# amazon-science/gnn-tail-generalization

Hardware: AMD Instinct MI355X
Metric: teachergnn_fullgraph_train_steps_per_sec (higher is better)
Workload: dtype f32

## Files before the change

gnn-tail-generalization_amd/_lib.py:

```python
import ctypes
import os

import torch

_HERE = os.path.dirname(os.path.abspath(__file__))
LIB_PATH = os.path.join(_HERE, 'lib', 'libcoldbrew_hip.so')

_c_i32p = ctypes.c_void_p
_c_f32p = ctypes.c_void_p
_I64 = ctypes.c_int64
_I32 = ctypes.c_int32
_SZ = ctypes.c_size_t
_P = ctypes.c_void_p


class CsrView(ctypes.Structure):
    _fields_ = [('rowptr', _P), ('col', _P), ('col_flags', _I32), ('n_rows', _I64), ('n_edges', _I64),
                ('hub_threshold', _I32), ('n_hubs', _I32), ('n_chunks', _I32), ('hub_rows', _P), ('hub_chunk_ptr', _P),
                ('ws', _P), ('ws_bytes', _SZ)]


class TrunkStore(ctypes.Structure):
    _fields_ = [('mix_src', _P), ('ld_mix', _I64), ('mix_index', _P), ('c_act', ctypes.c_float), ('c_mix', ctypes.c_float), ('drop_p', ctypes.c_float),
                ('seed', ctypes.c_uint64), ('seed_dev', _P), ('row0', _I64), ('relu_bits', _P), ('bits_relu_only', _I32), ('out_act', _P), ('ld_act', _I64)]


_G = ctypes.POINTER(CsrView)
_S = ctypes.POINTER(TrunkStore)

SIGNATURES = {
    'cb_version': (ctypes.c_int, []),
    'cb_last_error': (ctypes.c_char_p, []),
    'cb_device_status': (ctypes.c_int, []),
    'cb_agg_gemm_handover_selftest': (ctypes.c_int, [_P]),
    'cb_rows_zero_outside_mask_f32': (ctypes.c_int, [_P, _I64, _I64, _I64, _P, _P, _P]),
    'cb_csr_workspace_bytes': (_SZ, [_I64, _I64]),
    'cb_csr_from_coo_i64': (ctypes.c_int, [_P, _P, _I64, _I64, _P, _P, _P, _P, _P, _P, _SZ, _P]),
    'cb_deg_norm_f32': (ctypes.c_int, [_P, _I64, _P, _P]),
    'cb_csr64_from_coo_i64': (ctypes.c_int, [_P, _P, _I64, _I64, _P, _P, _P, _P, _P, _P, _SZ, _P]),
    'cb_csr_rebase_i64': (ctypes.c_int, [_P, _I64, _I64, _P, _P]),
    'cb_deg_norm_i64ptr_f32': (ctypes.c_int, [_P, _I64, _P, _P]),
    'cb_spmm_hub_count': (ctypes.c_int, [_P, _I64, _I32, _P, _P]),
    'cb_spmm_hub_fill_scratch_ints': (_I64, [_I64]),
    'cb_spmm_hub_fill': (ctypes.c_int, [_P, _I64, _I32, _I32, _P, _P, _P, _P]),
    'cb_spmm_workspace_bytes': (_SZ, [_I64, _I64]),
    'cb_spmm_csr_f32': (ctypes.c_int, [_G, _P, _I32, _I64, _I64, _P, _P, _P, ctypes.c_int, _P, _I64, _P, _I64, _P]),
    'cb_dropout_f32': (ctypes.c_int, [_P, _P, _I64, ctypes.c_float, ctypes.c_uint64, _P, _I64, _P]),
    'cb_axpby_f32': (ctypes.c_int, [ctypes.c_float, _P, ctypes.c_float, _P, _P, _I64, _P]),
    'cb_colsum_workspace_bytes': (_SZ, [_I64, _I64]),
    'cb_act_bwd_f32': (ctypes.c_int, [_P, _P, _P, _P, _I64, _I64, _P, _P, _SZ, _P]),
    'cb_reduce_workspace_bytes': (_SZ, []),
    'cb_frobenius_norm_f32': (ctypes.c_int, [_P, _I64, _P, _P, _SZ, _P]),
    'cb_nll_logsoftmax_f32': (ctypes.c_int, [_P, _I64, _P, _P, _I64, _I64, _I64, _P, _P, _P, _SZ, _P]),
    'cb_adam_step_f32': (ctypes.c_int, [_P, _P, _P, _P, _I64, ctypes.c_float, ctypes.c_float, ctypes.c_float,
                                        ctypes.c_float, ctypes.c_float, _I64, _P, _P]),
    'cb_adam_multi_f32': (ctypes.c_int, [_I32, _P, _P, _P, _P, _P, _P, ctypes.c_float, ctypes.c_float, ctypes.c_float, ctypes.c_float,
                                         ctypes.c_float, _I64, _P, _P, _P]),
    'cb_gemm_nn_workspace_bytes': (_SZ, [_I64, _I64]),
    'cb_gemm_nn_splitk_workspace_bytes': (_SZ, [_I64, _I64, _I64]),
    'cb_gemm_nn_f32': (ctypes.c_int, [_P, _I64, _P, _I64, _P, _I64, _I64, _I64, _I64, _P, _P, _I64, _P, ctypes.c_int, _P, _SZ, _P]),
    'cb_gemm_nn_drop2_f32': (ctypes.c_int, [_P, _I64, _P, _I64, _P, _I64, _P, _I64, _I64, _I64, _I64, _P, _P, _I64, _P, ctypes.c_int,
                                            ctypes.c_float, ctypes.c_uint64, _P, _I64, _P, _SZ, _P]),
    'cb_gemm_tn_workspace_bytes': (_SZ, [_I64, _I64, _I64]),
    'cb_gemm_tn_f32': (ctypes.c_int, [_P, _I64, _P, _I64, _P, _P, _I64, _I64, _I64, _P, _SZ, _P]),
    'cb_spmm_csr_fused_f32': (ctypes.c_int, [_G, _P, _P, _I32, _I64, _I64, _P, _P, _P, _I64, _S, _P, _I64, _P]),
    'cb_trunk_layer_bwd_f32': (ctypes.c_int, [_P, _P, _P, _P, ctypes.c_int, _P, ctypes.c_int, _I64, _I64, ctypes.c_float, ctypes.c_uint64,
                                              _P, _I64, ctypes.c_float, ctypes.c_float, _P, ctypes.c_uint64, ctypes.c_float, _P, _P, _P, _SZ, _P]),
    'cb_gemm_nn_bf16out_f32': (ctypes.c_int, [_P, _I64, _P, _I64, _P, _I64, _I64, _I64, _I64, _P, _P, _I64, _P, ctypes.c_int, _P, _SZ, _P]),
    'cb_node_norm_fwd_f32': (ctypes.c_int, [_P, _P, _P, _I64, _I64, ctypes.c_float, ctypes.c_float, ctypes.c_float, _P]),
    'cb_node_norm_bwd_f32': (ctypes.c_int, [_P, _P, _P, _P, _I64, _I64, ctypes.c_float, ctypes.c_float, _P]),
    'cb_colstats_workspace_bytes': (_SZ, [_I64, _I64]),
    'cb_colstats_f32': (ctypes.c_int, [_P, _P, _P, _I64, _I64, _P, _P, _P, _SZ, _P]),
    'cb_col_affine_f32': (ctypes.c_int, [_P, _P, _P, _P, ctypes.c_float, _P, _I64, _I64, _P]),
    'cb_col_bwd_combine_f32': (ctypes.c_int, [_P, _P, _P, _P, _P, _P, ctypes.c_float, ctypes.c_float, _P, _I64, _I64, _P]),
    'cb_topk_replace_workspace_bytes': (_SZ, [_I64, _I64, _I64]),
    'cb_topk_replace_f32': (ctypes.c_int, [_P, _I64, _P, _I64, _I64, _I64, _I64, _I32, _P, _P, _P, _P, _SZ, _P]),
    'cb_gather_rows_f32': (ctypes.c_int, [_P, _I64, _P, _I64, _I64, _P, _P]),
    'cb_gather_rows_bf16_f32': (ctypes.c_int, [_P, _I64, _P, _I64, _I64, _P, _P]),
    'cb_adam_norm_workspace_bytes': (ctypes.c_size_t, [_I32]),
    'cb_adam_multi_norm_f32': (ctypes.c_int, [_I32, _P, _P, _P, _P, _P, _P, _P, ctypes.c_float, ctypes.c_float, ctypes.c_float, ctypes.c_float,
                                              ctypes.c_float, _I64, _P, _P, _P, _SZ, _P]),
    'cb_expand_rows_f32': (ctypes.c_int, [_P, _P, _I64, _I64, ctypes.c_float, _P, _P]),
    'cb_gemm_nn_store_rows_supported': (ctypes.c_int, [_P, _I64, _P, _I64, _P, _I64, _I64, _I64, _I64]),
    'cb_gemm_nn_store_rows_f32': (ctypes.c_int, [_P, _I64, _P, _I64, _P, _I64, _I64, _I64, _I64, _P, _P, _I64, _P, _P, _S, _P, _SZ, _P]),
    'cb_trunk_store_rows_f32': (ctypes.c_int, [_P, _P, _I64, _I64, _S, _P, _P]),
    'cb_agg_gemm_image_bytes': (_SZ, [_I64, _I64]),
    'cb_agg_gemm_image_f32': (ctypes.c_int, [_P, _I64, _I64, _I64, ctypes.c_int, _P, _SZ, _P]),
    'cb_spmm_gemm_f32': (ctypes.c_int, [_G, _P, _I64, _I64, _P, _P, ctypes.c_int, _P, _I64, _P, _I64, _P, _P, _P, _I64, _P, _I64, _P]),
    'cb_spmm_gemm_fused_f32': (ctypes.c_int, [_G, _P, _I64, _P, _I64, _I64, _P, _P, _S, _P, _I64, _I32, _P, _P, _P, _I64, _P, _I64, _P]),
    'cb_agg_gemm_head_image_bytes': (_SZ, [_I64, _I64]),
    'cb_agg_gemm_head_image_f32': (ctypes.c_int, [_P, _I64, _I64, _I64, ctypes.c_int, _P, _SZ, _P]),
    'cb_spmm_gemm_fused_head_f32': (ctypes.c_int, [_G, _P, _I64, _P, _I64, _I64, _P, _P, _S, _P, _I64, _I32, _P, _P, _I64, _P, _I64, _P]),
    'cb_spmm_gemm_store_rows_f32': (ctypes.c_int, [_G, _P, _I64, _I64, _P, _P, _I64, _P, _P, _P, _P, _S, _P, _I64, _P]),
    'cb_spmm_csr_weighted_f32': (ctypes.c_int, [_P, _P, _P, _I64, _I64, _P, _I64, _I64, _P, _P, ctypes.c_int, _P, _I64, _P]),
    'cb_spmm_edge_dot_f32': (ctypes.c_int, [_P, _P, _I64, _I64, _P, _I64, _P, _I64, _I64, _P, _P]),
    'cb_gemm_nn_indrop_supported': (ctypes.c_int, [_P, _I64, _P, _I64, _P, _I64, _P, _I64, _I64, _I64, _I64]),
    'cb_gemm_nn_indrop_drop2_f32': (ctypes.c_int, [_P, _I64, _P, _I64, _P, _I64, _P, _I64, _I64, _I64, _I64, _P, ctypes.c_int, ctypes.c_float,
                                                   ctypes.c_uint64, ctypes.c_float, ctypes.c_uint64, _P, _I64, _P, _P]),
    'cb_gemm_nn_indrop_f32': (ctypes.c_int, [_P, _I64, _P, _I64, _P, _I64, _I64, _I64, _I64, _P, _P, _I64, _P, ctypes.c_int, ctypes.c_float,
                                             ctypes.c_uint64, _P, _I64, _P, _P]),
    'cb_gemm_tn_adrop_supported': (ctypes.c_int, [_P, _I64, _P, _I64, _I64, _I64]),
    'cb_gemm_tn_adrop_f32': (ctypes.c_int, [_P, _I64, _P, _I64, _P, _P, _I64, _I64, _I64, ctypes.c_float, ctypes.c_uint64, _P, _I64, _P, _SZ, _P]),
    'cb_front_image_bytes': (_SZ, [_I64]),
    'cb_front_image_f32': (ctypes.c_int, [_P, _I64, _I64, ctypes.c_int, _P, _SZ, _P]),
    'cb_trunk_front_f32': (ctypes.c_int, [_P, _I64, _I64, _I64, _P, _P, _P, _P, _P, _I64, _P, _I64, _P, _P, _I64, _P, _I64, ctypes.c_float,
                                          ctypes.c_uint64, ctypes.c_uint64, _P, _I64, _P]),
    'cb_gemm_tn_gdrop_supported': (ctypes.c_int, [_P, _I64, _P, _I64, _I64, _I64]),
    'cb_gemm_tn_gdrop_f32': (ctypes.c_int, [_P, _I64, _P, _I64, _P, _I64, _I64, _I64, ctypes.c_float, ctypes.c_uint64, _P, _I64, _P, _SZ, _P]),
    'cb_spmm_csr_lp_f32': (ctypes.c_int, [_G, _P, _I64, _I64, _P, _P, _I64, ctypes.c_float, _P, _P, _I64, _P]),
    'cb_spmm_csr_prop_f32': (ctypes.c_int, [_G, _P, _I64, _I64, _P, _P, _I64, ctypes.c_float, ctypes.c_float, ctypes.c_float, _P, _P, _P, _I64, _P]),
    'cb_cs_workspace_bytes': (_SZ, [_I64, _I64]),
    'cb_cs_residual_init_f32': (ctypes.c_int, [_P, _I64, _P, _P, _I64, _I64, _I64, _P, _P, _P, _P, _P, _SZ, _P]),
    'cb_cs_correct_snap_f32': (ctypes.c_int, [_I32, _P, _I64, _P, _I64, _P, _P, _I64, _I64, _I64, _P, _I64, ctypes.c_float, _P, _P, _I64, _P, _P, _P]),
    'cb_trunk_input_bwd_multi_f32': (ctypes.c_int, [_P, ctypes.c_uint64, _I32, _P, _P, ctypes.c_float, _P, _P, _I64, _I64, ctypes.c_float,
                                                    _P, _I64, _P, _P, _SZ, _P, _P, _P]),
    'cb_trunk_input_bwd_multi_cs_f32': (ctypes.c_int, [_P, ctypes.c_uint64, _I32, _P, _P, ctypes.c_float, _P, _P, _I64, _I64, ctypes.c_float,
                                                       _P, _I64, _P, _P, _SZ, _P, _P, _I32, _P, _P, _P, _P, _P, _SZ, _P]),
    'cb_spmm_csr_store_bwd_f32': (ctypes.c_int, [_G, _P, _I64, _I64, _P, _P, _P, ctypes.c_float, ctypes.c_float, ctypes.c_uint64, _P, _I64, _P, _I64, _P, _I64, _P]),
    'cb_spmm_store_bwd_mix_workspace_bytes': (_SZ, [_I64, _I64, _I64]),
    'cb_spmm_csr_store_bwd_mix_f32': (ctypes.c_int, [_G, _P, _I64, _I64, _P, _P, _P, ctypes.c_float, ctypes.c_float, ctypes.c_uint64, _P, _I64, _P, _I64, _P, _I64,
                                                     _I32, _P, _P, _P, ctypes.c_float, _P, _P, _SZ, _P]),
    'cb_gemm_tn_instage_supported': (ctypes.c_int, [_P, _P, _P, _I64, _I64, _I64]),
    'cb_gemm_tn_instage_workspace_bytes': (_SZ, [_I64, _I64]),
    'cb_gemm_tn_instage_f32': (ctypes.c_int, [_P, _P, _P, _P, _I64, _P, _P, _I64, _I64, ctypes.c_float, ctypes.c_uint64, ctypes.c_float, ctypes.c_uint64, _P, _I64,
                                              _P, _SZ, _P]),
    'cb_trunk_layer_bwd_fold_f32': (ctypes.c_int, [_P, _P, _P, _P, _I64, _I64, ctypes.c_float, ctypes.c_uint64, _P, _I64, ctypes.c_float, ctypes.c_float, _I32, _P, _P, _P,
                                                   _P, _P, _P, _SZ, _I32, _P, ctypes.c_float, _P, _P, _SZ, _P]),
    'cb_trunk_layer_bwd_rows_f32': (ctypes.c_int, [_P, _P, _I64, _P, _P, _P, _I64, ctypes.c_float, ctypes.c_uint64, _P, _I64, ctypes.c_float,
                                                   _P, ctypes.c_uint64, ctypes.c_float, _P, _P, _P, _SZ, _P]),
    'cb_id_count_i64': (ctypes.c_int, [_P, _I64, _I64, _P, _P, _P]),
    'cb_value_hist_i32': (ctypes.c_int, [_P, _I64, _I32, _P, _P, _P]),
    'cb_compact_workspace_bytes': (_SZ, [_I64]),
    'cb_select_range_i32': (ctypes.c_int, [_P, _I64, _I32, _I32, _P, _P, _P, _P, _SZ, _P]),
    'cb_craft_isolation_i64': (ctypes.c_int, [_P, _P, _I64, _P, _I64, _P, _P, _P, _P, _SZ, _P]),
    'cb_symmetrize_workspace_bytes': (_SZ, [_I64, _I64]),
    'cb_symmetrize_i64': (ctypes.c_int, [_P, _P, _I64, _I64, _P, _P, _P, _P, _P, _SZ, _P]),
    'cb_trunk_input_bwd_f32': (ctypes.c_int, [_P, _P, _P, _P, _I64, _I64, ctypes.c_float, ctypes.c_uint64, _P, _I64, _P, _P, _SZ, _P]),
    'cb_ln_gelu_drop_fwd_f32': (ctypes.c_int, [_P, _I64, _I64, _P, _P, ctypes.c_float, ctypes.c_float, ctypes.c_uint64, _P, _P, _P, _P]),
    'cb_ln_gelu_drop_bwd_workspace_bytes': (_SZ, [_I64, _I64]),
    'cb_ln_gelu_drop_bwd_f32': (ctypes.c_int, [_P, _P, _P, _I64, _I64, _P, _P, ctypes.c_float, ctypes.c_uint64, _P, _P, _P, _P, _P, _P, _SZ, _P]),
    'cb_mse_rows_f32': (ctypes.c_int, [_P, _I64, _I64, _P, _I64, _I64, _P, _P, _P, _P, _SZ, _P]),
    'cb_part2_assemble_f32': (ctypes.c_int, [_P, _I64, _P, _P, _I64, _P, _I64, _P, _P]),
    'cb_part2_assemble_bwd_f32': (ctypes.c_int, [_P, _I64, _P, _P, _I64, _I64, _P, _P, _SZ, _P]),
    'cb_ncloss_positions_i64': (ctypes.c_int, [_P, _I64, _I64, _P, _P, _P]),
    'cb_ncloss_row_norms_f32': (ctypes.c_int, [_P, _I64, _I64, _I64, _P, _P, _P]),
    'cb_cosine_scale_f32': (ctypes.c_int, [_P, _I64, _I64, _P, _P]),
    'cb_ncloss_uses_limb_core': (ctypes.c_int, [_P, _I64, _I64]),
    'cb_ncloss_workspace_bytes': (_SZ, [_I64, _I32]),
    'cb_ncloss_fwd_f32': (ctypes.c_int, [_P, _I64, _I64, _I64, ctypes.c_float, _P, _P, _P, _I64, _P, _P, _P, _I32, _P, _P, _P, _P, _P, _P, _P, _P, _SZ, _P]),
    'cb_ncloss_normalize_rows_f32': (ctypes.c_int, [_P, _I64, _I64, _I64, _P, _P, _P]),
    'cb_ncloss_bwd_slab_f32': (ctypes.c_int, [_P, _I64, _I64, _I64, ctypes.c_float, _P, _P, _I64, _I64, _I32, _P, _I64, _P]),
    'cb_ncloss_bwd_finish_f32': (ctypes.c_int, [_P, _I64, _P, _I64, _I64, ctypes.c_float, _P, _P, _P, _P, _P, _P, _P, _P, _I64, _P, _P, _P, _P, _P, _P, _P]),
    'cb_spgemm_offsets_workspace_bytes': (_SZ, [_I64]),
    'cb_spgemm_entry_offsets_i64': (ctypes.c_int, [_P, _I64, _P, _I64, _P, _P, _P, _SZ, _P]),
    'cb_spgemm_chunk_workspace_bytes': (_SZ, [_I64]),
    'cb_spgemm_chunk_count_f32': (ctypes.c_int, [_P, _P, _P, _P, _P, _P, _P, _I64, _I64, _I64, _I64, _I64, _P, _P, _SZ, _P]),
    'cb_spgemm_chunk_emit_f32': (ctypes.c_int, [_P, _SZ, _I64, _I64, _I64, _I64, _I64, _I64, _P, _P, _P, _P]),
    'cb_csr_transpose_workspace_bytes': (_SZ, [_I64]),
    'cb_csr_transpose_f32': (ctypes.c_int, [_P, _P, _P, _I64, _I64, _I64, _P, _P, _P, _P, _SZ, _P]),
    'cb_linkp_max_tries': (ctypes.c_int, []),
    'cb_linkp_valid_counts_i32': (ctypes.c_int, [_P, _P, _I32, _P, _P]),
    'cb_linkp_positives_i32': (ctypes.c_int, [_P, _P, _I32, _P, _I64, _I64, ctypes.c_uint64, _P, _P, _P]),
    'cb_linkp_negatives_i32': (ctypes.c_int, [_P, _P, _I32, _P, _I64, _I64, ctypes.c_uint64, _P, _P, _P, _P]),
    'cb_linkp_loss_fwd_f32': (ctypes.c_int, [_P, _I64, _I64, _I64, _P, _I64, _P, _I64, _P, _P, _P, _P, _P]),
    'cb_linkp_mrr_f32': (ctypes.c_int, [_P, _I64, _P, _I64, _P, _P]),
    'cb_linkp_bwd_workspace_bytes': (_SZ, [_I64, _I64]),
    'cb_linkp_loss_bwd_f32': (ctypes.c_int, [_P, _I64, _I64, _I64, _P, _I64, _P, _I64, _P, _P, _P, _I64, _P, _SZ, _P]),
    'cb_heur_aa_weights_f64': (ctypes.c_int, [_P, _P, _P]),
    'cb_heur_pair_scores_f32': (ctypes.c_int, [_P, _P, _P, _I64, _P, _P, _P]),
    'cb_heur_pair_scores_width_f32': (ctypes.c_int, [_P, _P, _P, _I64, _I32, _P, _P, _P]),
    'cb_rank_counts_workspace_bytes': (_SZ, [_I64, _I64]),
    'cb_rank_counts_f32': (ctypes.c_int, [_P, _I64, _P, _I64, _P, _P, _P, _P, _SZ, _P]),
    'cb_pair_gemm_nn_supported': (ctypes.c_int, [_P, _I64, _P, _I64, _I64, _I64]),
    'cb_pair_gemm_nn_f32': (ctypes.c_int, [_P, _I64, _I64, _P, _I64, _P, _I64, _P, _I64, _P, _I64, _I64, _I64, _P, ctypes.c_int, ctypes.c_float,
                                           ctypes.c_uint64, _P, _I64, _P, _P]),
    'cb_pair_dot_f32': (ctypes.c_int, [_P, _I64, _I64, _I64, _P, _I64, _P, _P, _P]),
    'cb_pair_scatter_workspace_bytes': (_SZ, [_I64]),
    'cb_pair_scatter_f32': (ctypes.c_int, [_P, _I64, _I64, _I64, _P, _I64, _P, _I64, _P, _I64, _P, _SZ, _P]),
    'cb_rank_loss_workspace_bytes': (_SZ, []),
    'cb_rank_loss_fwd_f32': (ctypes.c_int, [_I32, _P, _I64, _P, _I64, _P, _P, _P, _SZ, _P]),
    'cb_rank_loss_bwd_f32': (ctypes.c_int, [_I32, _P, _I64, _P, _I64, _P, _P, _P, _P, _P]),
    'cb_sage_image_bytes': (_SZ, [ctypes.c_int]),
    'cb_sage_image_f32': (ctypes.c_int, [_P, _I64, _P, _I64, ctypes.c_int, _P, _SZ, _P]),
    'cb_sage_layer_supported': (ctypes.c_int, [_I64, _I64, _I32, _P, _I64, _P, _I64, _P, _I64, _P, _I64]),
    'cb_sage_layer_f32': (ctypes.c_int, [_P, _P, _I64, _P, _I64, _P, _P, _P, _P, ctypes.c_int, ctypes.c_float, ctypes.c_uint64, _P, _I64, _P, _I64, _I32,
                                         _P, _I64, _P]),
}

_lib = None


class HipExtensionError(RuntimeError):
    pass


def load():
    global _lib
    if _lib is not None:
        return _lib
    if not os.path.isfile(LIB_PATH):
        raise HipExtensionError(
            f'{LIB_PATH} not found: the HIP extension is required (no CPU fallback). '
            'Build it with `python __graft_entry__.py` or `make -C gnn-tail-generalization_amd/csrc`.')
    lib = ctypes.CDLL(LIB_PATH)
    for name, (res, args) in SIGNATURES.items():
        fn = getattr(lib, name)
        fn.restype = res
        fn.argtypes = args
# ... 69 lines not shown
```

gnn-tail-generalization_amd/csrc/cb_front.hip:

```cpp
#include "cb_common.h"
#include "cb_limb_core.h"
#include "cb_philox.h"
#include "cb_tile_gemm.h"
#include "cb_trunk_store.h"

namespace cb {

struct FrontArgs {
  const float* x;
  int64_t ld_x;
  const uint4* image_in;
  const float* bias_in;
  const uint4* image_0;
  const float* rowscale;
  const float* addend;
  int64_t ld_add;
  float* x0;
  int64_t ld_x0;
  unsigned long long* bits;
  float* x0_drop;
  int64_t ld_drop;
  float* z0;
  int64_t ld_z;
  int64_t M;
  uint32_t thresh;
  float keep_scale;
  uint64_t seed_x, seed_x0;
  const uint64_t* seed_dev;
  int64_t row0;
  int n_tiles;
};

template <int NS1>
__global__ void __launch_bounds__(256, 2) k_front(FrontArgs fa) {
  constexpr int K1 = 16 * NS1, LDX = K1 + 4, NV = kTM * K1 / 4 / 256;
  static_assert(NV >= 1 && kTM * LDX <= kTM * kTLD, "x tile must fit the region of the X0 tile");
  __shared__ __attribute__((aligned(16))) float tile[kTM * kTLD];
  constexpr int kScratch = 2 * RowOperand<kTM>::BYTES > 4 * 8 * kCLD * 4 ? 2 * RowOperand<kTM>::BYTES : 4 * 8 * kCLD * 4;
  __shared__ __attribute__((aligned(16))) char scratch[kScratch];
  float (*cstrip)[8 * kCLD] = reinterpret_cast<float (*)[8 * kCLD]>(scratch);
  __shared__ float rs_tile[2][kTM];
  const int t = threadIdx.x, lane = t & 63, w = __builtin_amdgcn_readfirstlane(t >> 6);
  const uint64_t sx = fa.seed_dev ? fa.seed_x + *fa.seed_dev : fa.seed_x, s0 = fa.seed_dev ? fa.seed_x0 + *fa.seed_dev : fa.seed_x0;
  float4 xr[NV];
  auto load_x = [&](int tile_id) {
    const int64_t m0 = (int64_t)tile_id * kTM;
#pragma unroll
    for (int j = 0; j < NV; ++j) {
      const int idx = t + 256 * j, row = idx / (K1 / 4), c4 = idx % (K1 / 4);
      const int64_t m = m0 + row;
      xr[j] = (tile_id < fa.n_tiles && m < fa.M) ? *reinterpret_cast<const float4*>(fa.x + m * fa.ld_x + 4 * c4) : make_float4(0.f, 0.f, 0.f, 0.f);
    }
  };
  float bvec[4] = {0.f, 0.f, 0.f, 0.f};
  if (fa.bias_in) {
#pragma unroll
    for (int i = 0; i < 4; ++i) bvec[i] = fa.bias_in[4 * lane + i];
  }
  int par = 0;
  for (int tile_id = blockIdx.x; tile_id < fa.n_tiles; tile_id += gridDim.x, par ^= 1) {
    const int64_t m0 = (int64_t)tile_id * kTM;
    load_x(tile_id);
#pragma unroll
    for (int j = 0; j < NV; ++j) {
      const int idx = t + 256 * j, row = idx / (K1 / 4), c4 = idx % (K1 / 4);
      float v[4] = {xr[j].x, xr[j].y, xr[j].z, xr[j].w};
      if (fa.thresh) {
        float mk[4];
        keep4(sx, ((fa.row0 + m0 + row) * K1 + 4 * c4) >> 2, fa.thresh, fa.keep_scale, mk);
#pragma unroll
        for (int i = 0; i < 4; ++i) v[i] = mul_rounded(v[i], mk[i]);
      }
      *reinterpret_cast<float4*>(tile + row * LDX + 4 * c4) = make_float4(v[0], v[1], v[2], v[3]);
    }
    if (t < kTM) rs_tile[par][t] = (fa.rowscale && m0 + t < fa.M) ? fa.rowscale[m0 + t] : 1.f;
    __syncthreads();
    f32x16 acc[2][2];
    tile_times_image_coop<NS1, LDX, 1>(tile, scratch, fa.image_in, w, lane, t, acc);
    {
      const int l31 = lane & 31, lh = lane >> 5;
#pragma unroll
      for (int i = 0; i < 2; ++i)
#pragma unroll
        for (int j = 0; j < 2; ++j)
#pragma unroll
          for (int reg = 0; reg < 16; ++reg)
            tile[(32 * i + (reg & 3) + 8 * (reg >> 2) + 4 * lh) * kTLD + 64 * w + 32 * j + l31] = acc[i][j][reg];
    }
    __syncthreads();
#pragma unroll 4
    for (int r = 0; r < 16; ++r) {
      const int row = 16 * w + r;
      const int64_t m = m0 + row;
      float* tp = tile + row * kTLD + 4 * lane;
      const float4 v = *reinterpret_cast<const float4*>(tp);
      float o[4] = {v.x, v.y, v.z, v.w};
#pragma unroll
      for (int i = 0; i < 4; ++i) o[i] = fmaxf(o[i] + bvec[i], 0.f);
      float xd[4] = {o[0], o[1], o[2], o[3]};
      if (fa.thresh) {
        float mk[4];
        keep4(s0, ((fa.row0 + m) * kND + 4 * lane) >> 2, fa.thresh, fa.keep_scale, mk);
#pragma unroll
        for (int i = 0; i < 4; ++i) xd[i] = o[i] * mk[i];
      }
      *reinterpret_cast<float4*>(tp) = make_float4(xd[0], xd[1], xd[2], xd[3]);
      if (m < fa.M) {
        store_stream4(fa.x0 + m * fa.ld_x0 + 4 * lane, o);
        if (fa.bits) {
          const bool pos[4] = {o[0] > 0.f, o[1] > 0.f, o[2] > 0.f, o[3] > 0.f};
          write_row_mask_words(fa.bits + m * 4, lane, pos);
        }
        if (fa.x0_drop) store_stream4(fa.x0_drop + m * fa.ld_drop + 4 * lane, xd);
      }
    }
    __syncthreads();
    tile_times_image_coop<kNS, kTLD, 1>(tile, scratch, fa.image_0, w, lane, t, acc);
    acc_rows_through_strip(acc, cstrip[w], w, lane, [&](int row, int n, const float4& v) {
      const int64_t m = m0 + row;
      if (m < fa.M) {
        const float rs = rs_tile[par][row];
        float ad[4] = {0.f, 0.f, 0.f, 0.f};
        if (fa.addend) {
          const float4 a4 = *reinterpret_cast<const float4*>(fa.addend + m * fa.ld_add + n);
          ad[0] = a4.x; ad[1] = a4.y; ad[2] = a4.z; ad[3] = a4.w;
        }
        const float zero_bias = 0.f;
        float o[4] = {v.x, v.y, v.z, v.w};
#pragma unroll
        for (int e = 0; e < 4; ++e) o[e] = o[e] * rs + ad[e] + zero_bias;
        store_stream4(fa.z0 + m * fa.ld_z + n, o);
      }
    });
  }
}

}

using namespace cb;

extern "C" size_t cb_front_image_bytes(int64_t K) {
  if (K != 64 && K != 128) return 0;
  return (size_t)(K / 16) * kNT * 3 * 64 * sizeof(uint4);
}

extern "C" int cb_front_image_f32(const float* W, int64_t ld, int64_t K, int transpose, void* image, size_t image_bytes, void* stream) {
  CB_CHECK_ARG(cb_front_image_bytes(K) > 0, CB_E_INVALID, "cb_front_image_f32: K must be 64 or 128 (got %lld)", (long long)K);
  CB_CHECK_ARG(W && image && ld >= (transpose ? K : kND), CB_E_INVALID, "cb_front_image_f32: null pointer / bad leading dimension");
  CB_CHECK_ARG(image_bytes >= cb_front_image_bytes(K) && aligned16(image), CB_E_WORKSPACE, "cb_front_image_f32: image buffer too small or misaligned");
  const int64_t sk = transpose ? 1 : ld, sn = transpose ? ld : 1;
  const int ns = (int)(K / 16);
  hipLaunchKernelGGL(k_weight_image, dim3(ns * kNT * 64 / 256), dim3(256), 0, (hipStream_t)stream, W, sk, sn, (uint4*)image, ns);
  CB_LAUNCH_CHECK();
  return CB_OK;
}

extern "C" int cb_trunk_front_f32(const float* x, int64_t ld_x, int64_t M, int64_t K, const void* image_in, const float* bias_in, const void* image_0,
                                  const float* rowscale, const float* addend, int64_t ld_add, float* x0, int64_t ld_x0, uint64_t* relu_bits,
                                  float* x0_drop, int64_t ld_drop, float* z0, int64_t ld_z, float drop_p, uint64_t seed_x, uint64_t seed_x0,
                                  const uint64_t* seed_dev, int64_t row0, void* stream) {
  CB_CHECK_ARG(M >= 0 && cb_front_image_bytes(K) > 0 && drop_p >= 0.f && drop_p < 1.f && row0 >= 0, CB_E_INVALID,
               "cb_trunk_front_f32: bad size (K must be 64 or 128; hidden width 256) or p");
  CB_CHECK_ARG(M < ((int64_t)1 << 31) * kTM / 2, CB_E_RANGE, "cb_trunk_front_f32: size out of range");
  if (M == 0) return CB_OK;
  CB_CHECK_ARG(x && image_in && image_0 && x0 && z0, CB_E_INVALID, "cb_trunk_front_f32: null pointer");
  CB_CHECK_ARG(aligned16(x) && ld_x % 4 == 0 && ld_x >= K && aligned16(image_in) && aligned16(image_0) && aligned16(x0) && ld_x0 % 4 == 0 && ld_x0 >= kND &&
                   aligned16(z0) && ld_z % 4 == 0 && ld_z >= kND && (!addend || (aligned16(addend) && ld_add % 4 == 0 && ld_add >= kND)) &&
                   (!x0_drop || (aligned16(x0_drop) && ld_drop % 4 == 0 && ld_drop >= kND)) && (!relu_bits || (uintptr_t)relu_bits % 8 == 0),
               CB_E_INVALID, "cb_trunk_front_f32: 16-byte aligned rows required");
  FrontArgs fa{x, ld_x, (const uint4*)image_in, bias_in, (const uint4*)image_0, rowscale, addend, ld_add, x0, ld_x0, (unsigned long long*)relu_bits,
               x0_drop, ld_drop, z0, ld_z, M};
  fa.thresh = drop_p > 0.f ? dropout_threshold(drop_p) : 0u;
  fa.keep_scale = 1.f / (1.f - drop_p);
  fa.seed_x = seed_x; fa.seed_x0 = seed_x0; fa.seed_dev = seed_dev; fa.row0 = row0;
  fa.n_tiles = (int)((M + kTM - 1) / kTM);
  int dev = 0, n_cu = 0;
  if (hipGetDevice(&dev) != hipSuccess || hipDeviceGetAttribute(&n_cu, hipDeviceAttributeMultiprocessorCount, dev) != hipSuccess || n_cu <= 0) n_cu = 256;
  const int blocks = fa.n_tiles < 2 * n_cu ? fa.n_tiles : 2 * n_cu;
  const dim3 grid((unsigned)blocks), blk(256);
  hipStream_t st = (hipStream_t)stream;
  if (K == 64) hipLaunchKernelGGL((k_front<4>), grid, blk, 0, st, fa);
  else hipLaunchKernelGGL((k_front<8>), grid, blk, 0, st, fa);
  CB_LAUNCH_CHECK();
  return CB_OK;
}
```

gnn-tail-generalization_amd/csrc/cb_gemm.hip:

```cpp
#include <stdlib.h>

#include "cb_common.h"
#include "cb_gemm_core.h"
#include "cb_gemm_limb.h"

namespace cb {

template <int WM, int WN, bool ALIGNED, bool OUT_BF16, int BKT = BK, int WTN = 2>
__global__ void __launch_bounds__(256) k_gemm_nn(const float* __restrict__ A, int64_t lda, const float* __restrict__ B, int64_t ldb,
                                                 void* __restrict__ Cv, int64_t ldc, int64_t M, int N, int K, GemmEpilogue ep,
                                                 int n_row_blocks, int n_col_blocks, int c_vec_ok, int k_chunk) {
  using T = Tile<WM, WN, BKT, WTN>;
  if (k_chunk) {
    const int k0 = blockIdx.y * k_chunk;
    A += k0;
    B += (int64_t)k0 * ldb;
    Cv = reinterpret_cast<float*>(Cv) + (int64_t)blockIdx.y * M * ldc;
    K = min(k_chunk, K - k0);
  }
  constexpr int BM = T::BM, BN = T::BN, LDA = T::LDA, LDB = T::LDB;
  __shared__ __attribute__((aligned(16))) float smem[T::SMEM_FLOATS];
  auto As = [&](int b) { return smem + b * (BKT * LDA); };
  auto Bs = [&](int b) { return smem + 2 * BKT * LDA + b * (BKT * LDB); };
  const int per_group = 8 * n_col_blocks;
// ... 323 lines not shown
extern "C" int cb_gemm_nn_store_rows_supported(const float* A, int64_t lda, const float* B, int64_t ldb, const float* C, int64_t ldc, int64_t M, int64_t N,
                                               int64_t K) {
  return use_limb3() && N == 256 && M > 0 && limb3_nn_eligible(A, lda, B, ldb, N, K) && aligned16(C) && ldc % 4 == 0 ? 1 : 0;
}

extern "C" int cb_gemm_nn_store_rows_f32(const float* A, int64_t lda, const float* B, int64_t ldb, float* C, int64_t ldc, int64_t M, int64_t N, int64_t K,
                                         const float* rowscale, const float* addend, int64_t ld_add, const float* bias, const int64_t* row_index,
                                         const cb_trunk_store* store, void* ws, size_t ws_bytes, void* stream) {
  CB_CHECK_ARG(M >= 0 && N == 256 && K > 0, CB_E_INVALID, "cb_gemm_nn_store_rows_f32: bad size (N must be 256)");
  CB_CHECK_ARG(K < (1 << 24) && (M + 63) / 64 < (1 << 24), CB_E_RANGE, "cb_gemm_nn_store_rows_f32: size out of range");
  if (M == 0) return CB_OK;
  CB_CHECK_ARG(A && B && C && row_index && lda >= K && ldb >= N && ldc >= N && (!addend || ld_add >= N), CB_E_INVALID,
               "cb_gemm_nn_store_rows_f32: null pointer or leading dimension too small");
  const int rcs = check_trunk_store("cb_gemm_nn_store_rows_f32", store, N);
  if (rcs != CB_OK) return rcs;
  CB_CHECK_ARG(cb_gemm_nn_store_rows_supported(A, lda, B, ldb, C, ldc, M, N, K) && (!addend || (aligned16(addend) && ld_add % 4 == 0)), CB_E_INVALID,
               "cb_gemm_nn_store_rows_f32: shape / alignment outside the fused form (cb_gemm_nn_store_rows_supported)");
  GemmEpilogue ep{rowscale, addend, ld_add, bias, 1, nullptr, 0, 0u, 1.f, 0ull, nullptr, 0, 0};
  ep.row_ids = row_index; ep.st = make_trunk_store(*store);
  return launch_nn_limb3(A, lda, B, ldb, C, ldc, M, N, K, ep, false, (hipStream_t)stream, ws, ws_bytes);
}

extern "C" int cb_gemm_tn_f32(const float* A, int64_t lda, const float* G, int64_t ldg, const float* rowscale, float* C, int64_t M,
                              int64_t K1, int64_t K2, void* ws, size_t ws_bytes, void* stream) {
  CB_CHECK_ARG(M >= 0 && K1 >= 0 && K2 >= 0, CB_E_INVALID, "cb_gemm_tn_f32: negative size");
  CB_CHECK_ARG(K1 < (1 << 20) && K2 < (1 << 20), CB_E_RANGE, "cb_gemm_tn_f32: size out of range");
  if (K1 == 0 || K2 == 0) return CB_OK;
  CB_CHECK_ARG(C && (M == 0 || (A && G)) && lda >= K1 && ldg >= K2, CB_E_INVALID, "cb_gemm_tn_f32: null pointer or bad ld");
  hipStream_t st = (hipStream_t)stream;
  if (M == 0) {
    CB_HIP(hipMemsetAsync(C, 0, (size_t)K1 * K2 * sizeof(float), st));
    return CB_OK;
  }
  CB_CHECK_ARG(ws && ws_bytes >= cb_gemm_tn_workspace_bytes(M, K1, K2), CB_E_WORKSPACE, "cb_gemm_tn_f32: workspace too small");
  int bm, bn;
  tn_tile(K1, K2, bm, bn);
  if (bm == 64) return launch_tn<1, 4>(A, lda, G, ldg, rowscale, C, M, K1, K2, (float*)ws, st);
  if (bm == 256) return launch_tn<4, 1>(A, lda, G, ldg, rowscale, C, M, K1, K2, (float*)ws, st);
  return launch_tn<2, 2>(A, lda, G, ldg, rowscale, C, M, K1, K2, (float*)ws, st);
}

extern "C" int cb_gemm_tn_gdrop_supported(const float* A, int64_t lda, const float* G, int64_t ldg, int64_t K1, int64_t K2) {
  return use_limb3() && K2 % 4 == 0 && limb3_tn_eligible(A, lda, G, ldg, K1, K2) ? 1 : 0;
}

extern "C" int cb_gemm_tn_gdrop_f32(const float* A, int64_t lda, const float* G, int64_t ldg, float* C, int64_t M, int64_t K1, int64_t K2,
                                    float g_drop_p, uint64_t g_seed, const uint64_t* seed_dev, int64_t row0, void* ws, size_t ws_bytes,
                                    void* stream) {
  CB_CHECK_ARG(M >= 0 && K1 >= 0 && K2 >= 0 && g_drop_p > 0.f && g_drop_p < 1.f && row0 >= 0, CB_E_INVALID, "cb_gemm_tn_gdrop_f32: bad size or p");
  CB_CHECK_ARG(K1 < (1 << 20) && K2 < (1 << 20), CB_E_RANGE, "cb_gemm_tn_gdrop_f32: size out of range");
  if (K1 == 0 || K2 == 0) return CB_OK;
  CB_CHECK_ARG(C && (M == 0 || (A && G)) && lda >= K1 && ldg >= K2, CB_E_INVALID, "cb_gemm_tn_gdrop_f32: null pointer or bad ld");
  hipStream_t st = (hipStream_t)stream;
  if (M == 0) {
    CB_HIP(hipMemsetAsync(C, 0, (size_t)K1 * K2 * sizeof(float), st));
    return CB_OK;
  }
  CB_CHECK_ARG(cb_gemm_tn_gdrop_supported(A, lda, G, ldg, K1, K2), CB_E_INVALID, "cb_gemm_tn_gdrop_f32: operands outside the three-limb path");
  CB_CHECK_ARG(ws && ws_bytes >= cb_gemm_tn_workspace_bytes(M, K1, K2), CB_E_WORKSPACE, "cb_gemm_tn_gdrop_f32: workspace too small");
  const DropSpec gd{dropout_threshold(g_drop_p), 1.f / (1.f - g_drop_p), g_seed, seed_dev, row0, K2};
  int bm, bn;
  tn_tile(K1, K2, bm, bn);
  if (bm == 64) return launch_tn<1, 4>(A, lda, G, ldg, nullptr, C, M, K1, K2, (float*)ws, st, &gd);
  if (bm == 256) return launch_tn<4, 1>(A, lda, G, ldg, nullptr, C, M, K1, K2, (float*)ws, st, &gd);
  return launch_tn<2, 2>(A, lda, G, ldg, nullptr, C, M, K1, K2, (float*)ws, st, &gd);
}

static inline int instage_splits(int64_t M) { return tn_splits(M, 2); }

extern "C" int cb_gemm_tn_instage_supported(const float* g, const float* mfold, const float* X, int64_t ldx, int64_t M, int64_t K2) {
  return use_limb3() && K2 > 64 && K2 <= 128 && K2 % 4 == 0 && ldx % 4 == 0 && ldx >= K2 && ldx < (1 << 22) && aligned16(g) && aligned16(mfold) && aligned16(X) && M > 0 &&
                 instage_splits(M) >= 256
             ? 1
             : 0;
}

extern "C" size_t cb_gemm_tn_instage_workspace_bytes(int64_t M, int64_t K2) {
  if (M <= 0 || K2 <= 0) return 0;
  return (size_t)instage_splits(M) * (size_t)256 * (size_t)(K2 + 1) * sizeof(float);
}

extern "C" int cb_gemm_tn_instage_f32(const float* g, const float* mfold, const uint64_t* x0_bits, const float* X, int64_t ldx, float* C, float* colsum, int64_t M,
                                      int64_t K2, float g_drop_p, uint64_t g_seed, float x_drop_p, uint64_t x_seed, const uint64_t* seed_dev, int64_t row0, void* ws,
                                      size_t ws_bytes, void* stream) {
  CB_CHECK_ARG(M > 0 && K2 > 0 && g_drop_p > 0.f && g_drop_p < 1.f && x_drop_p > 0.f && x_drop_p < 1.f && row0 >= 0, CB_E_INVALID,
               "cb_gemm_tn_instage_f32: bad size or p (both dropouts must be active)");
  CB_CHECK_ARG(g && mfold && x0_bits && X && C && colsum && (uintptr_t)x0_bits % 8 == 0, CB_E_INVALID, "cb_gemm_tn_instage_f32: null or misaligned pointer");
  CB_CHECK_ARG(cb_gemm_tn_instage_supported(g, mfold, X, ldx, M, K2), CB_E_INVALID, "cb_gemm_tn_instage_f32: shape / alignment outside the fused form (cb_gemm_tn_instage_supported)");
  CB_CHECK_ARG(ws && ws_bytes >= cb_gemm_tn_instage_workspace_bytes(M, K2), CB_E_WORKSPACE, "cb_gemm_tn_instage_f32: workspace too small");
  hipStream_t st = (hipStream_t)stream;
  const int nsplit = instage_splits(M);
  int64_t rows_per_split = (M + nsplit - 1) / nsplit;
  rows_per_split = (rows_per_split + 31) / 32 * 32;
  const DropSpec xd{dropout_threshold(x_drop_p), 1.f / (1.f - x_drop_p), x_seed, seed_dev, row0, K2};
  const DropSpec gd{dropout_threshold(g_drop_p), 1.f / (1.f - g_drop_p), g_seed, seed_dev, row0, 256};
  float* partial = (float*)ws;
  float* cs_partial = partial + (size_t)nsplit * 256 * K2;
  const int rc = launch_tn_instage(g, mfold, x0_bits, X, ldx, partial, cs_partial, M, K2, nsplit, rows_per_split, st, xd, gd);
  if (rc != CB_OK) return rc;
  const int64_t n = 256 * K2;
  hipLaunchKernelGGL(k_sum_partials, dim3((unsigned)((n + 255) / 256)), dim3(256), 0, st, (const float*)partial, nsplit, n, C);
  CB_LAUNCH_CHECK();
  hipLaunchKernelGGL(k_sum_partials, dim3(1), dim3(256), 0, st, (const float*)cs_partial, nsplit, (int64_t)256, colsum);
  CB_LAUNCH_CHECK();
  return CB_OK;
}

extern "C" int cb_gemm_nn_indrop_f32(const float* A, int64_t lda, const float* B, int64_t ldb, float* C, int64_t ldc, int64_t M, int64_t N, int64_t K,
                                     const float* rowscale, const float* addend, int64_t ld_add, const float* bias, int relu, float a_drop_p,
                                     uint64_t a_seed, const uint64_t* seed_dev, int64_t row0, uint64_t* relu_bits, void* stream) {
  CB_CHECK_ARG(M >= 0 && N >= 0 && K >= 0 && a_drop_p > 0.f && a_drop_p < 1.f && row0 >= 0, CB_E_INVALID, "cb_gemm_nn_indrop_f32: bad size or p");
  CB_CHECK_ARG(!relu_bits || (N == 256 && relu && (uintptr_t)relu_bits % 8 == 0), CB_E_INVALID,
               "cb_gemm_nn_indrop_f32: mask words of the ReLU exist for N == 256 with relu only");
  CB_CHECK_ARG(N < (1 << 24) && K < (1 << 24) && (M + 63) / 64 < (1 << 24), CB_E_RANGE, "cb_gemm_nn_indrop_f32: size out of range");
  if (M == 0 || N == 0) return CB_OK;
  CB_CHECK_ARG(C && A && B && lda >= K && ldb >= N && ldc >= N && (!addend || ld_add >= N), CB_E_INVALID, "cb_gemm_nn_indrop_f32: null pointer or bad ld");
  CB_CHECK_ARG(cb_gemm_nn_indrop_supported(A, lda, B, ldb, C, ldc, C, ldc, M, N, K) && (!addend || (aligned16(addend) && ld_add % 4 == 0)), CB_E_INVALID,
               "cb_gemm_nn_indrop_f32: shape / alignment outside the fused form (cb_gemm_nn_indrop_supported)");
  GemmEpilogue ep{rowscale, addend, ld_add, bias, relu, nullptr, 0, 0u, 1.f, 0ull, nullptr, 0, gemm_nt_store(M, N)};
  ep.adrop = DropSpec{dropout_threshold(a_drop_p), 1.f / (1.f - a_drop_p), a_seed, seed_dev, row0, K};
  ep.relu_bits_out = (unsigned long long*)relu_bits;
  return launch_nn_limb3(A, lda, B, ldb, C, ldc, M, N, K, ep, false, (hipStream_t)stream, nullptr, 0);
}

extern "C" int cb_gemm_tn_adrop_supported(const float* A, int64_t lda, const float* G, int64_t ldg, int64_t K1, int64_t K2) {
  int bm, bn;
  tn_tile(K1, K2, bm, bn);
  return use_limb3() && K1 % 4 == 0 && bm == 128 && limb3_tn_eligible(A, lda, G, ldg, K1, K2) ? 1 : 0;
}

extern "C" int cb_gemm_tn_adrop_f32(const float* A, int64_t lda, const float* G, int64_t ldg, const float* rowscale, float* C, int64_t M, int64_t K1,
                                    int64_t K2, float a_drop_p, uint64_t a_seed, const uint64_t* seed_dev, int64_t row0, void* ws, size_t ws_bytes,
                                    void* stream) {
  CB_CHECK_ARG(M >= 0 && K1 >= 0 && K2 >= 0 && a_drop_p > 0.f && a_drop_p < 1.f && row0 >= 0, CB_E_INVALID, "cb_gemm_tn_adrop_f32: bad size or p");
  CB_CHECK_ARG(K1 < (1 << 20) && K2 < (1 << 20), CB_E_RANGE, "cb_gemm_tn_adrop_f32: size out of range");
  if (K1 == 0 || K2 == 0) return CB_OK;
  CB_CHECK_ARG(C && (M == 0 || (A && G)) && lda >= K1 && ldg >= K2, CB_E_INVALID, "cb_gemm_tn_adrop_f32: null pointer or bad ld");
  hipStream_t st = (hipStream_t)stream;
  if (M == 0) {
    CB_HIP(hipMemsetAsync(C, 0, (size_t)K1 * K2 * sizeof(float), st));
    return CB_OK;
  }
  CB_CHECK_ARG(cb_gemm_tn_adrop_supported(A, lda, G, ldg, K1, K2), CB_E_INVALID, "cb_gemm_tn_adrop_f32: operands outside the three-limb 128-row tile path");
  CB_CHECK_ARG(ws && ws_bytes >= cb_gemm_tn_workspace_bytes(M, K1, K2), CB_E_WORKSPACE, "cb_gemm_tn_adrop_f32: workspace too small");
  const DropSpec ad{dropout_threshold(a_drop_p), 1.f / (1.f - a_drop_p), a_seed, seed_dev, row0, K1};
  return launch_tn<2, 2>(A, lda, G, ldg, rowscale, C, M, K1, K2, (float*)ws, st, nullptr, &ad);
}
```

gnn-tail-generalization_amd/csrc/cb_gemm_core.h:

```cpp
#pragma once
#include "cb_common.h"
#include "cb_philox.h"
#include "cb_trunk_store.h"

namespace cb {

typedef float f32x16 __attribute__((ext_vector_type(16)));

constexpr int BK = 16;

struct DropSpec {
  uint32_t thresh;
  float scale;
  uint64_t seed;
  const uint64_t* seed_dev;
  int64_t row0;
  int64_t width;
};

struct GemmEpilogue {
  const float* rowscale;
  const float* addend;
  int64_t ld_add;
  const float* bias;
  int relu;
  float* out2;
  int64_t ld_out2;
  uint32_t thresh;
  float keep_scale;
  uint64_t seed;
  const uint64_t* seed_dev;
  int64_t row0;
  int nt_store;
  DropSpec adrop;
  unsigned long long* relu_bits_out;
  const int64_t* row_ids;
  TrunkStore st;
};

template <int WM, int WN, int BKT = BK, int WTN = 2>
struct Tile {
  static constexpr int BM = 64 * WM, BN = 32 * WTN * WN, LDA = BM + 4, LDB = BN + 4;
  static constexpr int SMEM_FLOATS = 2 * BKT * (LDA + LDB);
  static_assert(WM * WN == 4, "four wavefronts per block");
  static_assert(32 * LDB <= SMEM_FLOATS, "epilogue staging (32 rows) must fit the operand buffers");
};

template <int LDA, int LDB, int BKT, int WTN>
__device__ __forceinline__ void mfma_tile_step(const float* __restrict__ As, const float* __restrict__ Bs, int wr, int wc,
                                               int lane, f32x16 (&acc)[2][WTN]) {
  const int l31 = lane & 31, kh = lane >> 5;
  const float* ar = As + kh * LDA + wr * 64 + l31;
  const float* br = Bs + kh * LDB + wc * (32 * WTN) + l31;
  float a[2], b[WTN];
  a[0] = ar[0]; a[1] = ar[32];
#pragma unroll
  for (int j = 0; j < WTN; ++j) b[j] = br[32 * j];
#pragma unroll
  for (int kk = 0; kk < BKT; kk += 2) {
    float na[2] = {0.f, 0.f}, nb[WTN];
#pragma unroll
    for (int j = 0; j < WTN; ++j) nb[j] = 0.f;
    if (kk + 2 < BKT) {
      na[0] = ar[(kk + 2) * LDA];
      na[1] = ar[(kk + 2) * LDA + 32];
#pragma unroll
      for (int j = 0; j < WTN; ++j) nb[j] = br[(kk + 2) * LDB + 32 * j];
    }
#pragma unroll
    for (int i = 0; i < 2; ++i)
#pragma unroll
      for (int j = 0; j < WTN; ++j) acc[i][j] = __builtin_amdgcn_mfma_f32_32x32x2f32(a[i], b[j], acc[i][j], 0, 0, 0);
    a[0] = na[0]; a[1] = na[1];
#pragma unroll
    for (int j = 0; j < WTN; ++j) b[j] = nb[j];
  }
}

template <int BMT, int BKT>
struct RowFrag {
  float v[BMT * BKT / 1024][4];
};
template <bool ALIGNED, int BMT, int BKT>
__device__ __forceinline__ void load_rowmajor(RowFrag<BMT, BKT>& f, const float* __restrict__ A, int64_t lda, int64_t m0, int64_t M,
                                              int k0, int K, int t) {
  constexpr int TPR = BKT / 4, RPP = 256 / TPR;
  const int k = k0 + (t % TPR) * 4;
#pragma unroll
  for (int j = 0; j < BMT / RPP; ++j) {
    const int64_t m = m0 + t / TPR + RPP * j;
    if (ALIGNED && m < M && k + 4 <= K) {
      const float4 x = *reinterpret_cast<const float4*>(A + m * lda + k);
      f.v[j][0] = x.x; f.v[j][1] = x.y; f.v[j][2] = x.z; f.v[j][3] = x.w;
    } else {
#pragma unroll
      for (int i = 0; i < 4; ++i) f.v[j][i] = (m < M && k + i < K) ? A[m * lda + k + i] : 0.f;
    }
  }
}
template <int BMT, int BKT>
// ... 220 lines not shown
```

gnn-tail-generalization_amd/csrc/cb_gemm_limb.hip:

```cpp
#include <utility>

#include "cb_common.h"
#include "cb_gemm_core.h"
#include "cb_gemm_limb.h"
#include "cb_limb_core.h"

namespace cb {

template <int WM, int WN, int WTN = 2, int PD = 1>
struct LTile {
  static constexpr int BM = 64 * WM, BN = 32 * WTN * WN;
  static constexpr int MINW = (WM == 2 && WTN == 2 && PD < 3 ? 3 : 2);
  static constexpr int NTHR = 64 * WM * WN;
  static_assert(WM * WN == 4 || WM * WN == 8, "four or eight wavefronts per block");
};

template <int WM, int WN, bool OUT_BF16, int WTN = 2, int PD = 1, int EPI = 0, bool ADROP = false>
__global__ void __launch_bounds__(256, (LTile<WM, WN, WTN, PD>::MINW)) k_gemm_nn_l3(const float* __restrict__ A, int64_t lda,
                                                                                 const float* __restrict__ B, int64_t ldb,
                                                                                 void* __restrict__ Cv, int64_t ldc, int64_t M, int N,
                                                                                 int K, GemmEpilogue ep, int n_row_blocks,
                                                                                 int n_col_blocks, int c_vec_ok) {
  using T = LTile<WM, WN, WTN>;
  using OA = RowOperand<T::BM, ADROP>;
  using OB = ColOperand<T::BN, false>;
  constexpr int BM = T::BM, BN = T::BN;
  constexpr int SMEM = 2 * (OA::BYTES + OB::BYTES);
  static_assert(32 * (BN + 4) * 4 <= SMEM, "epilogue staging must fit");
  __shared__ __attribute__((aligned(16))) char smem[SMEM];
  const int per_group = 8 * n_col_blocks;
  const int grp = blockIdx.x / per_group, r = blockIdx.x % per_group;
  const int row_blk = grp * 8 + (r & 7), col_blk = r >> 3;
  if (row_blk >= n_row_blocks) return;
  const int64_t m0 = (int64_t)row_blk * BM;
  const int n0 = col_blk * BN;
  const int t = threadIdx.x, lane = t & 63, w = t >> 6, wr = w / WN, wc = w % WN;

  f32x16 acc[2][WTN];
  zero_acc_n<WTN>(acc);
  OA oa;
  OB ob;
  oa.init(lda, M - m0, t);
  if constexpr (ADROP) oa.set_drop(ep.adrop, m0, K, t);
  ob.init(ldb, N - n0, t);
  const uint32_t aaddr[2] = {OA::frag_addr(wr * 64, lane), OA::frag_addr(wr * 64 + 32, lane)};
  uint32_t baddr[WTN];
#pragma unroll
  for (int j = 0; j < WTN; ++j) baddr[j] = OB::frag_addr(wc * (32 * WTN) + 32 * j, lane);
  limb_k_loop<WTN, PD, OA, OB>(oa, ob, smem, A + m0 * lda, KS, lda, B + n0, (int64_t)KS * ldb, ldb, nullptr, K, aaddr, baddr, acc, t);
  nn_epilogue<WM, WN, WTN, OUT_BF16, EPI>(acc, reinterpret_cast<float*>(smem), Cv, ldc, m0, n0, M, N, ep, c_vec_ok, t);
}

template <int WM, int WN, bool SCALED, int WTN = 2, int PD = 1, bool GDROP = false, bool ADROP = false>
__global__ void __launch_bounds__((LTile<WM, WN, WTN, PD>::NTHR), (LTile<WM, WN, WTN, PD>::MINW)) k_gemm_tn_l3(const float* __restrict__ A, int64_t lda,
                                                                                 const float* __restrict__ G, int64_t ldg,
                                                                                 const float* __restrict__ rowscale,
                                                                                 float* __restrict__ partial, int64_t M, int K1, int K2,
                                                                                 int64_t rows_per_split, int tiles_j, int n_tiles,
                                                                                 int nsplit, DropSpec gd) {
  using T = LTile<WM, WN, WTN>;
  using OA = ColOperand<T::BM, false, ADROP, T::NTHR>;
  using OB = ColOperand<T::BN, SCALED, GDROP, T::NTHR>;
  constexpr int BM = T::BM, BN = T::BN;
  __shared__ __attribute__((aligned(16))) char smem[2 * (OA::BYTES + OB::BYTES)];
  const int b = blockIdx.x;
  const int tile = (b >> 3) % n_tiles, split = (b & 7) + 8 * (b / (8 * n_tiles));
  if (split >= nsplit) return;
  const int i0 = (tile / tiles_j) * BM, j0 = (tile % tiles_j) * BN;
  const int64_t r_begin = (int64_t)split * rows_per_split;
  const int64_t r_end = min(M, r_begin + rows_per_split);
  const int t = threadIdx.x, lane = t & 63, w = t >> 6, wr = w / WN, wc = w % WN;

  f32x16 acc[2][WTN];
  zero_acc_n<WTN>(acc);
  OA oa;
  OB ob;
  oa.init(lda, K1 - i0, t);
  ob.init(ldg, K2 - j0, t);
  if constexpr (GDROP) ob.set_drop(gd, r_begin, r_end - r_begin, j0, t);
  if constexpr (ADROP) oa.set_drop(gd, r_begin, r_end - r_begin, i0, t);
  const uint32_t aaddr[2] = {OA::frag_addr(wr * 64, lane), OA::frag_addr(wr * 64 + 32, lane)};
  uint32_t baddr[WTN];
#pragma unroll
  for (int j = 0; j < WTN; ++j) baddr[j] = OB::frag_addr(wc * (32 * WTN) + 32 * j, lane);
  limb_k_loop<WTN, PD, OA, OB>(oa, ob, smem, A + r_begin * lda + i0, (int64_t)KS * lda, lda, G + r_begin * ldg + j0, (int64_t)KS * ldg, ldg,
                           SCALED ? rowscale + r_begin : nullptr, r_end - r_begin, aaddr, baddr, acc, t);
  const int l31 = lane & 31, lh = lane >> 5;
  float* P = partial + (int64_t)split * K1 * K2;
#pragma unroll
  for (int ti = 0; ti < 2; ++ti)
#pragma unroll
    for (int tj = 0; tj < WTN; ++tj) {
      const int n = j0 + wc * (32 * WTN) + tj * 32 + l31;
      if (n >= K2) continue;
#pragma unroll
      for (int reg = 0; reg < 16; ++reg) {
        const int m = i0 + wr * 64 + ti * 32 + (reg & 3) + 8 * (reg >> 2) + 4 * lh;
        if (m < K1) P[(int64_t)m * K2 + n] = acc[ti][tj][reg];
      }
    }
}

__global__ void __launch_bounds__(512, 2) k_gemm_tn_instage(const float* __restrict__ g, const float* __restrict__ mfold,
                                                            const unsigned long long* __restrict__ x0_bits, const float* __restrict__ X, int64_t ldx,
                                                            float* __restrict__ partial, float* __restrict__ cs_partial, int64_t M, int K2,
                                                            int64_t rows_per_split, int nsplit, DropSpec xd, DropSpec gd) {
  using T = LTile<4, 2, 2>;
  using OA = ColOperandInStage<T::NTHR>;
  using OB = ColOperand<T::BN, false, true, T::NTHR>;
  constexpr int K1 = 256;
  __shared__ __attribute__((aligned(16))) char smem[2 * (OA::BYTES + OB::BYTES)];
  const int split = blockIdx.x;
  if (split >= nsplit) return;
  const int64_t r_begin = (int64_t)split * rows_per_split;
  const int64_t r_end = min(M, r_begin + rows_per_split);
  const int t = threadIdx.x, lane = t & 63, w = t >> 6, wr = w / 2, wc = w % 2;

  f32x16 acc[2][2];
  zero_acc_n<2>(acc);
  OA oa;
  OB ob;
  oa.init(K1, K1, t);
  ob.init(ldx, K2, t);
  oa.set_stage(g, mfold, x0_bits + r_begin * 4, gd, r_begin, r_end - r_begin, t);
  ob.set_drop(xd, r_begin, r_end - r_begin, 0, t);
  const uint32_t aaddr[2] = {OA::frag_addr(wr * 64, lane), OA::frag_addr(wr * 64 + 32, lane)};
  uint32_t baddr[2];
#pragma unroll
  for (int j = 0; j < 2; ++j) baddr[j] = OB::frag_addr(wc * 64 + 32 * j, lane);
  limb_k_loop<2, 1, OA, OB>(oa, ob, smem, g + r_begin * K1, (int64_t)KS * K1, K1, X + r_begin * ldx, (int64_t)KS * ldx, ldx, nullptr, r_end - r_begin, aaddr, baddr,
                            acc, t);
  const int l31 = lane & 31, lh = lane >> 5;
  float* P = partial + (int64_t)split * K1 * K2;
#pragma unroll
  for (int ti = 0; ti < 2; ++ti)
#pragma unroll
    for (int tj = 0; tj < 2; ++tj) {
      const int n = wc * 64 + tj * 32 + l31;
      if (n >= K2) continue;
#pragma unroll
      for (int reg = 0; reg < 16; ++reg) {
        const int m = wr * 64 + ti * 32 + (reg & 3) + 8 * (reg >> 2) + 4 * lh;
        P[(int64_t)m * K2 + n] = acc[ti][tj][reg];
      }
    }
  float* red = reinterpret_cast<float*>(smem);
#pragma unroll
  for (int i = 0; i < 4; ++i) red[w * 256 + lane * 4 + i] = oa.cs[i];
  __syncthreads();
  if (t < 256) {
    float s = 0.f;
#pragma unroll
    for (int j = 0; j < 8; ++j) s += red[j * 256 + t];
    cs_partial[(int64_t)split * 256 + t] = s;
  }
}

int launch_tn_instage(const float* g, const float* mfold, const uint64_t* x0_bits, const float* X, int64_t ldx, float* partial, float* cs_partial, int64_t M, int64_t K2,
                      int nsplit, int64_t rows_per_split, hipStream_t st, const DropSpec& xd, const DropSpec& gd) {
  hipLaunchKernelGGL(k_gemm_tn_instage, dim3((unsigned)nsplit), dim3(512), 0, st, g, mfold, (const unsigned long long*)x0_bits, X, ldx, partial, cs_partial, M, (int)K2,
                     rows_per_split, nsplit, xd, gd);
  CB_LAUNCH_CHECK();
  return CB_OK;
}

template <int WM, int WN, bool OUT_BF16, int WTN = 2>
static int launch_nn_l3_t(const float* A, int64_t lda, const float* B, int64_t ldb, void* C, int64_t ldc, int64_t M, int64_t N,
                          int64_t K, GemmEpilogue ep, hipStream_t st, void* ws = nullptr, size_t ws_bytes = 0) {
  using T = LTile<WM, WN, WTN>;
  const int nrb = (int)((M + T::BM - 1) / T::BM), ncb = (int)((N + T::BN - 1) / T::BN);
  const int64_t groups = (nrb + 7) / 8;
  const int c_vec_ok = ((uintptr_t)C % (OUT_BF16 ? 8 : 16) == 0) && ldc % 4 == 0 && (!ep.addend || (aligned16(ep.addend) && ep.ld_add % 4 == 0));
  const dim3 grid((unsigned)(groups * 8 * ncb));
  if constexpr (!OUT_BF16 && WM == 2 && WTN == 4) {
    if (ep.out2) {
      if (ep.adrop.thresh)
        hipLaunchKernelGGL((k_gemm_nn_l3<WM, WN, false, WTN, 1, 1, true>), grid, dim3(256), 0, st, A, lda, B, ldb, C, ldc, M, (int)N, (int)K, ep,
                           nrb, ncb, c_vec_ok);
      else
        hipLaunchKernelGGL((k_gemm_nn_l3<WM, WN, false, WTN, 1, 1>), grid, dim3(256), 0, st, A, lda, B, ldb, C, ldc, M, (int)N, (int)K, ep, nrb,
                           ncb, c_vec_ok);
      CB_LAUNCH_CHECK();
      return CB_OK;
    }
    if (ep.row_ids) {
      hipLaunchKernelGGL((k_gemm_nn_l3<WM, WN, false, WTN, 1, 2>), grid, dim3(256), 0, st, A, lda, B, ldb, C, ldc, M, (int)N, (int)K, ep, nrb, ncb, c_vec_ok);
      CB_LAUNCH_CHECK();
      return CB_OK;
    }
    if (ep.adrop.thresh) {
      hipLaunchKernelGGL((k_gemm_nn_l3<WM, WN, false, WTN, 1, 0, true>), grid, dim3(256), 0, st, A, lda, B, ldb, C, ldc, M, (int)N, (int)K, ep, nrb,
                         ncb, c_vec_ok);
      CB_LAUNCH_CHECK();
      return CB_OK;
    }
  }
  CB_CHECK_ARG(!ep.adrop.thresh, CB_E_INVALID, "NN contraction with operand dropout: wide fp32 tile only (check cb_gemm_nn_indrop_supported first)");
  hipLaunchKernelGGL((k_gemm_nn_l3<WM, WN, OUT_BF16, WTN, 1>), grid, dim3(256), 0, st, A, lda, B, ldb, C, ldc, M, (int)N, (int)K, ep, nrb, ncb,
                     c_vec_ok);
  CB_LAUNCH_CHECK();
  return CB_OK;
}

bool limb3_nn_eligible(const float* A, int64_t lda, const float* B, int64_t ldb, int64_t N, int64_t K) {
  return aligned16(A) && aligned16(B) && lda % 4 == 0 && ldb % 4 == 0 && K % 4 == 0 && N % 4 == 0 && K > 0 && lda < (1 << 22) && ldb < (1 << 22);
}

bool limb3_nn_dual_eligible(const float* A, int64_t lda, const float* B, int64_t ldb, const float* C, int64_t ldc, const float* C2, int64_t ldc2,
                            int64_t M, int64_t N, int64_t K, const GemmEpilogue& ep) {
  return N > 128 && ((M + 127) / 128) * ((N + 255) / 256) >= 256 && limb3_nn_eligible(A, lda, B, ldb, N, K) && aligned16(C) && aligned16(C2) && ldc % 4 == 0 && ldc2 % 4 == 0 &&
         (!ep.addend || (aligned16(ep.addend) && ep.ld_add % 4 == 0));
}

size_t limb3_nn_workspace_bytes(int64_t, int64_t) { return 0; }

int launch_nn_limb3(const float* A, int64_t lda, const float* B, int64_t ldb, void* C, int64_t ldc, int64_t M, int64_t N, int64_t K,
                    const GemmEpilogue& ep, bool out_bf16, hipStream_t st, void* ws, size_t ws_bytes) {
  if (N <= 64) {
    return out_bf16 ? launch_nn_l3_t<4, 1, true>(A, lda, B, ldb, C, ldc, M, N, K, ep, st)
                    : launch_nn_l3_t<4, 1, false>(A, lda, B, ldb, C, ldc, M, N, K, ep, st);
  }
  const bool fills = ((M + 127) / 128) * ((N + 255) / 256) >= 256 || ep.out2 || ep.adrop.thresh || ep.row_ids;
  if (N > 128 && fills)
    return out_bf16 ? launch_nn_l3_t<2, 2, true, 4>(A, lda, B, ldb, C, ldc, M, N, K, ep, st, ws, ws_bytes)
                    : launch_nn_l3_t<2, 2, false, 4>(A, lda, B, ldb, C, ldc, M, N, K, ep, st, ws, ws_bytes);
  return out_bf16 ? launch_nn_l3_t<2, 2, true>(A, lda, B, ldb, C, ldc, M, N, K, ep, st, ws, ws_bytes)
                  : launch_nn_l3_t<2, 2, false>(A, lda, B, ldb, C, ldc, M, N, K, ep, st, ws, ws_bytes);
}

template <int WM, int WN, int WTN = 2>
static void launch_tn_l3_t(const float* A, int64_t lda, const float* G, int64_t ldg, const float* rowscale, float* partial, int64_t M,
                           int64_t K1, int64_t K2, int nsplit, int64_t rows_per_split, hipStream_t st, const DropSpec& gd, const DropSpec& ad) {
  using T = LTile<WM, WN, WTN>;
  const int ti = (int)((K1 + T::BM - 1) / T::BM), tj = (int)((K2 + T::BN - 1) / T::BN);
  const dim3 grid((unsigned)(((nsplit + 7) / 8) * 8 * ti * tj));
#define CB_TN_LAUNCH(SC_, GD_, AD_)                                                                                                  \
  hipLaunchKernelGGL((k_gemm_tn_l3<WM, WN, SC_, WTN, 1, GD_, AD_>), grid, dim3(T::NTHR), 0, st, A, lda, G, ldg, rowscale, partial, M, (int)K1, \
                     (int)K2, rows_per_split, tj, ti * tj, nsplit, gd.thresh ? gd : ad)
  if (gd.thresh) CB_TN_LAUNCH(false, true, false);
  else if (ad.thresh) {
    if constexpr (WM == 2 && WN == 2 && WTN == 2) { if (rowscale) CB_TN_LAUNCH(true, false, true); else CB_TN_LAUNCH(false, false, true); }
  } else if (rowscale) CB_TN_LAUNCH(true, false, false);
  else CB_TN_LAUNCH(false, false, false);
#undef CB_TN_LAUNCH
}

bool limb3_tn_eligible(const float* A, int64_t lda, const float* G, int64_t ldg, int64_t K1, int64_t K2) {
  return aligned16(A) && aligned16(G) && lda % 4 == 0 && ldg % 4 == 0 && K1 % 4 == 0 && K2 % 4 == 0 && lda < (1 << 22) && ldg < (1 << 22);
}

int launch_tn_limb3(const float* A, int64_t lda, const float* G, int64_t ldg, const float* rowscale, float* partial, int64_t M,
                    int64_t K1, int64_t K2, int bm, int nsplit, int64_t rows_per_split, hipStream_t st, const DropSpec* gdrop, const DropSpec* adrop) {
  const DropSpec gd = gdrop ? *gdrop : DropSpec{};
  const DropSpec ad = adrop ? *adrop : DropSpec{};
  CB_CHECK_ARG(!gd.thresh || (!rowscale && gd.width % 4 == 0 && !ad.thresh), CB_E_INVALID,
               "TN contraction: dropout of the G operand needs width %% 4 == 0, no row scale and no dropout of A");
  CB_CHECK_ARG(!ad.thresh || (ad.width % 4 == 0 && bm == 128), CB_E_INVALID, "TN contraction: dropout of the A operand needs width %% 4 == 0 and the 128-row tile");
  if (bm == 64) launch_tn_l3_t<1, 4>(A, lda, G, ldg, rowscale, partial, M, K1, K2, nsplit, rows_per_split, st, gd, ad);
  else if (bm == 256) launch_tn_l3_t<4, 1>(A, lda, G, ldg, rowscale, partial, M, K1, K2, nsplit, rows_per_split, st, gd, ad);
  else {
    if (!ad.thresh && !gd.thresh && K1 == 256 && K2 == 256 && nsplit >= 256) {
      launch_tn_l3_t<4, 2, 4>(A, lda, G, ldg, rowscale, partial, M, K1, K2, nsplit, rows_per_split, st, gd, ad);
      CB_LAUNCH_CHECK();
      return CB_OK;
    }
    if (gd.thresh && !ad.thresh && !rowscale && K1 == 256 && K2 <= 128 && K2 > 64 && nsplit >= 256) {
      launch_tn_l3_t<4, 2, 2>(A, lda, G, ldg, rowscale, partial, M, K1, K2, nsplit, rows_per_split, st, gd, ad);
      CB_LAUNCH_CHECK();
      return CB_OK;
    }
    if (!ad.thresh && K2 > 128 && ((K1 + 127) / 128) * ((K2 + 255) / 256) * nsplit >= 256) launch_tn_l3_t<2, 2, 4>(A, lda, G, ldg, rowscale, partial, M, K1, K2, nsplit, rows_per_split, st, gd, ad);
    else launch_tn_l3_t<2, 2>(A, lda, G, ldg, rowscale, partial, M, K1, K2, nsplit, rows_per_split, st, gd, ad);
  }
  CB_LAUNCH_CHECK();
  return CB_OK;
}

}
```

gnn-tail-generalization_amd/csrc/cb_limb_core.h:

```cpp
#pragma once
#include <utility>

#include "cb_common.h"
#include "cb_gemm_core.h"
#include "cb_philox.h"

namespace cb {

typedef __bf16 bf16x8 __attribute__((ext_vector_type(8)));

typedef float f32x2 __attribute__((ext_vector_type(2)));
typedef __bf16 bf16x2 __attribute__((ext_vector_type(2)));
__device__ __forceinline__ uint32_t cvt_pk_bf16(float x0, float x1) {
  const f32x2 v = {x0, x1};
  return __builtin_bit_cast(uint32_t, __builtin_convertvector(v, bf16x2));
}
__device__ __forceinline__ void split3x2(float a0, float a1, uint32_t& hi, uint32_t& mid, uint32_t& lo) {
  hi = cvt_pk_bf16(a0, a1);
  const float r0 = a0 - __uint_as_float(hi << 16), r1 = a1 - __uint_as_float(hi & 0xffff0000u);
  mid = cvt_pk_bf16(r0, r1);
  const float s0 = r0 - __uint_as_float(mid << 16), s1 = r1 - __uint_as_float(mid & 0xffff0000u);
  lo = cvt_pk_bf16(s0, s1);
}

// ... 47 lines not shown
      const bool in = row + 64 * j < rows_left;
      rmask |= in ? (1u << j) : 0u;
      voff[j] = in ? (uint32_t)((row + 64 * j) * ld + kq * 4) : 0u;
    }
  }
  template <int J>
  __device__ __forceinline__ void load(float4 (&f)[NV], const float* __restrict__ base, int64_t , int64_t k_left, const float*,
                                       int t) const {
    f[J] = *reinterpret_cast<const float4*>(base + ((t & 3) * 4 < k_left ? voff[J] : 0u));
  }
  template <int J>
  __device__ __forceinline__ void stage(const float4 (&f)[NV], char* __restrict__ S, int64_t k_left, int t) const {
    const bool live = ((rmask >> J) & 1) && (t & 3) * 4 < k_left;
    float v[4] = {live ? f[J].x : 0.f, live ? f[J].y : 0.f, live ? f[J].z : 0.f, live ? f[J].w : 0.f};
    if constexpr (DROP) {
      float mk[4];
      keep4(dseed, (dbase[J] + (dK - k_left)) >> 2, dthresh, dscale, mk);
#pragma unroll
      for (int i = 0; i < 4; ++i) v[i] = mul_rounded(v[i], mk[i]);
    }
    uint2 pl[3];
    split4(v, pl);
#pragma unroll
    for (int p = 0; p < 3; ++p) *reinterpret_cast<uint2*>(S + p * PLANE + woff + J * (64 * 32)) = pl[p];
  }
  static __device__ __forceinline__ uint32_t frag_addr(int r0, int lane) {
    const int row = r0 + (lane & 31);
    return row * 32 + (((lane >> 5) ^ ((row >> 3) & 1)) << 4);
  }
  static __device__ __forceinline__ bf16x8 frag(const char* __restrict__ S, uint32_t addr, int plane) {
    return __builtin_bit_cast(bf16x8, *reinterpret_cast<const uint4*>(S + plane * PLANE + addr));
  }
};

template <int R>
struct PairRowOperand {
  static constexpr int PLANE = R * 32, BYTES = 3 * PLANE, NV = R / 64;
  static_assert(NV >= 1, "tile rows");
  int32_t nu[NV], nv[NV];
  uint32_t woff;
  static constexpr bool HAS_SC = false;
  float sc[1];
  float4 fv[NV];
  static __device__ __forceinline__ bool pair_of(const int32_t* __restrict__ pairs, int64_t S, int64_t rows_left, int64_t N, int row, int& u, int& v, bool& in) {
    in = row < rows_left;
    u = in ? pairs[row] : 0;
    v = in ? pairs[S + row] : 0;
    return in && u >= 0 && u < N && v >= 0 && v < N;
  }
  __device__ __forceinline__ void init(const int32_t* __restrict__ pairs, int64_t S, int64_t rows_left, int64_t N, int t) {
    const int row = t >> 2, kq = t & 3;
    woff = row * 32 + (((kq >> 1) ^ ((row >> 3) & 1)) << 4) + ((kq & 1) << 3);
#pragma unroll
    for (int j = 0; j < NV; ++j) {
      int u, v;
      bool in;
      const bool ok = pair_of(pairs, S, rows_left, N, row + 64 * j, u, v, in);
      nu[j] = ok ? u : -1;
      nv[j] = ok ? v : 0;
    }
  }
  template <int J>
  __device__ __forceinline__ void load(float4 (&f)[NV], const float* __restrict__ base, int64_t ld, int64_t k_left, const float*, int t) {
    const int kq4 = (t & 3) * 4 < k_left ? (t & 3) * 4 : 0;
    f[J] = *reinterpret_cast<const float4*>(base + ((int64_t)(nu[J] < 0 ? 0 : nu[J]) * ld + kq4));
    fv[J] = *reinterpret_cast<const float4*>(base + ((int64_t)nv[J] * ld + kq4));
  }
  template <int J>
  __device__ __forceinline__ void stage(const float4 (&f)[NV], char* __restrict__ S, int64_t k_left, int t) const {
    const bool live = nu[J] >= 0 && (t & 3) * 4 < k_left;
    const float a[4] = {f[J].x, f[J].y, f[J].z, f[J].w}, b[4] = {fv[J].x, fv[J].y, fv[J].z, fv[J].w};
    float v[4];
#pragma unroll
    for (int i = 0; i < 4; ++i) v[i] = live ? mul_rounded(a[i], b[i]) : 0.f;
    uint2 pl[3];
    split4(v, pl);
#pragma unroll
    for (int p = 0; p < 3; ++p) *reinterpret_cast<uint2*>(S + p * PLANE + woff + J * (64 * 32)) = pl[p];
  }
  static __device__ __forceinline__ uint32_t frag_addr(int r0, int lane) { return RowOperand<R>::frag_addr(r0, lane); }
  static __device__ __forceinline__ bf16x8 frag(const char* __restrict__ S, uint32_t addr, int plane) { return RowOperand<R>::frag(S, addr, plane); }
};

template <int C, bool SCALED, bool DROP = false, int NT = 256>
struct ColOperand {
  static constexpr int ROWB = C * 2, PLANE = 16 * ROWB, BYTES = 3 * PLANE;
  static constexpr int TPR = C / 4, KPP = NT / TPR, NV = 16 / KPP;
  static_assert(KPP >= 4 && KPP % 4 == 0 && NV >= 1, "staging map: whole swizzle groups of k rows per pass");
  static constexpr int NC = C / 32;
  static_assert(NC == 2 || NC == 4 || NC == 8, "tile widths 64 / 128 / 256");
  static __device__ __forceinline__ int swz(int k) { return NC == 2 ? ((k >> 1) & 1) : (k & 3); }
  uint32_t voff[NV];
  uint32_t woff;
  bool cok;
  static constexpr bool HAS_SC = SCALED;
  float sc[SCALED ? NV : 1];
  uint64_t dseed;
  uint32_t dthresh;
  float dscale;
  int64_t drow, dtot, dwidth;
  int dcol;
  __device__ __forceinline__ void set_drop(const DropSpec& d, int64_t r_begin, int64_t total, int j0, int t) {
    dseed = d.seed_dev ? d.seed + *d.seed_dev : d.seed;
    dthresh = d.thresh;
    dscale = d.scale;
    drow = d.row0 + r_begin + t / TPR;
    dtot = total;
    dwidth = d.width;
    dcol = j0 + (t % TPR) * 4;
  }
  __device__ __forceinline__ void init(int64_t ld, int cols_left, int t) {
    const int k = t / TPR, nq = t % TPR;
    cok = nq * 4 < cols_left;
#pragma unroll
    for (int j = 0; j < NV; ++j) voff[j] = (uint32_t)((k + KPP * j) * ld + (cok ? nq * 4 : 0));
    woff = k * ROWB + ((((nq >> 3) ^ swz(k)) & (NC - 1)) << 6) + ((nq & 7) << 3);
  }
  template <int J>
  __device__ __forceinline__ void load(float4 (&f)[NV], const float* __restrict__ base, int64_t , int64_t k_left,
                                       const float* __restrict__ kscale, int t) {
    const int k = t / TPR + KPP * J;
    const bool kin = k < k_left;
    f[J] = *reinterpret_cast<const float4*>(base + (kin ? voff[J] : 0u));
    if constexpr (SCALED) sc[J] = kscale[kin ? k : 0];
  }
  template <int J>
  __device__ __forceinline__ void stage(const float4 (&f)[NV], char* __restrict__ S, int64_t k_left, int t) const {
    const bool live = cok && t / TPR + KPP * J < k_left;
    const float m = SCALED ? sc[SCALED ? J : 0] : 1.f;
    float v[4] = {live ? f[J].x * m : 0.f, live ? f[J].y * m : 0.f, live ? f[J].z * m : 0.f, live ? f[J].w * m : 0.f};
    if constexpr (DROP) {
      static_assert(!SCALED, "dropout of a row-scaled operand is not needed anywhere");
      float mk[4];
      keep4(dseed, ((drow + KPP * J + (dtot - k_left)) * dwidth + dcol) >> 2, dthresh, dscale, mk);
#pragma unroll
      for (int i = 0; i < 4; ++i) v[i] = mul_rounded(v[i], mk[i]);
    }
    uint2 pl[3];
    split4(v, pl);
#pragma unroll
    for (int p = 0; p < 3; ++p) *reinterpret_cast<uint2*>(S + p * PLANE + woff + J * (KPP * ROWB)) = pl[p];
  }
  static __device__ __forceinline__ uint32_t frag_addr(int c0, int lane) {
    const int L = lane & 15, k = 8 * (lane >> 5) + (L >> 2);
    return k * ROWB + ((((c0 >> 5) ^ swz(k)) & (NC - 1)) << 6) + (((lane >> 4) & 1) << 5) + ((L & 3) << 3);
  }
  static __device__ __forceinline__ bf16x8 frag(const char* __restrict__ S, uint32_t addr, int plane) {
    const char* q = S + plane * PLANE + addr;
    const s16x4 lo = __builtin_amdgcn_ds_read_tr16_b64_v4i16((lds_s16x4*)(q));
    const s16x4 hi = __builtin_amdgcn_ds_read_tr16_b64_v4i16((lds_s16x4*)(q + 4 * ROWB));
    typedef short s16x8 __attribute__((ext_vector_type(8)));
    const s16x8 v = __builtin_shufflevector(lo, hi, 0, 1, 2, 3, 4, 5, 6, 7);
    return __builtin_bit_cast(bf16x8, v);
  }
};

template <int NT = 512>
struct ColOperandInStage {
  static constexpr int C = 256;
  static constexpr int ROWB = C * 2, PLANE = 16 * ROWB, BYTES = 3 * PLANE;
  static constexpr int TPR = C / 4, KPP = NT / TPR, NV = 16 / KPP;
  static_assert(TPR == 64 && KPP >= 4 && KPP % 4 == 0 && NV >= 1, "one wavefront per k row");
  static constexpr int NC = C / 32;
  static __device__ __forceinline__ int swz(int k) { return k & 3; }
  uint32_t voff[NV];
  uint32_t woff;
  bool cok;
  static constexpr bool HAS_SC = false;
  float sc[1];
  int64_t mdelta;
  const unsigned long long* bits;
  float4 fm[NV];
  unsigned long long bw[NV][4];
  uint64_t dseed;
  uint32_t dthresh;
  float dscale;
  int64_t drow, dtot, dwidth;
  int dcol, kw;
  float cs[4];
  __device__ __forceinline__ void set_stage(const float* g, const float* mfold, const unsigned long long* bits_block, const DropSpec& d, int64_t r_begin, int64_t total,
                                            int t) {
    mdelta = mfold - g;
    bits = bits_block;
    dseed = d.seed_dev ? d.seed + *d.seed_dev : d.seed;
    dthresh = d.thresh;
    dscale = d.scale;
    kw = __builtin_amdgcn_readfirstlane(t / TPR);
    drow = d.row0 + r_begin + kw;
    dtot = total;
    dwidth = d.width;
    dcol = (t % TPR) * 4;
#pragma unroll
    for (int i = 0; i < 4; ++i) cs[i] = 0.f;
  }
  __device__ __forceinline__ void init(int64_t ld, int cols_left, int t) {
    const int k = t / TPR, nq = t % TPR;
    cok = nq * 4 < cols_left;
#pragma unroll
    for (int j = 0; j < NV; ++j) voff[j] = (uint32_t)((k + KPP * j) * ld + (cok ? nq * 4 : 0));
    woff = k * ROWB + ((((nq >> 3) ^ swz(k)) & (NC - 1)) << 6) + ((nq & 7) << 3);
  }
  template <int J>
  __device__ __forceinline__ void load(float4 (&f)[NV], const float* __restrict__ base, int64_t , int64_t k_left, const float* __restrict__, int ) {
    const int k = kw + KPP * J;
    const bool kin = k < k_left;
    const float* p = base + (kin ? voff[J] : 0u);
    f[J] = *reinterpret_cast<const float4*>(p);
    fm[J] = *reinterpret_cast<const float4*>(p + mdelta);
    const unsigned long long* b = bits + ((dtot - k_left) + (kin ? k : 0)) * 4;
#pragma unroll
    for (int i = 0; i < 4; ++i) bw[J][i] = b[i];
  }
  template <int J>
  __device__ __forceinline__ void stage(const float4 (&f)[NV], char* __restrict__ S, int64_t k_left, int t) {
    const bool live = cok && kw + KPP * J < k_left;
    const int lane = t & 63;
    float mk[4];
    keep4(dseed, ((drow + KPP * J + (dtot - k_left)) * dwidth + dcol) >> 2, dthresh, dscale, mk);
    const float gv[4] = {f[J].x, f[J].y, f[J].z, f[J].w}, mv[4] = {fm[J].x, fm[J].y, fm[J].z, fm[J].w};
    float v[4];
#pragma unroll
    for (int i = 0; i < 4; ++i) {
      const float tsum = mul_rounded(gv[i], mk[i]) + mv[i];
      v[i] = (live && ((bw[J][i] >> lane) & 1ull)) ? tsum : 0.f;
      cs[i] += v[i];
    }
    uint2 pl[3];
    split4(v, pl);
#pragma unroll
    for (int p = 0; p < 3; ++p) *reinterpret_cast<uint2*>(S + p * PLANE + woff + J * (KPP * ROWB)) = pl[p];
  }
  static __device__ __forceinline__ uint32_t frag_addr(int c0, int lane) {
    const int L = lane & 15, k = 8 * (lane >> 5) + (L >> 2);
    return k * ROWB + ((((c0 >> 5) ^ swz(k)) & (NC - 1)) << 6) + (((lane >> 4) & 1) << 5) + ((L & 3) << 3);
  }
  static __device__ __forceinline__ bf16x8 frag(const char* __restrict__ S, uint32_t addr, int plane) {
    const char* q = S + plane * PLANE + addr;
    const s16x4 lo = __builtin_amdgcn_ds_read_tr16_b64_v4i16((lds_s16x4*)(q));
    const s16x4 hi = __builtin_amdgcn_ds_read_tr16_b64_v4i16((lds_s16x4*)(q + 4 * ROWB));
    typedef short s16x8 __attribute__((ext_vector_type(8)));
    const s16x8 v = __builtin_shufflevector(lo, hi, 0, 1, 2, 3, 4, 5, 6, 7);
    return __builtin_bit_cast(bf16x8, v);
  }
};

template <class OPA, class OPB>
struct Producer {
  OPA& oa;
  OPB& ob;
  float4 (&fa)[OPA::NV];
  float4 (&fb)[OPB::NV];
  char* dstA;
  char* dstB;
  const float* abase;
  const float* bbase;
  const float* bscale;
  int64_t lda, ldb;
  int64_t left1, left2;
  int t;
  bool do_stage = true;
  static constexpr int P = OPA::NV + OPB::NV;
  template <int PIECE>
  __device__ __forceinline__ void one() {
    if constexpr (PIECE < OPA::NV) {
      if (do_stage) oa.template stage<PIECE>(fa, dstA, left1, t);
      oa.template load<PIECE>(fa, abase, lda, left2, nullptr, t);
    } else {
      constexpr int J = PIECE - OPA::NV;
      if (do_stage) ob.template stage<J>(fb, dstB, left1, t);
      ob.template load<J>(fb, bbase, ldb, left2, bscale, t);
    }
  }
  template <int G, int NG, int... Is>
  __device__ __forceinline__ void group_impl(std::integer_sequence<int, Is...>) {
    ((Is * NG / P == G ? one<Is>() : void()), ...);
  }
  template <int G, int NG>
  __device__ __forceinline__ void group() { group_impl<G, NG>(std::make_integer_sequence<int, P>{}); }
};

template <int WTN, class OPA, class OPB, class PR>
__device__ __forceinline__ void limb_tile_step(const char* __restrict__ As, const char* __restrict__ Bs, const uint32_t (&aaddr)[2],
                                               const uint32_t (&baddr)[WTN], f32x16 (&acc)[2][WTN], PR& pr) {
  constexpr int NH = WTN / 2, NG = 6 * NH;
#define CB_MFMA4(A_, B_, H_, G_)                                                                             \
  _Pragma("unroll") for (int i = 0; i < 2; ++i) _Pragma("unroll") for (int j = 0; j < 2; ++j)               \
      acc[i][2 * H_ + j] = __builtin_amdgcn_mfma_f32_32x32x16_bf16(A_[i], B_[j], acc[i][2 * H_ + j], 0, 0, 0); \
  pr.template group<G_, NG>();
#define CB_HALF(H_)                                                                                                          \
  {                                                                                                                          \
    bf16x8 b_hi[2], b_mid[2], b_lo[2];                                                                                       \
    if (H_ == 0) { _Pragma("unroll") for (int i = 0; i < 2; ++i) a_lo[i] = OPA::frag(As, aaddr[i], 2); }                     \
    _Pragma("unroll") for (int j = 0; j < 2; ++j) b_hi[j] = OPB::frag(Bs, baddr[2 * H_ + j], 0);                             \
    if (H_ == 0) { _Pragma("unroll") for (int i = 0; i < 2; ++i) a_hi[i] = OPA::frag(As, aaddr[i], 0); }                     \
    _Pragma("unroll") for (int j = 0; j < 2; ++j) b_lo[j] = OPB::frag(Bs, baddr[2 * H_ + j], 2);                             \
    if (H_ == 0) { _Pragma("unroll") for (int i = 0; i < 2; ++i) a_mid[i] = OPA::frag(As, aaddr[i], 1); }                    \
    _Pragma("unroll") for (int j = 0; j < 2; ++j) b_mid[j] = OPB::frag(Bs, baddr[2 * H_ + j], 1);                            \
    CB_MFMA4(a_lo, b_hi, H_, H_ * 6 + 0)                                                                                     \
    CB_MFMA4(a_hi, b_lo, H_, H_ * 6 + 1)                                                                                     \
    CB_MFMA4(a_mid, b_mid, H_, H_ * 6 + 2)                                                                                   \
    CB_MFMA4(a_mid, b_hi, H_, H_ * 6 + 3)                                                                                    \
// ... 72 lines not shown
```

gnn-tail-generalization_amd/csrc/cb_philox.h:

```cpp
#pragma once
#include "cb_common.h"

namespace cb {

__device__ __forceinline__ void philox4x32_10(uint32_t c0, uint32_t c1, uint32_t k0, uint32_t k1, uint32_t (&out)[4]) {
  uint32_t c2 = 0x243F6A88u, c3 = 0x85A308D3u;
#pragma unroll
  for (int r = 0; r < 10; ++r) {
    const uint64_t p0 = (uint64_t)0xD2511F53u * (uint64_t)c0, p1 = (uint64_t)0xCD9E8D57u * (uint64_t)c2;
    const uint32_t hi0 = (uint32_t)(p0 >> 32), lo0 = (uint32_t)p0;
    const uint32_t hi1 = (uint32_t)(p1 >> 32), lo1 = (uint32_t)p1;
    const uint32_t n0 = hi1 ^ c1 ^ k0, n1 = lo1, n2 = hi0 ^ c3 ^ k1, n3 = lo0;
    c0 = n0; c1 = n1; c2 = n2; c3 = n3;
    k0 += 0x9E3779B9u;
    k1 += 0xBB67AE85u;
  }
  out[0] = c0; out[1] = c1; out[2] = c2; out[3] = c3;
}

__device__ __forceinline__ void keep4(uint64_t seed, int64_t quad, uint32_t thresh, float scale, float (&m)[4]) {
  uint32_t r[4];
  philox4x32_10((uint32_t)quad, (uint32_t)((uint64_t)quad >> 32), (uint32_t)seed, (uint32_t)(seed >> 32), r);
#pragma unroll
  for (int i = 0; i < 4; ++i) m[i] = (r[i] >= thresh) ? scale : 0.f;
}

static inline uint32_t dropout_threshold(float p) {
  const double t = (double)p * 4294967296.0;
  return t >= 4294967295.0 ? 0xFFFFFFFFu : (uint32_t)t;
}

}
```

gnn-tail-generalization_amd/gemm.py:

```python
import torch

from . import _lib


def _rowmajor(t):
    if t.dim() != 2:
        raise ValueError('expected a matrix')
    if t.shape[1] > 1 and t.stride(1) != 1:
        t = t.contiguous()
    elif t.shape[0] > 1 and t.stride(0) < t.shape[1]:
        t = t.contiguous()
    return t


def _ld(t):
    return t.stride(0) if t.shape[0] > 1 else max(t.shape[1], 1)


def _b_workspace(lib, N, K, M, device):
    wsb = lib.cb_gemm_nn_splitk_workspace_bytes(M, N, K) if K >= 512 else 0
    return (torch.empty(wsb, dtype=torch.uint8, device=device), wsb) if wsb else (None, 0)


def mm_nn(a, b, rowscale=None, addend=None, bias=None, relu=False, out_bf16=False, out=None):
# ... 33 lines not shown
        return None
    out = torch.empty((M, N), dtype=torch.float32, device=a.device)
    if not lib.cb_gemm_nn_store_rows_supported(_lib.ptr(a), _ld(a), _lib.ptr(b), _ld(b), _lib.ptr(out), _ld(out), M, N, K):
        return None
    if addend is not None:
        addend = _rowmajor(addend)
    act = torch.empty_like(out) if want_act else None
    with torch.cuda.device(a.device):
        _lib.check(lib.cb_gemm_nn_store_rows_f32(_lib.ptr(a), _ld(a), _lib.ptr(b), _ld(b), _lib.ptr(out), _ld(out), M, N, K, _lib.ptr(rowscale), _lib.ptr(addend),
                                                 _ld(addend) if addend is not None else 0, _lib.ptr(bias), _lib.ptr(row_index),
                                                 ops.store_args(mix, mix_index, c_act, c_mix, p, seed, row0, bits, relu_only, act), None, 0,
                                                 _lib.stream_ptr()), 'cb_gemm_nn_store_rows_f32')
    return out, act


def mm_nn_drop2(a, b, p, seed, row0=0, bias=None, relu=False):
    import ctypes
    from . import ops
    lib = _lib.load()
    _lib.require_device(a, b, bias)
    a, b = _rowmajor(a), _rowmajor(b)
    M, K = a.shape
    K2, N = b.shape
    if K != K2 or a.dtype != torch.float32 or b.dtype != torch.float32:
        raise ValueError(f'mm_nn_drop2: bad operands {tuple(a.shape)} @ {tuple(b.shape)}')
    y = torch.empty((M, N), dtype=torch.float32, device=a.device)
    yd = torch.empty((M, N), dtype=torch.float32, device=a.device)
    ws, wsb = _b_workspace(lib, N, K, M, a.device)
    with torch.cuda.device(a.device):
        _lib.check(lib.cb_gemm_nn_drop2_f32(_lib.ptr(a), _ld(a), _lib.ptr(b), _ld(b), _lib.ptr(y), N, _lib.ptr(yd), N, M, N, K, None, None, 0,
                                            _lib.ptr(bias), int(bool(relu)), float(p), ctypes.c_uint64(seed), ops.seed_dev_ptr(), int(row0),
                                            _lib.ptr(ws), wsb, _lib.stream_ptr()), 'cb_gemm_nn_drop2_f32')
    return y, yd


def mm_nn_indrop_drop2(a, b, p, a_seed, seed, row0=0, bias=None, relu=False, want_bits=False):
    import ctypes
    from . import ops
    lib = _lib.load()
    _lib.require_device(a, b, bias)
    a, b = _rowmajor(a), _rowmajor(b)
    M, K = a.shape
    K2, N = b.shape
    if K != K2 or a.dtype != torch.float32 or b.dtype != torch.float32 or not (0.0 < p < 1.0):
        return None
    y = torch.empty((M, N), dtype=torch.float32, device=a.device)
    yd = torch.empty((M, N), dtype=torch.float32, device=a.device)
    if not lib.cb_gemm_nn_indrop_supported(_lib.ptr(a), _ld(a), _lib.ptr(b), _ld(b), _lib.ptr(y), N, _lib.ptr(yd), N, M, N, K):
        return None
    bits = torch.empty((M, 1, 4), dtype=torch.int64, device=a.device) if (want_bits and N == 256 and relu) else None
    with torch.cuda.device(a.device):
        _lib.check(lib.cb_gemm_nn_indrop_drop2_f32(_lib.ptr(a), _ld(a), _lib.ptr(b), _ld(b), _lib.ptr(y), N, _lib.ptr(yd), N, M, N, K, _lib.ptr(bias),
                                                   int(bool(relu)), float(p), ctypes.c_uint64(a_seed), float(p), ctypes.c_uint64(seed),
                                                   ops.seed_dev_ptr(), int(row0), _lib.ptr(bits), _lib.stream_ptr()), 'cb_gemm_nn_indrop_drop2_f32')
    return (y, yd, bits) if want_bits else (y, yd)


def mm_nn_indrop(a, b, p, a_seed, row0=0, rowscale=None, addend=None, bias=None, relu=False, want_bits=False, out=None):
    import ctypes
    from . import ops
    lib = _lib.load()
    _lib.require_device(a, b, rowscale, addend, bias, out)
    a, b = _rowmajor(a), _rowmajor(b)
    M, K = a.shape
    K2, N = b.shape
    if K != K2 or a.dtype != torch.float32 or b.dtype != torch.float32 or not (0.0 < p < 1.0):
        return None
    if addend is not None:
        addend = _rowmajor(addend)
        if addend.data_ptr() % 16 or _ld(addend) % 4:
            return None
    y = out if out is not None else torch.empty((M, N), dtype=torch.float32, device=a.device)
    if not lib.cb_gemm_nn_indrop_supported(_lib.ptr(a), _ld(a), _lib.ptr(b), _ld(b), _lib.ptr(y), _ld(y), _lib.ptr(y), _ld(y), M, N, K):
        return None
    bits = torch.empty((M, 1, 4), dtype=torch.int64, device=a.device) if (want_bits and N == 256 and relu) else None
    with torch.cuda.device(a.device):
        _lib.check(lib.cb_gemm_nn_indrop_f32(_lib.ptr(a), _ld(a), _lib.ptr(b), _ld(b), _lib.ptr(y), _ld(y), M, N, K, _lib.ptr(rowscale), _lib.ptr(addend),
                                             _ld(addend) if addend is not None else 0, _lib.ptr(bias), int(bool(relu)), float(p),
                                             ctypes.c_uint64(a_seed), ops.seed_dev_ptr(), int(row0), _lib.ptr(bits), _lib.stream_ptr()),
                   'cb_gemm_nn_indrop_f32')
    return (y, bits) if want_bits else y


def trunk_front(x, w_in, b_in, w0, rowscale, addend, p, seed_x, seed_x0, row0=0, want_bits=False, want_drop=False, z_out=None):
    import ctypes
    from . import ops
    lib = _lib.load()
    _lib.require_device(x, w_in, b_in, w0, rowscale, addend)
    if x.dim() != 2 or x.dtype != torch.float32 or tuple(w_in.shape) != (256, x.shape[1]) or tuple(w0.shape) != (256, 256):
        return None
    M, K = x.shape
    nb_in = lib.cb_front_image_bytes(K)
    if not nb_in or w_in.dtype != torch.float32 or w0.dtype != torch.float32:
        return None
    x, w_in, w0 = _rowmajor(x), _rowmajor(w_in), _rowmajor(w0)
    if addend is not None:
        addend = _rowmajor(addend)
    if x.data_ptr() % 16 or _ld(x) % 4 or (addend is not None and (addend.data_ptr() % 16 or _ld(addend) % 4)):
        return None
    dev = x.device
    img_in = torch.empty(nb_in, dtype=torch.uint8, device=dev)
    nb0 = lib.cb_agg_gemm_image_bytes(256, 256)
    img0 = torch.empty(nb0, dtype=torch.uint8, device=dev)
    x0 = torch.empty((M, 256), dtype=torch.float32, device=dev)
    z0 = z_out if z_out is not None else torch.empty((M, 256), dtype=torch.float32, device=dev)
    bits = torch.empty((M, 1, 4), dtype=torch.int64, device=dev) if want_bits else None
    xd = torch.empty((M, 256), dtype=torch.float32, device=dev) if want_drop else None
    with torch.cuda.device(dev):
        _lib.check(lib.cb_front_image_f32(_lib.ptr(w_in), _ld(w_in), K, 1, _lib.ptr(img_in), nb_in, _lib.stream_ptr()), 'cb_front_image_f32')
        _lib.check(lib.cb_agg_gemm_image_f32(_lib.ptr(w0), _ld(w0), 256, 256, 0, _lib.ptr(img0), nb0, _lib.stream_ptr()), 'cb_agg_gemm_image_f32')
        _lib.check(lib.cb_trunk_front_f32(_lib.ptr(x), _ld(x), M, K, _lib.ptr(img_in), _lib.ptr(b_in), _lib.ptr(img0), _lib.ptr(rowscale),
                                          _lib.ptr(addend), _ld(addend) if addend is not None else 0, _lib.ptr(x0), 256, _lib.ptr(bits),
                                          _lib.ptr(xd), 256, _lib.ptr(z0), 256, float(p), ctypes.c_uint64(seed_x), ctypes.c_uint64(seed_x0),
                                          ops.seed_dev_ptr(), int(row0), _lib.stream_ptr()), 'cb_trunk_front_f32')
    return x0, bits, xd, z0


def mm_tn_adrop(a, g, p, a_seed, row0=0, rowscale=None):
    import ctypes
    from . import ops
    lib = _lib.load()
    _lib.require_device(a, g, rowscale)
    a, g = _rowmajor(a), _rowmajor(g)
    M, K1 = a.shape
    M2, K2 = g.shape
    if M != M2 or not (0.0 < p < 1.0) or not lib.cb_gemm_tn_adrop_supported(_lib.ptr(a), _ld(a), _lib.ptr(g), _ld(g), K1, K2):
        return None
    out = torch.empty((K1, K2), dtype=torch.float32, device=a.device)
    wsb = lib.cb_gemm_tn_workspace_bytes(M, K1, K2)
    ws = torch.empty(max(wsb, 16), dtype=torch.uint8, device=a.device)
    with torch.cuda.device(a.device):
        _lib.check(lib.cb_gemm_tn_adrop_f32(_lib.ptr(a), _ld(a), _lib.ptr(g), _ld(g), _lib.ptr(rowscale), _lib.ptr(out), M, K1, K2, float(p),
                                            ctypes.c_uint64(a_seed), ops.seed_dev_ptr(), int(row0), _lib.ptr(ws), wsb, _lib.stream_ptr()),
                   'cb_gemm_tn_adrop_f32')
    return out


def mm_tn_gdrop(a, g, p, g_seed, row0=0):
    import ctypes
    from . import ops
    lib = _lib.load()
    _lib.require_device(a, g)
    a, g = _rowmajor(a), _rowmajor(g)
    M, K1 = a.shape
    M2, K2 = g.shape
    if M != M2 or not (0.0 < p < 1.0) or not lib.cb_gemm_tn_gdrop_supported(_lib.ptr(a), _ld(a), _lib.ptr(g), _ld(g), K1, K2):
        return None
    out = torch.empty((K1, K2), dtype=torch.float32, device=a.device)
    wsb = lib.cb_gemm_tn_workspace_bytes(M, K1, K2)
    ws = torch.empty(max(wsb, 16), dtype=torch.uint8, device=a.device)
    with torch.cuda.device(a.device):
        _lib.check(lib.cb_gemm_tn_gdrop_f32(_lib.ptr(a), _ld(a), _lib.ptr(g), _ld(g), _lib.ptr(out), M, K1, K2, float(p), ctypes.c_uint64(g_seed),
                                            ops.seed_dev_ptr(), int(row0), _lib.ptr(ws), wsb, _lib.stream_ptr()), 'cb_gemm_tn_gdrop_f32')
    return out


def mm_tn_instage_supported(g_like, x, M):
    lib = _lib.load()
    return (g_like.dim() == 2 and g_like.shape[1] == 256 and g_like.is_contiguous() and x.dim() == 2 and x.stride(1) == 1
            and bool(lib.cb_gemm_tn_instage_supported(_lib.ptr(g_like), _lib.ptr(g_like), _lib.ptr(x), _ld(x), int(M), int(x.shape[1]))))


def mm_tn_instage(g, mfold, x0_bits, x, p_g, g_seed, p_x, x_seed, row0=0):
    import ctypes
    from . import ops
    lib = _lib.load()
    _lib.require_device(g, mfold, x0_bits, x)
    M, K2 = x.shape
    if (tuple(g.shape) != (M, 256) or tuple(mfold.shape) != (M, 256) or not g.is_contiguous() or not mfold.is_contiguous() or x0_bits.numel() != 4 * M
            or not x0_bits.is_contiguous() or x0_bits.dtype != torch.int64):
        raise ValueError('mm_tn_instage: contiguous [M, 256] gradients, [M, 1, 4] int64 mask words and [M, F] features expected')
    out = torch.empty((256, K2), dtype=torch.float32, device=g.device)
    colsum = torch.empty(256, dtype=torch.float32, device=g.device)
    wsb = lib.cb_gemm_tn_instage_workspace_bytes(M, K2)
    ws = torch.empty(max(wsb, 16), dtype=torch.uint8, device=g.device)
    with torch.cuda.device(g.device):
        _lib.check(lib.cb_gemm_tn_instage_f32(_lib.ptr(g), _lib.ptr(mfold), _lib.ptr(x0_bits), _lib.ptr(x), _ld(x), _lib.ptr(out), _lib.ptr(colsum), M, K2,
                                              float(p_g), ctypes.c_uint64(g_seed), float(p_x), ctypes.c_uint64(x_seed), ops.seed_dev_ptr(), int(row0),
                                              _lib.ptr(ws), wsb, _lib.stream_ptr()), 'cb_gemm_tn_instage_f32')
    return out, colsum


def mm_tn(a, g, rowscale=None):
    lib = _lib.load()
    _lib.require_device(a, g, rowscale)
    a, g = _rowmajor(a), _rowmajor(g)
    M, K1 = a.shape
    M2, K2 = g.shape
    if M != M2:
        raise ValueError(f'shape mismatch: {tuple(a.shape)}^T @ {tuple(g.shape)}')
    out = torch.empty((K1, K2), dtype=torch.float32, device=a.device)
    wsb = lib.cb_gemm_tn_workspace_bytes(M, K1, K2)
    ws = torch.empty(max(wsb, 16), dtype=torch.uint8, device=a.device)
    with torch.cuda.device(a.device):
        _lib.check(lib.cb_gemm_tn_f32(_lib.ptr(a), _ld(a), _lib.ptr(g), _ld(g), _lib.ptr(rowscale), _lib.ptr(out), M, K1, K2,
                                      _lib.ptr(ws), wsb, _lib.stream_ptr()), 'cb_gemm_tn_f32')
    return out


class _LinearRowscaleFn(torch.autograd.Function):

    @staticmethod
    def forward(ctx, x, w, rowscale, addend):
        ctx.save_for_backward(x, w, rowscale)
        ctx.has_addend = addend is not None
        return mm_nn(x, w, rowscale=rowscale, addend=addend)

    @staticmethod
    def backward(ctx, g):
        x, w, rowscale = ctx.saved_tensors
        g = _rowmajor(g)
        dx = mm_nn(g, w.t().contiguous(), rowscale=rowscale) if ctx.needs_input_grad[0] else None
        dw = mm_tn(x, g, rowscale=rowscale) if ctx.needs_input_grad[1] else None
        de = g if (ctx.has_addend and ctx.needs_input_grad[3]) else None
        return dx, dw, None, de


def linear_rowscale(x, w, rowscale=None, addend=None):
    return _LinearRowscaleFn.apply(x, w, rowscale, addend)


class _LinearFn(torch.autograd.Function):

    @staticmethod
    def forward(ctx, x, weight, bias, relu):
        y = mm_nn(x, weight.t().contiguous(), bias=bias, relu=relu)
        ctx.relu, ctx.has_bias = relu, bias is not None
        ctx.save_for_backward(x, weight, y if relu else None)
        return y

    @staticmethod
    def backward(ctx, g):
        from .ops import act_bwd
        x, weight, y = ctx.saved_tensors
        need_b = ctx.has_bias and ctx.needs_input_grad[2]
        g = _rowmajor(g)
        if ctx.relu or need_b:
            gm, db = act_bwd(g, y if ctx.relu else None, None, want_out=ctx.relu, want_colsum=need_b)
            if gm is None:
                gm = g
        else:
            gm, db = g, None
        dx = mm_nn(gm, weight) if ctx.needs_input_grad[0] else None
        dw = mm_tn(gm, x) if ctx.needs_input_grad[1] else None
        return dx, dw, db, None


def linear(x, weight, bias=None, relu=False):
    _lib.require_device(x, weight)
    return _LinearFn.apply(x, weight, bias, bool(relu))
```

gnn-tail-generalization_amd/trunk.py:

```python
import ctypes
import os
from typing import NamedTuple

import torch

from . import _lib, gemm, ops
from .graph import head_image, prof_rec, weight_image
from .tuning import T


def _switch(name, default):
    return os.environ.get(name, default)


TrunkCfg = NamedTuple('TrunkCfg', [('L', int), ('alpha', float), ('p', float), ('seeds', tuple), ('agg_bf16', bool), ('track', bool), ('loss_rows', object),
                                   ('residual', bool), ('rows_only', bool)])
TrunkCfg.__doc__ = """What one call of the trunk was asked for (second argument of _TrunkFn.apply).  L: number of GCNConv layers; alpha: weight of the mix
source in a layer's output (res_tricks.py); p: the one dropout rate (0 in evaluation); seeds: L + 2 dropout seeds (features, X0, one per layer); agg_bf16:
the gathered rows Z_l are stored as bf16; track: autograd was recording when the trunk was called (inside a Function's forward it never is, and
needs_input_grad does not know about no_grad); loss_rows: None or (bool mask [N], count), the caller's promise that the output receives gradient in those
rows only (ops.py); residual: the 'Residual' connection (mix source of layer l > 0 = the previous layer's ReLU output) instead of 'Initial' (X0);
rows_only: the second promise — the caller READS the output in the rows of loss_rows only (the others: ops.unread_rows_fill)."""


class RowsOnly(NamedTuple):
    plan: object = None
    below: object = None
    sharded: object = None
    sum_first_below: bool = False


class SavedRows(NamedTuple):
    x_last: str = 'all'
    x_below: str = 'all'


def _layers(layer_params):
    return [tuple(layer_params[i:i + 3]) for i in range(0, len(layer_params), 3)]


def _save(ctx, **named):
    many = {k: isinstance(v, (list, tuple)) for k, v in named.items()}
    ctx.save_for_backward(*[t for k, v in named.items() for t in (v if many[k] else [v]) if t is not None])
    ctx.saved_layout = [(k, [t is not None for t in v] if many[k] else v is not None) for k, v in named.items()]


def _saved(ctx):
    it = iter(ctx.saved_tensors)
    return {name: [next(it) if q else None for q in here] if isinstance(here, list) else (next(it) if here else None)
            for name, here in ctx.saved_layout}


def _dw_regen(x, gz, p, seed, row0, rowscale):
    dw = gemm.mm_tn_adrop(x, gz, p, seed, row0, rowscale=rowscale)
    return dw if dw is not None else gemm.mm_tn(ops._dropout_raw(x, p, seed, row0 * x.shape[1]), gz, rowscale=rowscale)


def _collect_layer_params(tc, graph):
    params, se_reg_all = [], None
    for conv in tc.layers_GCN:
        le = conv.le if conv.whetherHasSE else None
        params += [conv.weight, conv.bias, le]
        if le is not None:
            reg = ops.frobenius_norm(le)
            if hasattr(graph, 'part'):
                from .dist import allreduce_sum
                reg = allreduce_sum(reg * reg, graph.group).sqrt()
            conv.se_norm = reg.detach()
            se_reg_all = reg if se_reg_all is None else se_reg_all + reg
    if not all(c._allow_zero_in_degree for c in tc.layers_GCN):
        graph.check_zero_in_degree()
    return params, se_reg_all


def connection(tc):
    t = tc.type_trick
    return 'residual' if 'Residual' in t else 'initial' if 'Initial' in t else None


def eligible(tc, x, want_les):
    t = tc.type_trick
    return (tc.has_residual_MLP and connection(tc) is not None and 'Jumping' not in t and not want_les
            and tc.args.type_trick not in ('BatchNorm', 'PairNorm', 'NodeNorm', 'MeanNorm', 'GroupNorm', 'CombNorm')
            and tc.dim_hidden % 256 == 0 and x.is_cuda and x.dtype == torch.float32 and len(tc.layers_GCN) == tc.num_layers
            and len(tc.layers_MLP) == 2
            and tc.embedding_dropout == tc.dropout and tc.args.dropout == tc.dropout)


def _exchanged(graph, n_rows, d=256):
    if hasattr(graph, 'part'):
        from .dist import alloc_exchanged
        return alloc_exchanged(graph, n_rows, d)
    return torch.empty((n_rows, d), dtype=torch.float32, device=graph.norm_in.device)


def _fused_spmm(graph, z, bias, x0, c_act, c_mix, p, seed, want_act=False, produce=None, want_bits=True, relu_only=False):
    lib = _lib.load()
    sh = graph if hasattr(graph, 'part') else None
    if sh is not None and sh.overlap and z.dtype == torch.float32:
        flights = sh.start_halo(z, False, produce)
        return sh.finish_halo(flights, sh.f, None, lambda g, recv, a_: _fused_launch(
            lib, graph, g, recv, a_, bias, x0, c_act, c_mix, p, seed, want_act, want_bits, relu_only), x_local=z)
    if produce is not None:
        produce(0, 0, z.shape[0])
    if sh is None:
        return _fused_launch(lib, graph, graph, z, None, bias, x0, c_act, c_mix, p, seed, want_act, want_bits, relu_only)
    return _fused_launch(lib, graph, sh.f.whole, sh.exchange(z, False), None, bias, x0, c_act, c_mix, p, seed, want_act, want_bits, relu_only)


def _fused_gemm_launch(graph, z, bias, x0, c_act, c_mix, p, seed, image, g_rowscale, g_addend, want_bits=True, g=None, acc=None, want_act=False,
                       relu_only=False, head=None):
    lib = _lib.load()
    g = graph if g is None else g
    fn = lib.cb_spmm_gemm_fused_head_f32 if head is not None else lib.cb_spmm_gemm_fused_f32
    n, d = g.N, z.shape[1]
    dev = z.device
    bits = torch.empty((n, d // 256, 4), dtype=torch.int64, device=dev) if want_bits else None
    out_next = torch.empty((n, d), dtype=torch.float32, device=dev) if (want_bits or g._plan.n_hubs > 0) else None
    z_next = _exchanged(graph, n) if head is None else torch.empty((n, int(head[1])), dtype=torch.float32, device=dev)
    act = torch.empty((n, d), dtype=torch.float32, device=dev) if want_act else None
    prof = getattr(graph, 'profile', None)
    if prof is not None:
        ev0, ev1 = torch.cuda.Event(enable_timing=True), torch.cuda.Event(enable_timing=True)
        ev0.record()
    if g_addend is not None and g_addend.stride(1) != 1:
        g_addend = g_addend.contiguous()
    with torch.cuda.device(dev):
        _lib.check(fn(g._view(d, use_flags=True), _lib.ptr(acc), acc.stride(0) if acc is not None else 0,
                      _lib.ptr(z), z.stride(0), d, _lib.ptr(graph.norm_in), _lib.ptr(bias),
                      ops.store_args(x0, None, c_act, c_mix, p, seed, getattr(graph, 'row_offset', 0), bits, relu_only, act),
                      _lib.ptr(out_next), d, int(not want_bits), _lib.ptr(image),
                      *((_lib.ptr(head[0]), int(head[1])) if head is not None
                        else (_lib.ptr(g_rowscale), _lib.ptr(g_addend), g_addend.stride(0) if g_addend is not None else 0)),
                      _lib.ptr(z_next), z_next.stride(0), _lib.stream_ptr()),
                   'cb_spmm_gemm_fused_f32')
    if prof is not None:
        ev1.record()
# ... 264 lines not shown
        le_sum = fwd_le.spmm(le, row_scale=b_rows)
    fused = gemm.mm_nn_store_rows(h_agg, w, b_rows, le_sum, b, space.idx, mix, mix_index, 1 - alpha, alpha, p, seed, row0, bits, residual, want_act)
    if fused is not None:
        return bits, fused[0], fused[1], h_agg
    y = gemm.mm_nn(h_agg, w, rowscale=b_rows, addend=le_sum, bias=b)
    del le_sum
    x_next, act = _store_rows(y, space.idx, mix, 1 - alpha, alpha, p, seed, row0, bits, residual, mix_index, want_act)
    return bits, x_next, act, h_agg


def _last_layer_on_loss_rows(graph, plan, cur, w, b, mix, alpha, p, seed, row0, residual, w_out, b_out, below=None, le=None):
    sp = plan.space0
    fwd0 = graph.loss_rows_fwd(plan) if below is None else below.fwd0c
    mix_index = None
    if below is not None and residual:
        mix_index = getattr(plan, '_pos0_in_1', None)
        if mix_index is None:
            mix_index = plan._pos0_in_1 = below.s1.pos[sp.idx].long().contiguous()
    bits, x_l, _act, h_agg = _layer_on_rows(graph, sp, fwd0, graph.norm_out if below is None else below.s1.a, cur, w, b, mix, mix_index, alpha, p, seed, row0,
                                           residual, le=le, fwd_le=graph.loss_rows_fwd(plan) if le is not None else None)
    n = graph.N
    logits_c = gemm.mm_nn(x_l, w_out.t().contiguous(), bias=b_out)
    out = ops.expand_unread(logits_c, sp, n)
    graph.rows_only_forwards = getattr(graph, 'rows_only_forwards', 0) + 1
    return bits, x_l, (out, logits_c), h_agg


def _last_layer_on_loss_rows_sharded(graph, s0, orient, cur, w, b, mix, alpha, p, seed, row0, residual, w_out, b_out, le=None):
    lib = _lib.load()
    xs = _exchanged(graph, cur.shape[0], cur.shape[1])
    with torch.cuda.device(cur.device):
        _lib.check(lib.cb_act_bwd_f32(_lib.ptr(cur), None, _lib.ptr(graph.norm_out), _lib.ptr(xs), cur.shape[0], cur.shape[1], None, None, 0,
                                      _lib.stream_ptr()), 'cb_act_bwd_f32')
    h_agg = graph.aggregate_finish(graph.aggregate_start(xs, False, orient=orient), False)
    del xs
    b0 = s0.norm_in_of(graph)
    le_sum = graph.aggregate_finish(graph.aggregate_start(le, False, orient=orient), False, row_scale=b0) if le is not None else None
    y = gemm.mm_nn(h_agg, w, rowscale=b0, addend=le_sum, bias=b)
    del h_agg, le_sum
    n, d = graph.N, w.shape[1]
    bits = torch.empty((n, d // 256, 4), dtype=torch.int64, device=cur.device)
    x_l, _act = _store_rows(y, s0.idx, mix, 1 - alpha, alpha, p, seed, row0, bits, residual)
    del y
    logits_c = gemm.mm_nn(x_l, w_out.t().contiguous(), bias=b_out)
    out = ops.expand_unread(logits_c, s0, n)
    graph.rows_only_forwards += 1
    return bits, x_l, out


class _Forward:

    def __init__(self, ctx, graph, cfg, x, w_in, b_in, w_out, b_out, layer_params):
        self.graph, self.cfg, self.x = graph, cfg, x.contiguous()
        self.w_in, self.b_in, self.w_out, self.b_out = w_in, b_in, w_out, b_out
        self.layer_params, self.layers = layer_params, _layers(layer_params)
        self.row0, self.a = int(getattr(graph, 'row_offset', 0)), graph.norm_out
        self.bwd = bool(cfg.track) and any(ctx.needs_input_grad)
        self.z_ready = self.out_head = self.out_rows = self.h_last = self.h_below = None

    def run(self):
        cfg, graph = self.cfg, self.graph
        (self.xd, self.x0, self.x0_bits, self.cur, self.z_front), self.indrop = self._front()
        h = self.x0.shape[1]
        self.saved_in, self.saved_bits = [self.cur], []
        self.ag = agg_gemm_eligible(graph, h, cfg.agg_bf16)
        self.ro = _rows_only_decision(graph, cfg, self.x, self.x0, h, self.ag, self.bwd, self.layer_params)
        self.mix, self.kw = self.x0, dict(want_bits=self.bwd, relu_only=cfg.residual)
        for l in range(cfg.L):
            self.st = (self.layers[l][1], self.mix, 1 - cfg.alpha, cfg.alpha, cfg.p, cfg.seeds[l + 2] if cfg.p > 0 else 0)
            self.keep_act = cfg.residual and l + 1 < cfg.L
            z0 = self._z0() if l == 0 else None
            bits, self.cur, act = self._form(l, z0 is not None)(l, z0)
            del z0
            if cfg.residual:
                self.mix = act
            if self.bwd:
                self.saved_bits.append(bits)
                self.saved_in.append(self.cur)
        self.mix = None
        return self.out_head if self.out_head is not None else gemm.mm_nn(self.cur, self.w_out.t().contiguous(), bias=self.b_out)

    def _front(self):
        c, x, w_in, b_in, row0, bwd, p, seeds = self.cfg, self.x, self.w_in, self.b_in, self.row0, self.bwd, self.cfg.p, self.cfg.seeds
        indrop = p > 0 and _switch('CB_TRUNK_INDROP', '1') != '0'
        copy = _switch('CB_TRUNK_X0_COPY', '1') == '1'
        if (indrop or p == 0) and not c.agg_bf16 and c.L >= 1 and w_in.shape[0] == 256 and _switch('CB_TRUNK_FRONT', '1') != '0':
            w0, _b0, le0 = self.layers[0]
            fr = gemm.trunk_front(x, w_in, b_in, w0, self.a, le0, p, seeds[0], seeds[1], row0, want_bits=bwd, want_drop=bwd and p > 0 and copy,
                                  z_out=_exchanged(self.graph, x.shape[0]) if hasattr(self.graph, 'part') else None)
            if fr is not None:
                x0, x0_bits, cur, z_front = fr
                return (x, x0, x0_bits, x0 if p == 0 else cur, z_front), True
        if indrop:
            wb = bwd and w_in.shape[0] == 256
            r = None if copy else gemm.mm_nn_indrop(x, w_in.t().contiguous(), p, seeds[0], row0, bias=b_in, relu=True, want_bits=wb)
            if r is not None:
                return (x, *(r if wb else (r, None)), None, None), True
            r = gemm.mm_nn_indrop_drop2(x, w_in.t().contiguous(), p, seeds[0], seeds[1], row0, bias=b_in, relu=True, want_bits=wb)
            if r is not None:
                return (x, r[0], r[2] if len(r) > 2 else None, r[1], None), True
        xd = ops._dropout_raw(x, p, seeds[0], row0 * x.shape[1]) if p > 0 else x
        if p > 0:
            x0, cur = gemm.mm_nn_drop2(xd, w_in.t().contiguous(), p, seeds[1], row0, bias=b_in, relu=True)
        else:
            x0 = cur = gemm.mm_nn(xd, w_in.t().contiguous(), bias=b_in, relu=True)
        return (xd, x0, None, cur, None), False

    def dropped_x0(self):
        return ops._dropout_raw(self.x0, self.cfg.p, self.cfg.seeds[1], self.row0 * self.x0.shape[1])

    def _z0(self):
        z0, self.z_front = self.z_front, None
        if z0 is not None or self.cur is not None:
            return z0
        c, (w, _b, le) = self.cfg, self.layers[0]
        if not (c.agg_bf16 or (not self.ag and _chunked(self.graph, c.agg_bf16))):
            z0 = gemm.mm_nn_indrop(self.x0, w, c.p, c.seeds[1], self.row0, rowscale=self.a, addend=le, out=_exchanged(self.graph, self.x0.shape[0], w.shape[1]))
        if z0 is None:
            self.cur = self.saved_in[0] = self.dropped_x0()
        return z0

    def _form(self, l, have_z0):
        L, ro = self.cfg.L, self.ro
        if self.ag and ro.sum_first_below and l == L - 2:
            return self._form_sum_first_below
        if self.ag and ro.sharded is not None and l == L - 1:
            return self._form_last_on_loss_rows_sharded
        if ro.plan is not None and l == L - 1:
            return self._form_last_on_loss_rows
        if self.ag:
            if ro.sum_first_below and l + 3 == L:
                return self._form_store
            if ro.plan is not None and l + 2 == L and ro.below is not None:
                return self._form_store_on_s1
            if (ro.plan is not None or ro.sharded is not None) and l + 2 == L:
                return self._form_store
            return self._form_store_gemm if l + 1 < L else self._form_store_head
        if not have_z0 and _chunked(self.graph, self.cfg.agg_bf16):
            return self._form_chunked
        return self._form_store

    def _z(self, l, z0):
        z, self.z_ready = self.z_ready, None
        if z is None and z0 is None:
            (w, _b, le), bf = self.layers[l], self.cfg.agg_bf16
            return gemm.mm_nn(self.cur, w, rowscale=self.a, addend=le, out_bf16=bf, out=None if bf else _exchanged(self.graph, self.cur.shape[0], w.shape[1]))
        return z if z is not None else z0

    def _form_sum_first_below(self, l, z0):
        c, below, (w, b, _le) = self.cfg, self.ro.below, self.layers[l]
        bits, cur, act, self.h_below = _layer_on_rows(self.graph, below.s1, below.fwd1, self.a, self.cur, w, b, self.mix, None, c.alpha, c.p,
                                                      self.st[5], self.row0, c.residual, want_act=self.keep_act)
        self.saved_in[l] = None
        return bits, cur, act

    def _form_last_on_loss_rows_sharded(self, l, z0):
        c, (s0, orient), (w, b, le) = self.cfg, self.ro.sharded, self.layers[l]
        bits, cur, self.out_head = _last_layer_on_loss_rows_sharded(self.graph, s0, orient, self.cur, w, b, self.mix, c.alpha, c.p, self.st[5],
                                                                    self.row0, c.residual, self.w_out, self.b_out, le=le)
        return bits, cur, None

    def _form_last_on_loss_rows(self, l, z0):
        c, (w, b, le) = self.cfg, self.layers[l]
        bits, cur, (self.out_head, self.out_rows), self.h_last = _last_layer_on_loss_rows(
            self.graph, self.ro.plan, self.cur, w, b, self.mix, c.alpha, c.p, self.st[5], self.row0, c.residual, self.w_out, self.b_out,
            below=self.ro.below, le=le)
        if le is None:
            self.saved_in[l] = None
        else:
            self.h_last = None
        return bits, cur, None

    def _form_store(self, l, z0):
        return _fused_spmm(self.graph, self._z(l, z0), *self.st, want_act=self.keep_act, **self.kw)

    def _form_store_on_s1(self, l, z0):
        below, z = self.ro.below, self._z(l, z0)
        below.fwd1.profile = getattr(self.graph, 'profile', None)
        return _fused_launch(_lib.load(), self.graph, below.fwd1, z, None, *self.st, self.keep_act, row_ids=below.ids1, row_scale=below.b1, **self.kw)

    def _form_store_gemm(self, l, z0):
        w1, _, le1 = self.layers[l + 1]
        res = _fused_gemm(self.graph, self._z(l, z0), *self.st, weight_image(w1), self.a, le1, want_act=self.keep_act, **self.kw)
        self.z_ready = res[2]
        return res[0], res[1], res[3] if self.keep_act else None

    def _form_store_head(self, l, z0):
        z = self._z(l, z0)
        himg = head_image(self.w_out) if head_tail_enabled(self.bwd) else None
        if himg is None:
            return _fused_spmm(self.graph, z, *self.st, **self.kw)
        bits, cur, self.out_head = _fused_gemm(self.graph, z, *self.st, himg, None, None, head=(self.b_out, self.w_out.shape[0]), **self.kw)[:3]
        return bits, cur, None

    def _form_chunked(self, l, z0):
        (w, _b, le), cur, a = self.layers[l], self.cur, self.a
        z = _exchanged(self.graph, cur.shape[0], w.shape[1])

        def produce(k, r0, r1):
            if r1 > r0:
                gemm.mm_nn(cur[r0:r1], w, rowscale=a[r0:r1], addend=le[r0:r1] if le is not None else None, out=z[r0:r1])
        return _fused_spmm(self.graph, z, *self.st, want_act=self.keep_act, produce=produce, **self.kw)


class _TrunkFn(torch.autograd.Function):
    @staticmethod
    def forward(ctx, graph, cfg, x, w_in, b_in, w_out, b_out, *layer_params):
        f = _Forward(ctx, graph, cfg, x, w_in, b_in, w_out, b_out, layer_params)
        out = f.run()
        ctx.graph, ctx.cfg, ctx.row0, ctx.indrop, ctx.n_layer_params = graph, cfg, f.row0, f.indrop, len(layer_params)
        if f.bwd:
            _save(ctx, xd=f.xd, x0=f.x0, w_in=w_in, w_out=w_out, saved_in=f.saved_in, saved_bits=f.saved_bits, layer_params=layer_params,
                  h_last=f.h_last, h_below=f.h_below, x0_bits=f.x0_bits)
            ro = f.ro
            ctx.saved_rows = SavedRows('S0' if (ro.plan is not None or ro.sharded is not None) else 'all',
                                       'absent' if f.h_last is not None else 'S1' if (ro.plan is not None and ro.below is not None) else 'all')
        ctx.set_materialize_grads(False)
        return out, f.out_rows

    @staticmethod
    def backward(ctx, gout, gout_rows=None):
        if gout is None and gout_rows is None:
            return (None,) * (7 + ctx.n_layer_params)
        return _Backward(ctx, gout, gout_rows).run()


class _Carry:
    __slots__ = ('g', 'gr', 'dbias', 'handle', 'space', 'g_above', 'deferred')

    def __init__(self, g, gr, dbias, handle, space):
        self.g, self.gr, self.dbias, self.handle, self.space, self.g_above, self.deferred = g, gr, dbias, handle, space, None, None


class _Backward:

    def __init__(self, ctx, gout, gout_rows=None):
        self.gout_rows = gemm._rowmajor(gout_rows) if gout_rows is not None else None
        self.ctx, graph, c = ctx, ctx.graph, ctx.cfg
        self.graph, self.row0, self.L, self.alpha, self.p, self.seeds = graph, ctx.row0, c.L, c.alpha, c.p, c.seeds
        self.agg_bf16, self.residual = c.agg_bf16, c.residual
        sv = _saved(ctx)
        self.xd, self.x0, self.w_in, self.w_out = sv['xd'], sv['x0'], sv['w_in'], sv['w_out']
        self.saved_in, self.saved_bits, self.x0_bits = sv['saved_in'], sv['saved_bits'], sv['x0_bits']
        self.h_last, self.h_below = sv['h_last'], sv['h_below']
        self.lp, self.where = _layers(sv['layer_params']), ctx.saved_rows
        self.a, self.bnorm = graph.norm_out, graph.norm_in
        self.need = ctx.needs_input_grad
        self.gout = gemm._rowmajor(gout) if gout is not None else None
        self.n_rows, self.h = self.x0.shape
        self.sharded, loss_rows = hasattr(graph, 'part'), c.loss_rows
        if loss_rows is not None and self.where.x_last != 'S0' and (not ops.loss_rows_enabled() or loss_rows[0].shape[0] != self.x0.shape[0]):
            loss_rows = None
        self.loss_rows = loss_rows
        self.gather = _gather(graph, c.L, c.residual, self.x0)
        self.gx0 = None if self.gather else torch.empty_like(self.x0)
        self.g_mix, self.seeds_mix, self.mix_pos = [], [], []
        self.cs = []
        self.grads_layers = [None] * (3 * c.L)
        self.ag = agg_gemm_eligible(graph, self.h, c.agg_bf16)
        self.chunked = (self.gather and _chunked(graph, c.agg_bf16) and graph.b.plan.n_slices > 1 and not self.ag)
        self.fold_ok = (_switch('CB_INSTAGE_FOLD', '1') != '0' and self.gather and not c.residual and not c.agg_bf16 and c.p > 0
                        and ctx.indrop and self.need[3] and not self.need[2] and self.x0_bits is not None and self.h == 256
                        and gemm.mm_tn_instage_supported(self.x0, self.xd, self.x0.shape[0]))
        self.mfold, self.plan_taken = None, False

    def seed(self, i):
        return self.seeds[i] if self.p > 0 else 0

    def need_w(self, l):
        return self.need[7 + 3 * l]

    def need_b(self, l):
        return self.need[7 + 3 * l + 1]

    def need_le(self, l):
        return self.lp[l][2] is not None and self.need[7 + 3 * l + 2]

    def _dw(self, l, x_in, gz):
        if x_in is not None:
            return gemm.mm_tn(x_in, gz, rowscale=self.a)
        return _dw_regen(self.x0, gz, self.p, self.seed(1), self.row0, self.a)

    def _second(self, below, g_above, pos_above=None):
        if not self.residual or g_above is None:
            return {}
        return dict(g2=g_above, seed2=self.seed(below + 3), c2=self.alpha, **({'g2_pos': pos_above} if pos_above is not None else {}))

    def _dx_and_store_bwd(self, src, wt, rowscale, below, g_ready=None, g_above=None, orient=None, pos_above=None):
        p, alpha, row0, bnorm = self.p, self.alpha, self.row0, self.bnorm
        sd, want_b, bits = self.seed(below + 2), self.need_b(below), self.saved_bits[below]
        if self.chunked:
            g_ = torch.empty((src.shape[0], wt.shape[1]), dtype=torch.float32, device=src.device)
            gr_ = _exchanged(self.graph, g_.shape[0], g_.shape[1])
            colsums = []
            sec = self._second(below, g_above, pos_above)

            def produce(k, r0, r1):
                if r1 <= r0:
                    return
                gemm.mm_nn(src[r0:r1], wt, rowscale=rowscale[r0:r1] if rowscale is not None else None, out=g_[r0:r1])
                sec_k = dict(sec, g2=sec['g2'][r0:r1]) if sec else {}
                _, cs = _layer_bwd(g_[r0:r1], bits[r0:r1], bnorm[r0:r1], None, False, p, sd, row0 + r0, 1 - alpha, alpha, want_b, out=gr_[r0:r1], **sec_k)
                if want_b:
                    colsums.append(cs)
            h_ = self.graph.aggregate_start(gr_, True, produce=produce, orient=orient)
            db_ = None
            if want_b:
                db_ = (torch.zeros(wt.shape[1], dtype=torch.float32, device=src.device) if not colsums
                       else colsums[0] if len(colsums) == 1 else torch.stack(colsums).sum(0))
            return g_, gr_, db_, h_
        g_ = g_ready if g_ready is not None else gemm.mm_nn(src, wt, rowscale=rowscale)
        cs_ = self.cs
        if (below == 0 and self.fold_ok and self.mfold is None and self.plan_taken and len(self.g_mix) <= 2 and len(cs_) <= 1
                and all(t.is_contiguous() for t in self.g_mix) and g_.is_contiguous()):
            res = _layer_bwd_fold(g_, bits, bnorm, p, sd, row0, 1 - alpha, alpha, want_b, self.g_mix, self.mix_pos, self.seeds_mix,
                                  out=_exchanged(self.graph, g_.shape[0], g_.shape[1]) if self.sharded else None, cs=cs_[0][:3] if cs_ else None)
            gr_, db_, self.mfold = res[:3]
            if cs_:
                self.grads_layers[3 * cs_[0][3] + 1] = res[3]
                self.cs = []
            self.g_mix, self.mix_pos, self.seeds_mix = [], [], []
            return None, gr_, db_, None
        gr_, db_ = _layer_bwd(g_, bits, bnorm, self.gx0, below != self.L - 1, p, sd, row0, 1 - alpha, alpha, want_b, out_bf16=self.agg_bf16,
                              out=_exchanged(self.graph, g_.shape[0], g_.shape[1]) if (self.sharded and not self.agg_bf16) else None,
                              **self._second(below, g_above, pos_above))
        return g_, gr_, db_, None

    def _head(self, space):
        L, need, gout, xl = self.L, self.need, self.gout, self.saved_in[self.L]
        if space is not None:
            gout = ops.gather_rows_by_index(gout, space.idx) if gout is not None else None
            if self.gout_rows is not None:
                gout = self.gout_rows if gout is None else gout + self.gout_rows
            xl = xl if self.where.x_last == 'S0' else ops.gather_rows_by_index(xl, space.idx)
        self.d_w_out = gemm.mm_tn(gout, xl) if need[5] else None
        self.d_b_out = ops.act_bwd(gout, None, None, want_out=False, want_colsum=True)[1] if need[6] else None
        if space is None:
            return _Carry(*self._dx_and_store_bwd(gout, self.w_out, None, L - 1, orient=self._orient_of(L - 1)), None)
        g = gemm.mm_nn(gout, self.w_out)
        gr, dbias = _layer_bwd_rows(g, space.idx, self.saved_bits[L - 1], self.bnorm, self.p, self.seed(L + 1), self.row0, 1 - self.alpha,
                                    self.need_b(L - 1), out=_exchanged(self.graph, g.shape[0], g.shape[1]) if self.sharded else None)
        return _Carry(g, gr, dbias, None, space)

    def _sh_level(self, layer):
        j = self.L - 1 - layer
        return self.sh_levels[j] if 0 <= j < len(self.sh_levels) else None

    def _orient_of(self, layer):
        return getattr(self._sh_level(layer), 'orient', None)

    def _dw_rows(self, l, x_in, gz, dst):
        if dst is None:
            return self._dw(l, x_in, gz)
        return gemm.mm_tn(ops.gather_rows_by_index(x_in, dst.idx), gz, rowscale=dst.a)

    def _layer_source_side(self, l, gr, level, fwd_j):
        w = self.lp[l][0]
        dst = level[1]
        level[0].profile = getattr(self.graph, 'profile', None)
        if fwd_j is not None:
            fwd_j.profile = level[0].profile
        t = gemm.mm_nn(gr, w.t().contiguous())
        fused = None
        if (l > 0 and not self.residual and self.gather and len(self.cs) < 2 and dst is None
# ... 65 lines not shown
                               'CB_LOSS_ROWS / tuning.T / the mask changed between the forward and the backward')
        space0 = plan.space0 if plan is not None else (self.sh_levels[0].src if self.sh_levels else None)
        if xl_compact and space0 is None:
            raise RuntimeError('the forward evaluated its last layer on the loss rows (rows_only), but its backward has no compact level 0')
        return plan, space0

    def _layer(self, l, c, plan):
        L, graph, sharded = self.L, self.graph, self.sharded
        j = L - 1 - l
        level = plan.levels[j] if (plan is not None and j < len(plan.levels)) else None
        lv = self._sh_level(l)
        dst = level[1] if level is not None else lv.dst if lv is not None else None
        if sharded and c.handle is None:
            c.handle = graph.aggregate_start(c.gr, True, orient=self._orient_of(l))
        if c.deferred is not None:
            self.grads_layers[3 * c.deferred[0]] = self._dw_rows(*c.deferred)
            c.deferred = None
        fwd_j = plan.fwd[j] if (level is not None and j < len(plan.fwd)) else None
        source_side = ((self.where.x_below == 'absent' and l == L - 1) or (self.h_below is not None and l == L - 2)
                       or (T.rowsparse_loss_side and fwd_j is not None and not self.need_le(l)
                           and not (self.need_w(l) and self.saved_in[l] is None)
                           and not (self.where.x_below == 'S1' and l == L - 1)))
        if source_side:
            _gz, g_new, fused = self._layer_source_side(l, c.gr, level, fwd_j)
            return None, g_new, dst, fused
        if level is not None:
            return (*self._layer_compact(l, c.gr, level), dst, None)
        gz, g_new = self._layer_fused(l, c.gr, c.handle, dst) if self.ag else (self._layer_plain(c.gr, c.handle), None)
        if self.need_w(l):
            if sharded:
                c.deferred = (l, self.saved_in[l], gz, dst if self.ag else None)
            else:
                self.grads_layers[3 * l] = self._dw(l, self.saved_in[l], gz)
        return gz, g_new, dst, None

    def _store_bwd_below(self, l, c, gz, g_new, dst, fused, pos_above):
        w = self.lp[l][0]
        if l > 0 and fused is not None:
            c.g, (c.gr, _below), c.dbias = g_new, fused, None
            if self.mfold is not None:
                c.dbias = self.grads_layers[3 * (l - 1) + 1]
            elif self.need_b(l - 1):
                self.cs = self.cs + [(len(self.g_mix), self.saved_bits[l - 1], 1 - self.alpha, l - 1)]
        elif l > 0 and dst is not None:
            c.g = g_new
            c.gr, c.dbias = _layer_bwd_rows(g_new, dst.idx, self.saved_bits[l - 1], self.bnorm, self.p, self.seed(l + 1), self.row0, 1 - self.alpha,
                                            self.need_b(l - 1), out=_exchanged(self.graph, g_new.shape[0], g_new.shape[1]) if self.sharded else None,
                                            **self._second(l - 1, c.g_above, pos_above))
        elif l > 0:
            c.g, c.gr, c.dbias, c.handle = self._dx_and_store_bwd(gz, w.t().contiguous(), self.a, l - 1, g_new, c.g_above, orient=self._orient_of(l - 1),
                                                                  pos_above=pos_above)
        else:
            c.g = g_new if g_new is not None else gemm.mm_nn(gz, w.t().contiguous(), rowscale=self.a)

    def run(self):
        plan, space0 = self._resolve_plan()
        c = self._head(space0)
        for l in range(self.L - 1, -1, -1):
            if self.gather and (not self.residual or l == 0) and self.mfold is None:
                self.g_mix.append(c.g)
                self.mix_pos.append(c.space.pos if c.space is not None else None)
                self.seeds_mix.append(self.seed(l + 2))
            gz, g_new, dst, fused = self._layer(l, c, plan)
            c.g_above = c.g if self.residual else None
            pos_above = c.space.pos if (self.residual and c.space is not None) else None
            c.g = c.gr = c.handle = None
            self.grads_layers[3 * l + 1] = c.dbias
            c.space = dst
            self._store_bwd_below(l, c, gz, g_new, dst, fused, pos_above)
            c.g_above = None
            if self.need_le(l):
                if dst is not None:
                    gz = ops.expand_rows(gz, dst.pos)
                self.grads_layers[3 * l + 2] = gz
            del gz, g_new
        if c.deferred is not None:
            self.grads_layers[3 * c.deferred[0]] = self._dw_rows(*c.deferred)
        return self._input_stage(c)

    def _input_stage(self, c):
        graph, p, need, xd, row0 = self.graph, self.p, self.need, self.xd, self.row0
        g, c.g = c.g, None
        if self.mfold is not None:
            d_w_in, d_b_in = gemm.mm_tn_instage(g, self.mfold, self.x0_bits, xd, p, self.seed(1), p, self.seeds[0], row0)
            del g
            self.gx0 = self.g_mix = self.mfold = None
            graph.instage_folds = getattr(graph, 'instage_folds', 0) + 1
            return (None, None, None, d_w_in, d_b_in if need[4] else None, self.d_w_out, self.d_b_out, *self.grads_layers)
        if self.gather:
            res = _input_bwd_multi(g, self.seed(1), self.g_mix, self.seeds_mix, self.alpha, self.x0, p, row0, act_bits=self.x0_bits,
                                   mix_pos=self.mix_pos, cs=[q[:3] for q in self.cs])
            gpre, d_b_in = res[0], res[1]
            for q, db in zip(self.cs, res[2] if self.cs else []):
                self.grads_layers[3 * q[3] + 1] = db
        else:
            gpre, d_b_in = _input_bwd(g, self.gx0, self.x0, p, self.seed(1), row0)
        del g
        self.gx0 = self.g_mix = None
        d_w_in = None
        if need[3]:
            if self.ctx.indrop and p > 0:
                d_w_in = gemm.mm_tn_gdrop(gpre, xd, p, self.seeds[0], row0)
                if d_w_in is None:
                    d_w_in = gemm.mm_tn(gpre, ops._dropout_raw(xd, p, self.seeds[0], row0 * xd.shape[1]))
            else:
                d_w_in = gemm.mm_tn(gpre, xd)
        d_x = None
        if need[2]:
            d_x = gemm.mm_nn(gpre, self.w_in)
            if p > 0:
                d_x = ops._dropout_raw(d_x, p, self.seeds[0], row0 * d_x.shape[1])
        return (None, None, d_x, d_w_in, d_b_in if need[4] else None, self.d_w_out, self.d_b_out, *self.grads_layers)


def forward(tc, x, graph, loss_rows=None, rows_only=False):
    L = tc.num_layers
    p = float(tc.dropout) if tc.training else 0.0
    seeds = tuple(ops.next_seed() for _ in range(L + 2)) if p > 0 else (0,) * (L + 2)
    params, se_reg_all = _collect_layer_params(tc, graph)
    agg_bf16 = getattr(tc.args, 'agg_dtype', 'f32') == 'bf16'
    if loss_rows is not None:
        mask, count = loss_rows if isinstance(loss_rows, (tuple, list)) else (loss_rows, None)
        if count is None:
            count = int(mask.sum().item())
        if mask.dtype != torch.bool or mask.dim() != 1 or mask.shape[0] != x.shape[0]:
            raise ValueError(f'loss_rows: a bool mask over the {x.shape[0]} rows expected, got {tuple(mask.shape)} {mask.dtype}')
        loss_rows = (mask, int(count))
    cfg = TrunkCfg(L, float(tc.alpha), p, seeds, agg_bf16, torch.is_grad_enabled(), loss_rows, connection(tc) == 'residual',
                   bool(rows_only) and loss_rows is not None)
    out, out_rows = _TrunkFn.apply(graph, cfg, x, tc.layers_MLP[0].weight, tc.layers_MLP[0].bias, tc.layers_MLP[1].weight, tc.layers_MLP[1].bias, *params)
    if out_rows is not None:
        out._cb_rows = (out_rows, loss_rows[0])
    return out, se_reg_all
```

include/coldbrew_hip.h:

```cpp
#ifndef COLDBREW_HIP_H
#define COLDBREW_HIP_H

#include <stddef.h>
#include <stdint.h>

#ifdef __cplusplus
extern "C" {
#endif

#define CB_OK 0
#define CB_E_INVALID (-1)
#define CB_E_RANGE (-2)
#define CB_E_WORKSPACE (-3)
#define CB_E_HIP (-4)
#define CB_E_DEVICE (-5)

#define CB_DEVERR_HANDOVER 1
#define CB_DEVERR_GRADROWS 2

int cb_version(void);
const char* cb_last_error(void);
int cb_device_status(void);

int cb_rows_zero_outside_mask_f32(const float* g, int64_t ld, int64_t rows, int64_t d, const uint8_t* mask, int32_t* guard, void* stream);
// ... 90 lines not shown
                                const int32_t* const* mix_pos, const uint64_t* mix_seeds, float* out_m, float* colsum, void* ws, size_t ws_bytes, int32_t cs_src,
                                const uint64_t* cs_bits, float cs_c, float* colsum2, void* ws2, size_t ws2_bytes, void* stream);
int cb_trunk_layer_bwd_rows_f32(const float* g, const int64_t* row_index, int64_t n_rows, const uint64_t* relu_bits, const float* row_scale, float* out,
                                int64_t d, float drop_p, uint64_t seed, const uint64_t* seed_dev, int64_t row0, float c_act, const float* g2, uint64_t seed2,
                                float c2, const int32_t* g2_pos, float* colsum, void* ws, size_t ws_bytes, void* stream);

int cb_trunk_input_bwd_f32(const float* g, const float* add, const float* act, float* out, int64_t rows, int64_t d, float drop_p,
                           uint64_t seed, const uint64_t* seed_dev, int64_t row0, float* colsum, void* ws, size_t ws_bytes,
                           void* stream);

int cb_trunk_input_bwd_multi_f32(const float* g, uint64_t seed, int32_t n_mix, const float* const* g_mix, const uint64_t* seeds_mix,
                                 float c_mix, const float* act, float* out, int64_t rows, int64_t d, float drop_p,
                                 const uint64_t* seed_dev, int64_t row0, float* colsum, void* ws, size_t ws_bytes,
                                 const uint64_t* act_bits, const int32_t* const* g_mix_pos, void* stream);
int cb_trunk_input_bwd_multi_cs_f32(const float* g, uint64_t seed, int32_t n_mix, const float* const* g_mix, const uint64_t* seeds_mix,
                                    float c_mix, const float* act, float* out, int64_t rows, int64_t d, float drop_p,
                                    const uint64_t* seed_dev, int64_t row0, float* colsum, void* ws, size_t ws_bytes,
                                    const uint64_t* act_bits, const int32_t* const* g_mix_pos, int32_t n_cs, const int32_t* cs_src,
                                    const uint64_t* const* cs_bits, const float* cs_c, float* const* colsum2, void* ws2, size_t ws2_bytes, void* stream);
int cb_spmm_csr_store_bwd_f32(const cb_csr_view* g, const float* h, int64_t ld_h, int64_t d, const float* row_scale, const uint64_t* relu_bits,
                              const float* bwd_rowscale, float c_act, float drop_p, uint64_t seed, const uint64_t* seed_dev, int64_t row0,
                              float* out_g, int64_t ld_g, float* out_gr, int64_t ld_gr, void* stream);
size_t cb_spmm_store_bwd_mix_workspace_bytes(int64_t N, int64_t n_hubs, int64_t d);
int cb_spmm_csr_store_bwd_mix_f32(const cb_csr_view* g, const float* h, int64_t ld_h, int64_t d, const float* row_scale, const uint64_t* relu_bits,
                                  const float* bwd_rowscale, float c_act, float drop_p, uint64_t seed, const uint64_t* seed_dev, int64_t row0,
                                  float* out_m, int64_t ld_m, float* out_gr, int64_t ld_gr, int32_t n_mix, const float* const* mix_g,
                                  const int32_t* const* mix_pos, const uint64_t* mix_seeds, float c_mix, float* colsum, void* ws2, size_t ws2_bytes,
                                  void* stream);

int cb_gemm_nn_bf16out_f32(const float* A, int64_t lda, const float* B, int64_t ldb, uint16_t* C, int64_t ldc, int64_t M, int64_t N,
                           int64_t K, const float* rowscale, const float* addend, int64_t ld_add, const float* bias, int relu,
                           void* ws, size_t ws_bytes, void* stream);

int cb_node_norm_fwd_f32(const float* x, float* y, float* stats2, int64_t rows, int64_t d, float c, float q, float eps, void* stream);
int cb_node_norm_bwd_f32(const float* x, const float* g, const float* stats2, float* dx, int64_t rows, int64_t d, float c, float q,
                         void* stream);
size_t cb_colstats_workspace_bytes(int64_t rows, int64_t d);
int cb_colstats_f32(const float* x, const float* w, const float* shift, int64_t rows, int64_t d, float* colsum, float* colsum2,
                    void* ws, size_t ws_bytes, void* stream);
int cb_col_affine_f32(const float* x, const float* shift, const float* scale, const float* bias, float gscale, float* y, int64_t rows,
                      int64_t d, void* stream);
int cb_col_bwd_combine_f32(const float* g, const float* xh, const float* xs, const float* a, const float* b, const float* e, float ga,
                           float gb, float* dx, int64_t rows, int64_t d, void* stream);

size_t cb_topk_replace_workspace_bytes(int64_t B, int64_t N, int64_t K);
int cb_topk_replace_f32(const float* q, int64_t ldq, const float* t, int64_t ldt, int64_t B, int64_t N, int64_t D, int32_t K,
                        float* out, int32_t* out_idx, float* out_w, void* ws, size_t ws_bytes, void* stream);

int cb_id_count_i64(const int64_t* ids, int64_t E, int64_t N, int32_t* counts, int32_t* n_bad, void* stream);
int cb_value_hist_i32(const int32_t* vals, int64_t N, int32_t n_bins, int32_t* hist, int32_t* n_bad, void* stream);
size_t cb_compact_workspace_bytes(int64_t n);
int cb_select_range_i32(const int32_t* vals, int64_t N, int32_t lo, int32_t hi, int64_t* out_idx, uint8_t* out_mask, int64_t* count,
                        void* ws, size_t ws_bytes, void* stream);
int cb_craft_isolation_i64(const int64_t* src, const int64_t* dst, int64_t E, const uint8_t* node_flag, int64_t N, int64_t* out_src,
                           int64_t* out_dst, int64_t* count, void* ws, size_t ws_bytes, void* stream);
size_t cb_symmetrize_workspace_bytes(int64_t E, int64_t N);
int cb_symmetrize_i64(const int64_t* src, const int64_t* dst, int64_t E, int64_t N, int64_t* out_row, int64_t* out_col, int64_t* count,
                      int32_t* n_bad, void* ws, size_t ws_bytes, void* stream);

int cb_gather_rows_f32(const float* src, int64_t ld, const int64_t* idx, int64_t n_idx, int64_t d, float* out, void* stream);

size_t cb_agg_gemm_image_bytes(int64_t K, int64_t N);
int cb_agg_gemm_image_f32(const float* W, int64_t ld, int64_t K, int64_t N, int transpose, void* image, size_t image_bytes, void* stream);
int cb_spmm_gemm_f32(const cb_csr_view* g, const float* h, int64_t ld_h, int64_t d, const float* row_scale, const float* bias, int relu,
                     const float* acc_init, int64_t ld_init, float* out, int64_t ld_out, const void* image, const float* g_rowscale,
                     const float* g_addend, int64_t ld_add, float* g_out, int64_t ld_gout, void* stream);
int cb_spmm_gemm_fused_f32(const cb_csr_view* g, const float* acc_init, int64_t ld_init, const float* h, int64_t ld_h, int64_t d,
                           const float* row_scale, const float* bias, const cb_trunk_store* store, float* out_next, int64_t ld_next,
                           int32_t skip_next, const void* image, const float* g_rowscale, const float* g_addend, int64_t ld_add, float* g_out,
                           int64_t ld_gout, void* stream);
size_t cb_agg_gemm_head_image_bytes(int64_t K, int64_t C);
int cb_agg_gemm_head_image_f32(const float* W, int64_t ld, int64_t K, int64_t C, int transpose, void* image, size_t image_bytes, void* stream);
int cb_spmm_gemm_fused_head_f32(const cb_csr_view* g, const float* acc_init, int64_t ld_init, const float* h, int64_t ld_h, int64_t d,
                                const float* row_scale, const float* bias, const cb_trunk_store* store, float* out_next, int64_t ld_next,
                                int32_t skip_next, const void* head_image, const float* head_bias, int64_t C, float* logits, int64_t ld_logits,
                                void* stream);
int cb_agg_gemm_handover_selftest(void* stream);

size_t cb_front_image_bytes(int64_t K);
int cb_front_image_f32(const float* W, int64_t ld, int64_t K, int transpose, void* image, size_t image_bytes, void* stream);
int cb_trunk_front_f32(const float* x, int64_t ld_x, int64_t M, int64_t K, const void* image_in, const float* bias_in, const void* image_0,
                       const float* rowscale, const float* addend, int64_t ld_add, float* x0, int64_t ld_x0, uint64_t* relu_bits, float* x0_drop,
                       int64_t ld_drop, float* z0, int64_t ld_z, float drop_p, uint64_t seed_x, uint64_t seed_x0, const uint64_t* seed_dev,
                       int64_t row0, void* stream);

int cb_spmm_csr_weighted_f32(const int32_t* rowptr, const int32_t* col, const float* w, int64_t N, int64_t E, const float* h, int64_t ld_h,
                             int64_t d, const float* row_scale, const float* bias, int relu, float* out, int64_t ld_out, void* stream);
int cb_spmm_edge_dot_f32(const int32_t* rowptr, const int32_t* col, int64_t N, int64_t E, const float* h, int64_t ld_h, const float* g,
                         int64_t ld_g, int64_t d, float* dw, void* stream);

int cb_gemm_nn_indrop_supported(const float* A, int64_t lda, const float* B, int64_t ldb, const float* C, int64_t ldc, const float* C2, int64_t ldc2,
                                int64_t M, int64_t N, int64_t K);
int cb_gemm_nn_indrop_drop2_f32(const float* A, int64_t lda, const float* B, int64_t ldb, float* C, int64_t ldc, float* C2, int64_t ldc2,
                                int64_t M, int64_t N, int64_t K, const float* bias, int relu, float a_drop_p, uint64_t a_seed, float drop_p,
                                uint64_t seed, const uint64_t* seed_dev, int64_t row0, uint64_t* relu_bits, void* stream);
int cb_gemm_nn_indrop_f32(const float* A, int64_t lda, const float* B, int64_t ldb, float* C, int64_t ldc, int64_t M, int64_t N, int64_t K,
                          const float* rowscale, const float* addend, int64_t ld_add, const float* bias, int relu, float a_drop_p, uint64_t a_seed,
                          const uint64_t* seed_dev, int64_t row0, uint64_t* relu_bits, void* stream);
int cb_gemm_tn_adrop_supported(const float* A, int64_t lda, const float* G, int64_t ldg, int64_t K1, int64_t K2);
int cb_gemm_tn_adrop_f32(const float* A, int64_t lda, const float* G, int64_t ldg, const float* rowscale, float* C, int64_t M, int64_t K1, int64_t K2,
                         float a_drop_p, uint64_t a_seed, const uint64_t* seed_dev, int64_t row0, void* ws, size_t ws_bytes, void* stream);
int cb_gemm_tn_gdrop_supported(const float* A, int64_t lda, const float* G, int64_t ldg, int64_t K1, int64_t K2);
int cb_gemm_tn_gdrop_f32(const float* A, int64_t lda, const float* G, int64_t ldg, float* C, int64_t M, int64_t K1, int64_t K2, float g_drop_p,
                         uint64_t g_seed, const uint64_t* seed_dev, int64_t row0, void* ws, size_t ws_bytes, void* stream);
int cb_gemm_tn_instage_supported(const float* g, const float* mfold, const float* X, int64_t ldx, int64_t M, int64_t K2);
size_t cb_gemm_tn_instage_workspace_bytes(int64_t M, int64_t K2);
int cb_gemm_tn_instage_f32(const float* g, const float* mfold, const uint64_t* x0_bits, const float* X, int64_t ldx, float* C, float* colsum, int64_t M, int64_t K2,
                           float g_drop_p, uint64_t g_seed, float x_drop_p, uint64_t x_seed, const uint64_t* seed_dev, int64_t row0, void* ws, size_t ws_bytes,
                           void* stream);

int cb_spmm_gemm_store_rows_f32(const cb_csr_view* g, const float* h, int64_t ld_h, int64_t d, const float* col_scale, float* out, int64_t ld_out,
                                const void* image, const float* g_rowscale, const float* bias, const int64_t* row_ids, const cb_trunk_store* store,
                                float* g_out, int64_t ld_gout, void* stream);

int cb_spmm_csr_lp_f32(const cb_csr_view* g, const float* h, int64_t ld_h, int64_t d, const float* row_scale, const float* mix, int64_t ld_mix,
                       float c_mix, const float* post_scale, float* out, int64_t ld_out, void* stream);

int cb_spmm_csr_prop_f32(const cb_csr_view* g, const float* h, int64_t ld_h, int64_t d, const float* row_scale, const float* mix, int64_t ld_mix,
                         float c_mix, float lo, float hi, const uint8_t* fix_rows, const float* post_scale, float* out, int64_t ld_out,
                         void* stream);

size_t cb_cs_workspace_bytes(int64_t N, int64_t Cp);
int cb_cs_residual_init_f32(const float* P, int64_t ld_p, const int64_t* labels, const uint8_t* label_rows, int64_t N, int64_t C, int64_t Cp,
                            const float* state_scale, float* E0, float* state, float* abs_sum, void* ws, size_t ws_bytes, void* stream);
int cb_cs_correct_snap_f32(int32_t mode, const float* P, int64_t ld_p, const float* resid, int64_t ld_r, const int64_t* labels,
                           const uint8_t* label_rows, int64_t N, int64_t C, int64_t Cp, const float* abs_sum, int64_t n_label, float scale,
                           const float* state_scale, float* res_result, int64_t ld_res, float* y2, float* state, void* stream);

int cb_gather_rows_bf16_f32(const float* src, int64_t ld, const int64_t* idx, int64_t n_idx, int64_t d, uint16_t* out, void* stream);
int cb_expand_rows_f32(const float* src, const int32_t* pos, int64_t n_rows, int64_t d, float fill, float* out, void* stream);
int cb_trunk_store_rows_f32(const float* y, const int64_t* row_index, int64_t n_rows, int64_t d, const cb_trunk_store* store, float* out, void* stream);
int cb_gemm_nn_store_rows_supported(const float* A, int64_t lda, const float* B, int64_t ldb, const float* C, int64_t ldc, int64_t M, int64_t N, int64_t K);
int cb_gemm_nn_store_rows_f32(const float* A, int64_t lda, const float* B, int64_t ldb, float* C, int64_t ldc, int64_t M, int64_t N, int64_t K,
                              const float* rowscale, const float* addend, int64_t ld_add, const float* bias, const int64_t* row_index,
                              const cb_trunk_store* store, void* ws, size_t ws_bytes, void* stream);


int cb_ln_gelu_drop_fwd_f32(const float* z, int64_t rows, int64_t d, const float* gamma, const float* beta, float eps, float p,
                            uint64_t seed, const uint64_t* seed_dev, float* out, float* stats, void* stream);
size_t cb_ln_gelu_drop_bwd_workspace_bytes(int64_t rows, int64_t d);
int cb_ln_gelu_drop_bwd_f32(const float* dy, const float* z, const float* stats, int64_t rows, int64_t d, const float* gamma,
                            const float* beta, float p, uint64_t seed, const uint64_t* seed_dev, float* dz, float* dgamma,
                            float* dbeta, float* dbias, void* ws, size_t ws_bytes, void* stream);

int cb_mse_rows_f32(const float* pred, int64_t B, int64_t D, const float* target, int64_t ld_t, int64_t n_target_rows,
                    const int64_t* row_index, float* loss, float* grad, void* ws, size_t ws_bytes, void* stream);

int cb_part2_assemble_f32(const float* x, int64_t F, const float* replaced, const float* part1_out, int64_t D, const float* alphas,
                          int64_t B, float* out, void* stream);
int cb_part2_assemble_bwd_f32(const float* g, int64_t F, const float* replaced, const float* part1_out, int64_t D, int64_t B,
                              float* dalphas, void* ws, size_t ws_bytes, void* stream);


int cb_ncloss_positions_i64(const int64_t* batch_idx, int64_t B, int64_t n, int32_t* pos, int32_t* rep, void* stream);

int cb_ncloss_row_norms_f32(const float* x, int64_t ldx, int64_t rows, int64_t D, float* nrm, float* rinv, void* stream);

int cb_cosine_scale_f32(float* s, int64_t ld, int64_t N, const float* nrm, void* stream);

int cb_ncloss_uses_limb_core(const float* z, int64_t ldz, int64_t D);

size_t cb_ncloss_workspace_bytes(int64_t B, int32_t max_splits);
int cb_ncloss_fwd_f32(const float* z, int64_t ldz, int64_t B, int64_t D, float tau, const int32_t* rowptr, const int32_t* col,
                      const float* val, int64_t n, const int64_t* batch_idx, const int32_t* pos, const int32_t* rep, int32_t max_splits,
                      float* rinv, float* num, float* den, float* w, float* u, float* loss, int32_t* m_count, void* ws, size_t ws_bytes,
                      void* stream);

int cb_ncloss_normalize_rows_f32(const float* z, int64_t ldz, int64_t B, int64_t D, const float* rinv, float* zhat, void* stream);
int cb_ncloss_bwd_slab_f32(const float* z, int64_t ldz, int64_t B, int64_t D, float tau, const float* rinv, const float* w, int64_t row0,
                           int64_t rows, int32_t max_splits, float* P, int64_t ldp, void* stream);
int cb_ncloss_bwd_finish_f32(const float* z, int64_t ldz, const float* zhat, int64_t B, int64_t D, float tau, const float* rinv, const float* u,
                             const int32_t* rowptr, const int32_t* col, const float* val, const int32_t* rowptr_t, const int32_t* col_t,
                             const float* val_t, int64_t n, const int64_t* batch_idx, const int32_t* pos, const int32_t* rep, const float* g,
                             float* dzh, float* dz, void* stream);


size_t cb_spgemm_offsets_workspace_bytes(int64_t nnz_a);
int cb_spgemm_entry_offsets_i64(const int32_t* col_a, int64_t nnz_a, const int32_t* rowptr_b, int64_t k, int64_t* ent_off, int32_t* n_bad,
                                void* ws, size_t ws_bytes, void* stream);

size_t cb_spgemm_chunk_workspace_bytes(int64_t n_products);
int cb_spgemm_chunk_count_f32(const int32_t* rowptr_a, const int32_t* col_a, const float* val_a, const int32_t* rowptr_b, const int32_t* col_b,
                              const float* val_b, const int64_t* ent_off, int64_t row0, int64_t row1, int64_t k, int64_t n_cols,
                              int64_t n_products, int64_t* count, void* ws, size_t ws_bytes, void* stream);

int cb_spgemm_chunk_emit_f32(const void* ws, size_t ws_bytes, int64_t row0, int64_t row1, int64_t n_cols, int64_t n_products, int64_t count,
                             int64_t nnz_base, int32_t* rowptr, int32_t* col_out, float* val_out, void* stream);

size_t cb_csr_transpose_workspace_bytes(int64_t nnz);
int cb_csr_transpose_f32(const int32_t* rowptr, const int32_t* col, const float* val, int64_t m, int64_t n, int64_t nnz, int32_t* rowptr_t,
                         int32_t* col_t, float* val_t, void* ws, size_t ws_bytes, void* stream);

// ... 69 lines not shown
```

Before: 9.161.

## Store dropout keep-bit words in forward front kernel and reuse them in backward

The fused front kernel now records the dropout keep masks for the input features and the first hidden activation as packed bit words. The backward input-stage weight-gradient kernel and the adrop TN GEMM read these words instead of regenerating the masks from the hash-based RNG. This removes repeated per-element RNG work in the backward pass. In exchange the forward pass does extra global writes and the step keeps a small bitmask buffer alive.

Result: no change. 9.232 (median of 6 runs) (+0.8%).

```diff
diff --git a/gnn-tail-generalization_amd/_lib.py b/gnn-tail-generalization_amd/_lib.py
--- a/gnn-tail-generalization_amd/_lib.py
+++ b/gnn-tail-generalization_amd/_lib.py
@@ -100,11 +100,11 @@
     'cb_gemm_nn_indrop_f32': (ctypes.c_int, [_P, _I64, _P, _I64, _P, _I64, _I64, _I64, _I64, _P, _P, _I64, _P, ctypes.c_int, ctypes.c_float,
                                              ctypes.c_uint64, _P, _I64, _P, _P]),
     'cb_gemm_tn_adrop_supported': (ctypes.c_int, [_P, _I64, _P, _I64, _I64, _I64]),
-    'cb_gemm_tn_adrop_f32': (ctypes.c_int, [_P, _I64, _P, _I64, _P, _P, _I64, _I64, _I64, ctypes.c_float, ctypes.c_uint64, _P, _I64, _P, _SZ, _P]),
+    'cb_gemm_tn_adrop_f32': (ctypes.c_int, [_P, _I64, _P, _I64, _P, _P, _I64, _I64, _I64, ctypes.c_float, ctypes.c_uint64, _P, _I64, _P, _SZ, _P, _P]),
     'cb_front_image_bytes': (_SZ, [_I64]),
     'cb_front_image_f32': (ctypes.c_int, [_P, _I64, _I64, ctypes.c_int, _P, _SZ, _P]),
     'cb_trunk_front_f32': (ctypes.c_int, [_P, _I64, _I64, _I64, _P, _P, _P, _P, _P, _I64, _P, _I64, _P, _P, _I64, _P, _I64, ctypes.c_float,
-                                          ctypes.c_uint64, ctypes.c_uint64, _P, _I64, _P]),
+                                          ctypes.c_uint64, ctypes.c_uint64, _P, _I64, _P, _P, _P]),
     'cb_gemm_tn_gdrop_supported': (ctypes.c_int, [_P, _I64, _P, _I64, _I64, _I64]),
     'cb_gemm_tn_gdrop_f32': (ctypes.c_int, [_P, _I64, _P, _I64, _P, _I64, _I64, _I64, ctypes.c_float, ctypes.c_uint64, _P, _I64, _P, _SZ, _P]),
     'cb_spmm_csr_lp_f32': (ctypes.c_int, [_G, _P, _I64, _I64, _P, _P, _I64, ctypes.c_float, _P, _P, _I64, _P]),
@@ -123,7 +123,7 @@
     'cb_gemm_tn_instage_supported': (ctypes.c_int, [_P, _P, _P, _I64, _I64, _I64]),
     'cb_gemm_tn_instage_workspace_bytes': (_SZ, [_I64, _I64]),
     'cb_gemm_tn_instage_f32': (ctypes.c_int, [_P, _P, _P, _P, _I64, _P, _P, _I64, _I64, ctypes.c_float, ctypes.c_uint64, ctypes.c_float, ctypes.c_uint64, _P, _I64,
-                                              _P, _SZ, _P]),
+                                              _P, _SZ, _P, _P, _P]),
     'cb_trunk_layer_bwd_fold_f32': (ctypes.c_int, [_P, _P, _P, _P, _I64, _I64, ctypes.c_float, ctypes.c_uint64, _P, _I64, ctypes.c_float, ctypes.c_float, _I32, _P, _P, _P,
                                                    _P, _P, _P, _SZ, _I32, _P, ctypes.c_float, _P, _P, _SZ, _P]),
     'cb_trunk_layer_bwd_rows_f32': (ctypes.c_int, [_P, _P, _I64, _P, _P, _P, _I64, ctypes.c_float, ctypes.c_uint64, _P, _I64, ctypes.c_float,
diff --git a/gnn-tail-generalization_amd/csrc/cb_front.hip b/gnn-tail-generalization_amd/csrc/cb_front.hip
--- a/gnn-tail-generalization_amd/csrc/cb_front.hip
+++ b/gnn-tail-generalization_amd/csrc/cb_front.hip
@@ -29,6 +29,8 @@
   const uint64_t* seed_dev;
   int64_t row0;
   int n_tiles;
+  uint32_t* keep_x;
+  unsigned long long* keep_x0;
 };
 
 template <int NS1>
@@ -61,18 +63,22 @@
   for (int tile_id = blockIdx.x; tile_id < fa.n_tiles; tile_id += gridDim.x, par ^= 1) {
     const int64_t m0 = (int64_t)tile_id * kTM;
     load_x(tile_id);
+    uint32_t kwx = 0;
 #pragma unroll
     for (int j = 0; j < NV; ++j) {
       const int idx = t + 256 * j, row = idx / (K1 / 4), c4 = idx % (K1 / 4);
       float v[4] = {xr[j].x, xr[j].y, xr[j].z, xr[j].w};
       if (fa.thresh) {
         float mk[4];
-        keep4(sx, ((fa.row0 + m0 + row) * K1 + 4 * c4) >> 2, fa.thresh, fa.keep_scale, mk);
+        const uint32_t kb = keep4_bits(sx, ((fa.row0 + m0 + row) * K1 + 4 * c4) >> 2, fa.thresh);
+        keep4_from_bits(kb, fa.keep_scale, mk);
+        kwx |= (m0 + row < fa.M ? kb : 0u) << (4 * j);
 #pragma unroll
         for (int i = 0; i < 4; ++i) v[i] = mul_rounded(v[i], mk[i]);
       }
       *reinterpret_cast<float4*>(tile + row * LDX + 4 * c4) = make_float4(v[0], v[1], v[2], v[3]);
     }
+    if (fa.keep_x) fa.keep_x[(int64_t)tile_id * 256 + t] = kwx;
     if (t < kTM) rs_tile[par][t] = (fa.rowscale && m0 + t < fa.M) ? fa.rowscale[m0 + t] : 1.f;
     __syncthreads();
     f32x16 acc[2][2];
@@ -88,6 +94,8 @@
             tile[(32 * i + (reg & 3) + 8 * (reg >> 2) + 4 * lh) * kTLD + 64 * w + 32 * j + l31] = acc[i][j][reg];
     }
     __syncthreads();
+    unsigned long long kw0 = 0;
+    uint32_t k16 = 0;
 #pragma unroll 4
     for (int r = 0; r < 16; ++r) {
       const int row = 16 * w + r;
@@ -100,7 +108,9 @@
       float xd[4] = {o[0], o[1], o[2], o[3]};
       if (fa.thresh) {
         float mk[4];
-        keep4(s0, ((fa.row0 + m) * kND + 4 * lane) >> 2, fa.thresh, fa.keep_scale, mk);
+        const uint32_t kb = keep4_bits(s0, ((fa.row0 + m) * kND + 4 * lane) >> 2, fa.thresh);
+        keep4_from_bits(kb, fa.keep_scale, mk);
+        k16 |= (m < fa.M ? kb : 0u) << (4 * (r & 3));
 #pragma unroll
         for (int i = 0; i < 4; ++i) xd[i] = o[i] * mk[i];
       }
@@ -113,7 +123,12 @@
         }
         if (fa.x0_drop) store_stream4(fa.x0_drop + m * fa.ld_drop + 4 * lane, xd);
       }
-    }
+      if ((r & 3) == 3) {
+        kw0 |= (unsigned long long)k16 << (4 * (r - 3));
+        k16 = 0;
+      }
+    }
+    if (fa.keep_x0 && m0 + 16 * w < fa.M) fa.keep_x0[((int64_t)tile_id * 4 + w) * 64 + lane] = kw0;
     __syncthreads();
     tile_times_image_coop<kNS, kTLD, 1>(tile, scratch, fa.image_0, w, lane, t, acc);
     acc_rows_through_strip(acc, cstrip[w], w, lane, [&](int row, int n, const float4& v) {
@@ -158,12 +173,14 @@
 extern "C" int cb_trunk_front_f32(const float* x, int64_t ld_x, int64_t M, int64_t K, const void* image_in, const float* bias_in, const void* image_0,
                                   const float* rowscale, const float* addend, int64_t ld_add, float* x0, int64_t ld_x0, uint64_t* relu_bits,
                                   float* x0_drop, int64_t ld_drop, float* z0, int64_t ld_z, float drop_p, uint64_t seed_x, uint64_t seed_x0,
-                                  const uint64_t* seed_dev, int64_t row0, void* stream) {
+                                  const uint64_t* seed_dev, int64_t row0, uint32_t* keep_x, uint64_t* keep_x0, void* stream) {
   CB_CHECK_ARG(M >= 0 && cb_front_image_bytes(K) > 0 && drop_p >= 0.f && drop_p < 1.f && row0 >= 0, CB_E_INVALID,
                "cb_trunk_front_f32: bad size (K must be 64 or 128; hidden width 256) or p");
   CB_CHECK_ARG(M < ((int64_t)1 << 31) * kTM / 2, CB_E_RANGE, "cb_trunk_front_f32: size out of range");
   if (M == 0) return CB_OK;
   CB_CHECK_ARG(x && image_in && image_0 && x0 && z0, CB_E_INVALID, "cb_trunk_front_f32: null pointer");
+  CB_CHECK_ARG(!(keep_x || keep_x0) || (drop_p > 0.f && (uintptr_t)keep_x % 4 == 0 && (uintptr_t)keep_x0 % 8 == 0), CB_E_INVALID,
+               "cb_trunk_front_f32: keep words exist with dropout only (p > 0); 4- / 8-byte aligned");
   CB_CHECK_ARG(aligned16(x) && ld_x % 4 == 0 && ld_x >= K && aligned16(image_in) && aligned16(image_0) && aligned16(x0) && ld_x0 % 4 == 0 && ld_x0 >= kND &&
                    aligned16(z0) && ld_z % 4 == 0 && ld_z >= kND && (!addend || (aligned16(addend) && ld_add % 4 == 0 && ld_add >= kND)) &&
                    (!x0_drop || (aligned16(x0_drop) && ld_drop % 4 == 0 && ld_drop >= kND)) && (!relu_bits || (uintptr_t)relu_bits % 8 == 0),
@@ -174,6 +191,7 @@
   fa.keep_scale = 1.f / (1.f - drop_p);
   fa.seed_x = seed_x; fa.seed_x0 = seed_x0; fa.seed_dev = seed_dev; fa.row0 = row0;
   fa.n_tiles = (int)((M + kTM - 1) / kTM);
+  fa.keep_x = keep_x; fa.keep_x0 = (unsigned long long*)keep_x0;
   int dev = 0, n_cu = 0;
   if (hipGetDevice(&dev) != hipSuccess || hipDeviceGetAttribute(&n_cu, hipDeviceAttributeMultiprocessorCount, dev) != hipSuccess || n_cu <= 0) n_cu = 256;
   const int blocks = fa.n_tiles < 2 * n_cu ? fa.n_tiles : 2 * n_cu;
diff --git a/gnn-tail-generalization_amd/csrc/cb_gemm.hip b/gnn-tail-generalization_amd/csrc/cb_gemm.hip
--- a/gnn-tail-generalization_amd/csrc/cb_gemm.hip
+++ b/gnn-tail-generalization_amd/csrc/cb_gemm.hip
@@ -429,7 +429,7 @@
 
 extern "C" int cb_gemm_tn_instage_f32(const float* g, const float* mfold, const uint64_t* x0_bits, const float* X, int64_t ldx, float* C, float* colsum, int64_t M,
                                       int64_t K2, float g_drop_p, uint64_t g_seed, float x_drop_p, uint64_t x_seed, const uint64_t* seed_dev, int64_t row0, void* ws,
-                                      size_t ws_bytes, void* stream) {
+                                      size_t ws_bytes, const uint32_t* keep_x, const uint64_t* keep_x0, void* stream) {
   CB_CHECK_ARG(M > 0 && K2 > 0 && g_drop_p > 0.f && g_drop_p < 1.f && x_drop_p > 0.f && x_drop_p < 1.f && row0 >= 0, CB_E_INVALID,
                "cb_gemm_tn_instage_f32: bad size or p (both dropouts must be active)");
   CB_CHECK_ARG(g && mfold && x0_bits && X && C && colsum && (uintptr_t)x0_bits % 8 == 0, CB_E_INVALID, "cb_gemm_tn_instage_f32: null or misaligned pointer");
@@ -439,8 +439,10 @@
   const int nsplit = instage_splits(M);
   int64_t rows_per_split = (M + nsplit - 1) / nsplit;
   rows_per_split = (rows_per_split + 31) / 32 * 32;
-  const DropSpec xd{dropout_threshold(x_drop_p), 1.f / (1.f - x_drop_p), x_seed, seed_dev, row0, K2};
-  const DropSpec gd{dropout_threshold(g_drop_p), 1.f / (1.f - g_drop_p), g_seed, seed_dev, row0, 256};
+  CB_CHECK_ARG(!keep_x == !keep_x0 && (!keep_x || (row0 == 0 && K2 == 128 && (uintptr_t)keep_x % 4 == 0 && (uintptr_t)keep_x0 % 8 == 0)), CB_E_INVALID,
+               "cb_gemm_tn_instage_f32: keep words come as a pair, for row0 == 0 and 128 input features");
+  const DropSpec xd{dropout_threshold(x_drop_p), 1.f / (1.f - x_drop_p), x_seed, seed_dev, row0, K2, keep_x};
+  const DropSpec gd{dropout_threshold(g_drop_p), 1.f / (1.f - g_drop_p), g_seed, seed_dev, row0, 256, keep_x0};
   float* partial = (float*)ws;
   float* cs_partial = partial + (size_t)nsplit * 256 * K2;
   const int rc = launch_tn_instage(g, mfold, x0_bits, X, ldx, partial, cs_partial, M, K2, nsplit, rows_per_split, st, xd, gd);
@@ -478,7 +480,7 @@
 
 extern "C" int cb_gemm_tn_adrop_f32(const float* A, int64_t lda, const float* G, int64_t ldg, const float* rowscale, float* C, int64_t M, int64_t K1,
                                     int64_t K2, float a_drop_p, uint64_t a_seed, const uint64_t* seed_dev, int64_t row0, void* ws, size_t ws_bytes,
-                                    void* stream) {
+                                    const uint64_t* keep_x0, void* stream) {
   CB_CHECK_ARG(M >= 0 && K1 >= 0 && K2 >= 0 && a_drop_p > 0.f && a_drop_p < 1.f && row0 >= 0, CB_E_INVALID, "cb_gemm_tn_adrop_f32: bad size or p");
   CB_CHECK_ARG(K1 < (1 << 20) && K2 < (1 << 20), CB_E_RANGE, "cb_gemm_tn_adrop_f32: size out of range");
   if (K1 == 0 || K2 == 0) return CB_OK;
@@ -490,6 +492,7 @@
   }
   CB_CHECK_ARG(cb_gemm_tn_adrop_supported(A, lda, G, ldg, K1, K2), CB_E_INVALID, "cb_gemm_tn_adrop_f32: operands outside the three-limb 128-row tile path");
   CB_CHECK_ARG(ws && ws_bytes >= cb_gemm_tn_workspace_bytes(M, K1, K2), CB_E_WORKSPACE, "cb_gemm_tn_adrop_f32: workspace too small");
-  const DropSpec ad{dropout_threshold(a_drop_p), 1.f / (1.f - a_drop_p), a_seed, seed_dev, row0, K1};
+  CB_CHECK_ARG(!keep_x0 || (row0 == 0 && K1 == 256 && (uintptr_t)keep_x0 % 8 == 0), CB_E_INVALID, "cb_gemm_tn_adrop_f32: X0 keep words need row0 == 0 and K1 == 256");
+  const DropSpec ad{dropout_threshold(a_drop_p), 1.f / (1.f - a_drop_p), a_seed, seed_dev, row0, K1, keep_x0};
   return launch_tn<2, 2>(A, lda, G, ldg, rowscale, C, M, K1, K2, (float*)ws, st, nullptr, &ad);
 }
diff --git a/gnn-tail-generalization_amd/csrc/cb_gemm_core.h b/gnn-tail-generalization_amd/csrc/cb_gemm_core.h
--- a/gnn-tail-generalization_amd/csrc/cb_gemm_core.h
+++ b/gnn-tail-generalization_amd/csrc/cb_gemm_core.h
@@ -16,6 +16,7 @@
   const uint64_t* seed_dev;
   int64_t row0;
   int64_t width;
+  const void* words;
 };
 
 struct GemmEpilogue {
diff --git a/gnn-tail-generalization_amd/csrc/cb_gemm_limb.hip b/gnn-tail-generalization_amd/csrc/cb_gemm_limb.hip
--- a/gnn-tail-generalization_amd/csrc/cb_gemm_limb.hip
+++ b/gnn-tail-generalization_amd/csrc/cb_gemm_limb.hip
@@ -51,7 +51,7 @@
   nn_epilogue<WM, WN, WTN, OUT_BF16, EPI>(acc, reinterpret_cast<float*>(smem), Cv, ldc, m0, n0, M, N, ep, c_vec_ok, t);
 }
 
-template <int WM, int WN, bool SCALED, int WTN = 2, int PD = 1, bool GDROP = false, bool ADROP = false>
+template <int WM, int WN, bool SCALED, int WTN = 2, int PD = 1, bool GDROP = false, int ADROP = 0>
 __global__ void __launch_bounds__((LTile<WM, WN, WTN, PD>::NTHR), (LTile<WM, WN, WTN, PD>::MINW)) k_gemm_tn_l3(const float* __restrict__ A, int64_t lda,
                                                                                  const float* __restrict__ G, int64_t ldg,
                                                                                  const float* __restrict__ rowscale,
@@ -101,13 +101,14 @@
     }
 }
 
+template <bool WORDS>
 __global__ void __launch_bounds__(512, 2) k_gemm_tn_instage(const float* __restrict__ g, const float* __restrict__ mfold,
                                                             const unsigned long long* __restrict__ x0_bits, const float* __restrict__ X, int64_t ldx,
                                                             float* __restrict__ partial, float* __restrict__ cs_partial, int64_t M, int K2,
                                                             int64_t rows_per_split, int nsplit, DropSpec xd, DropSpec gd) {
   using T = LTile<4, 2, 2>;
-  using OA = ColOperandInStage<T::NTHR>;
-  using OB = ColOperand<T::BN, false, true, T::NTHR>;
+  using OA = ColOperandInStage<T::NTHR, WORDS>;
+  using OB = ColOperand<T::BN, false, WORDS ? 2 : 1, T::NTHR>;
   constexpr int K1 = 256;
   __shared__ __attribute__((aligned(16))) char smem[2 * (OA::BYTES + OB::BYTES)];
   const int split = blockIdx.x;
@@ -158,8 +159,14 @@
 
 int launch_tn_instage(const float* g, const float* mfold, const uint64_t* x0_bits, const float* X, int64_t ldx, float* partial, float* cs_partial, int64_t M, int64_t K2,
                       int nsplit, int64_t rows_per_split, hipStream_t st, const DropSpec& xd, const DropSpec& gd) {
-  hipLaunchKernelGGL(k_gemm_tn_instage, dim3((unsigned)nsplit), dim3(512), 0, st, g, mfold, (const unsigned long long*)x0_bits, X, ldx, partial, cs_partial, M, (int)K2,
-                     rows_per_split, nsplit, xd, gd);
+  CB_CHECK_ARG(!xd.words == !gd.words && (!xd.words || (K2 == 128 && xd.row0 == 0)), CB_E_INVALID,
+               "input-stage weight gradient: the words form needs both keep-word buffers, 128 input features and row0 == 0");
+  if (xd.words)
+    hipLaunchKernelGGL(k_gemm_tn_instage<true>, dim3((unsigned)nsplit), dim3(512), 0, st, g, mfold, (const unsigned long long*)x0_bits, X, ldx, partial, cs_partial, M,
+                       (int)K2, rows_per_split, nsplit, xd, gd);
+  else
+    hipLaunchKernelGGL(k_gemm_tn_instage<false>, dim3((unsigned)nsplit), dim3(512), 0, st, g, mfold, (const unsigned long long*)x0_bits, X, ldx, partial, cs_partial, M,
+                       (int)K2, rows_per_split, nsplit, xd, gd);
   CB_LAUNCH_CHECK();
   return CB_OK;
 }
@@ -239,7 +246,11 @@
                      (int)K2, rows_per_split, tj, ti * tj, nsplit, gd.thresh ? gd : ad)
   if (gd.thresh) CB_TN_LAUNCH(false, true, false);
   else if (ad.thresh) {
-    if constexpr (WM == 2 && WN == 2 && WTN == 2) { if (rowscale) CB_TN_LAUNCH(true, false, true); else CB_TN_LAUNCH(false, false, true); }
+    if constexpr (WM == 2 && WN == 2 && WTN == 2) {
+      if (ad.words) { if (rowscale) CB_TN_LAUNCH(true, false, 3); else CB_TN_LAUNCH(false, false, 3); }
+      else if (rowscale) CB_TN_LAUNCH(true, false, 1);
+      else CB_TN_LAUNCH(false, false, 1);
+    }
   } else if (rowscale) CB_TN_LAUNCH(true, false, false);
   else CB_TN_LAUNCH(false, false, false);
 #undef CB_TN_LAUNCH
@@ -256,6 +267,8 @@
   CB_CHECK_ARG(!gd.thresh || (!rowscale && gd.width % 4 == 0 && !ad.thresh), CB_E_INVALID,
                "TN contraction: dropout of the G operand needs width %% 4 == 0, no row scale and no dropout of A");
   CB_CHECK_ARG(!ad.thresh || (ad.width % 4 == 0 && bm == 128), CB_E_INVALID, "TN contraction: dropout of the A operand needs width %% 4 == 0 and the 128-row tile");
+  CB_CHECK_ARG(!gd.words && (!ad.words || (ad.thresh && ad.width == 256 && K1 == 256 && ad.row0 == 0)), CB_E_INVALID,
+               "TN contraction: keep words exist for the A operand only (X0 words: width 256, row0 == 0)");
   if (bm == 64) launch_tn_l3_t<1, 4>(A, lda, G, ldg, rowscale, partial, M, K1, K2, nsplit, rows_per_split, st, gd, ad);
   else if (bm == 256) launch_tn_l3_t<4, 1>(A, lda, G, ldg, rowscale, partial, M, K1, K2, nsplit, rows_per_split, st, gd, ad);
   else {
diff --git a/gnn-tail-generalization_amd/csrc/cb_limb_core.h b/gnn-tail-generalization_amd/csrc/cb_limb_core.h
--- a/gnn-tail-generalization_amd/csrc/cb_limb_core.h
+++ b/gnn-tail-generalization_amd/csrc/cb_limb_core.h
@@ -153,7 +153,7 @@
   static __device__ __forceinline__ bf16x8 frag(const char* __restrict__ S, uint32_t addr, int plane) { return RowOperand<R>::frag(S, addr, plane); }
 };
 
-template <int C, bool SCALED, bool DROP = false, int NT = 256>
+template <int C, bool SCALED, int DROP = 0, int NT = 256>
 struct ColOperand {
   static constexpr int ROWB = C * 2, PLANE = 16 * ROWB, BYTES = 3 * PLANE;
   static constexpr int TPR = C / 4, KPP = NT / TPR, NV = 16 / KPP;
@@ -171,6 +171,10 @@
   float dscale;
   int64_t drow, dtot, dwidth;
   int dcol;
+  const void* dwords;
+  int dlq;
+  uint32_t kw32[NV];
+  unsigned long long kw64[NV];
   __device__ __forceinline__ void set_drop(const DropSpec& d, int64_t r_begin, int64_t total, int j0, int t) {
     dseed = d.seed_dev ? d.seed + *d.seed_dev : d.seed;
     dthresh = d.thresh;
@@ -179,6 +183,8 @@
     dtot = total;
     dwidth = d.width;
     dcol = j0 + (t % TPR) * 4;
+    dwords = d.words;
+    dlq = d.width == 128 ? 5 : 4;
   }
   __device__ __forceinline__ void init(int64_t ld, int cols_left, int t) {
     const int k = t / TPR, nq = t % TPR;
@@ -194,6 +200,12 @@
     const bool kin = k < k_left;
     f[J] = *reinterpret_cast<const float4*>(base + (kin ? voff[J] : 0u));
     if constexpr (SCALED) sc[J] = kscale[kin ? k : 0];
+    if constexpr (DROP >= 2) {
+      const int64_t m = drow + (dtot - k_left) + (kin ? KPP * J : -(t / TPR));
+      const int q = cok ? dcol >> 2 : 0;
+      if constexpr (DROP == 2) kw32[J] = static_cast<const uint32_t*>(dwords)[keep_x_word(m, q, dlq)];
+      else kw64[J] = static_cast<const unsigned long long*>(dwords)[keep_x0_word(m, q)];
+    }
   }
   template <int J>
   __device__ __forceinline__ void stage(const float4 (&f)[NV], char* __restrict__ S, int64_t k_left, int t) const {
@@ -203,7 +215,10 @@
     if constexpr (DROP) {
       static_assert(!SCALED, "dropout of a row-scaled operand is not needed anywhere");
       float mk[4];
-      keep4(dseed, ((drow + KPP * J + (dtot - k_left)) * dwidth + dcol) >> 2, dthresh, dscale, mk);
+      const int64_t m = drow + KPP * J + (dtot - k_left);
+      if constexpr (DROP == 1) keep4(dseed, (m * dwidth + dcol) >> 2, dthresh, dscale, mk);
+      else if constexpr (DROP == 2) keep4_from_bits(kw32[J] >> keep_x_shift(m, dlq), dscale, mk);
+      else keep4_from_bits((uint32_t)(kw64[J] >> keep_x0_shift(m)), dscale, mk);
 #pragma unroll
       for (int i = 0; i < 4; ++i) v[i] = mul_rounded(v[i], mk[i]);
     }
@@ -226,7 +241,7 @@
   }
 };
 
-template <int NT = 512>
+template <int NT = 512, bool WORDS = false>
 struct ColOperandInStage {
   static constexpr int C = 256;
   static constexpr int ROWB = C * 2, PLANE = 16 * ROWB, BYTES = 3 * PLANE;
@@ -248,6 +263,8 @@
   float dscale;
   int64_t drow, dtot, dwidth;
   int dcol, kw;
+  const unsigned long long* kwords;
+  unsigned long long kq[NV];
   float cs[4];
   __device__ __forceinline__ void set_stage(const float* g, const float* mfold, const unsigned long long* bits_block, const DropSpec& d, int64_t r_begin, int64_t total,
                                             int t) {
@@ -261,6 +278,7 @@
     dtot = total;
     dwidth = d.width;
     dcol = (t % TPR) * 4;
+    kwords = static_cast<const unsigned long long*>(d.words);
 #pragma unroll
     for (int i = 0; i < 4; ++i) cs[i] = 0.f;
   }
@@ -281,13 +299,16 @@
     const unsigned long long* b = bits + ((dtot - k_left) + (kin ? k : 0)) * 4;
 #pragma unroll
     for (int i = 0; i < 4; ++i) bw[J][i] = b[i];
+    if constexpr (WORDS) kq[J] = kwords[keep_x0_word(drow + (dtot - k_left) + (kin ? KPP * J : -kw), dcol >> 2)];
   }
   template <int J>
   __device__ __forceinline__ void stage(const float4 (&f)[NV], char* __restrict__ S, int64_t k_left, int t) {
     const bool live = cok && kw + KPP * J < k_left;
     const int lane = t & 63;
     float mk[4];
-    keep4(dseed, ((drow + KPP * J + (dtot - k_left)) * dwidth + dcol) >> 2, dthresh, dscale, mk);
+    const int64_t m = drow + KPP * J + (dtot - k_left);
+    if constexpr (WORDS) keep4_from_bits((uint32_t)(kq[J] >> keep_x0_shift(m)), dscale, mk);
+    else keep4(dseed, (m * dwidth + dcol) >> 2, dthresh, dscale, mk);
     const float gv[4] = {f[J].x, f[J].y, f[J].z, f[J].w}, mv[4] = {fm[J].x, fm[J].y, fm[J].z, fm[J].w};
     float v[4];
 #pragma unroll
diff --git a/gnn-tail-generalization_amd/csrc/cb_philox.h b/gnn-tail-generalization_amd/csrc/cb_philox.h
--- a/gnn-tail-generalization_amd/csrc/cb_philox.h
+++ b/gnn-tail-generalization_amd/csrc/cb_philox.h
@@ -18,12 +18,28 @@
   out[0] = c0; out[1] = c1; out[2] = c2; out[3] = c3;
 }
 
-__device__ __forceinline__ void keep4(uint64_t seed, int64_t quad, uint32_t thresh, float scale, float (&m)[4]) {
+__device__ __forceinline__ uint32_t keep4_bits(uint64_t seed, int64_t quad, uint32_t thresh) {
   uint32_t r[4];
   philox4x32_10((uint32_t)quad, (uint32_t)((uint64_t)quad >> 32), (uint32_t)seed, (uint32_t)(seed >> 32), r);
+  uint32_t b = 0;
 #pragma unroll
-  for (int i = 0; i < 4; ++i) m[i] = (r[i] >= thresh) ? scale : 0.f;
+  for (int i = 0; i < 4; ++i) b |= (r[i] >= thresh ? 1u : 0u) << i;
+  return b;
 }
+
+__device__ __forceinline__ void keep4_from_bits(uint32_t bits, float scale, float (&m)[4]) {
+#pragma unroll
+  for (int i = 0; i < 4; ++i) m[i] = ((bits >> i) & 1u) ? scale : 0.f;
+}
+
+__device__ __forceinline__ void keep4(uint64_t seed, int64_t quad, uint32_t thresh, float scale, float (&m)[4]) {
+  keep4_from_bits(keep4_bits(seed, quad, thresh), scale, m);
+}
+
+__device__ __forceinline__ int64_t keep_x0_word(int64_t m, int q) { return (m >> 4) * 64 + q; }
+__device__ __forceinline__ int keep_x0_shift(int64_t m) { return 4 * (int)(m & 15); }
+__device__ __forceinline__ int64_t keep_x_word(int64_t m, int q, int lq) { return (m >> 6) * 256 + ((((int)m & 63) & ((256 >> lq) - 1)) << lq) + q; }
+__device__ __forceinline__ int keep_x_shift(int64_t m, int lq) { return 4 * (((int)m & 63) >> (8 - lq)); }
 
 static inline uint32_t dropout_threshold(float p) {
   const double t = (double)p * 4294967296.0;
diff --git a/gnn-tail-generalization_amd/gemm.py b/gnn-tail-generalization_amd/gemm.py
--- a/gnn-tail-generalization_amd/gemm.py
+++ b/gnn-tail-generalization_amd/gemm.py
@@ -139,7 +139,11 @@
     return (y, bits) if want_bits else y
 
 
-def trunk_front(x, w_in, b_in, w0, rowscale, addend, p, seed_x, seed_x0, row0=0, want_bits=False, want_drop=False, z_out=None):
+def keep_words_alloc(M, device):
+    return (torch.empty(((M + 63) // 64, 256), dtype=torch.int32, device=device), torch.empty(((M + 15) // 16, 64), dtype=torch.int64, device=device))
+
+
+def trunk_front(x, w_in, b_in, w0, rowscale, addend, p, seed_x, seed_x0, row0=0, want_bits=False, want_drop=False, z_out=None, want_keep=False):
     import ctypes
     from . import ops
     lib = _lib.load()
@@ -163,17 +167,18 @@
     z0 = z_out if z_out is not None else torch.empty((M, 256), dtype=torch.float32, device=dev)
     bits = torch.empty((M, 1, 4), dtype=torch.int64, device=dev) if want_bits else None
     xd = torch.empty((M, 256), dtype=torch.float32, device=dev) if want_drop else None
+    keep_x, keep_x0 = keep_words_alloc(M, dev) if want_keep and p > 0 else (None, None)
     with torch.cuda.device(dev):
         _lib.check(lib.cb_front_image_f32(_lib.ptr(w_in), _ld(w_in), K, 1, _lib.ptr(img_in), nb_in, _lib.stream_ptr()), 'cb_front_image_f32')
         _lib.check(lib.cb_agg_gemm_image_f32(_lib.ptr(w0), _ld(w0), 256, 256, 0, _lib.ptr(img0), nb0, _lib.stream_ptr()), 'cb_agg_gemm_image_f32')
         _lib.check(lib.cb_trunk_front_f32(_lib.ptr(x), _ld(x), M, K, _lib.ptr(img_in), _lib.ptr(b_in), _lib.ptr(img0), _lib.ptr(rowscale),
                                           _lib.ptr(addend), _ld(addend) if addend is not None else 0, _lib.ptr(x0), 256, _lib.ptr(bits),
                                           _lib.ptr(xd), 256, _lib.ptr(z0), 256, float(p), ctypes.c_uint64(seed_x), ctypes.c_uint64(seed_x0),
-                                          ops.seed_dev_ptr(), int(row0), _lib.stream_ptr()), 'cb_trunk_front_f32')
-    return x0, bits, xd, z0
-
-
-def mm_tn_adrop(a, g, p, a_seed, row0=0, rowscale=None):
+                                          ops.seed_dev_ptr(), int(row0), _lib.ptr(keep_x), _lib.ptr(keep_x0), _lib.stream_ptr()), 'cb_trunk_front_f32')
+    return (x0, bits, xd, z0, keep_x, keep_x0) if want_keep else (x0, bits, xd, z0)
+
+
+def mm_tn_adrop(a, g, p, a_seed, row0=0, rowscale=None, keep_x0=None):
     import ctypes
     from . import ops
     lib = _lib.load()
@@ -188,7 +193,7 @@
     ws = torch.empty(max(wsb, 16), dtype=torch.uint8, device=a.device)
     with torch.cuda.device(a.device):
         _lib.check(lib.cb_gemm_tn_adrop_f32(_lib.ptr(a), _ld(a), _lib.ptr(g), _ld(g), _lib.ptr(rowscale), _lib.ptr(out), M, K1, K2, float(p),
-                                            ctypes.c_uint64(a_seed), ops.seed_dev_ptr(), int(row0), _lib.ptr(ws), wsb, _lib.stream_ptr()),
+                                            ctypes.c_uint64(a_seed), ops.seed_dev_ptr(), int(row0), _lib.ptr(ws), wsb, _lib.ptr(keep_x0), _lib.stream_ptr()),
                    'cb_gemm_tn_adrop_f32')
     return out
 
@@ -218,7 +223,7 @@
             and bool(lib.cb_gemm_tn_instage_supported(_lib.ptr(g_like), _lib.ptr(g_like), _lib.ptr(x), _ld(x), int(M), int(x.shape[1]))))
 
 
-def mm_tn_instage(g, mfold, x0_bits, x, p_g, g_seed, p_x, x_seed, row0=0):
+def mm_tn_instage(g, mfold, x0_bits, x, p_g, g_seed, p_x, x_seed, row0=0, keep=None):
     import ctypes
     from . import ops
     lib = _lib.load()
@@ -234,7 +239,8 @@
     with torch.cuda.device(g.device):
         _lib.check(lib.cb_gemm_tn_instage_f32(_lib.ptr(g), _lib.ptr(mfold), _lib.ptr(x0_bits), _lib.ptr(x), _ld(x), _lib.ptr(out), _lib.ptr(colsum), M, K2,
                                               float(p_g), ctypes.c_uint64(g_seed), float(p_x), ctypes.c_uint64(x_seed), ops.seed_dev_ptr(), int(row0),
-                                              _lib.ptr(ws), wsb, _lib.stream_ptr()), 'cb_gemm_tn_instage_f32')
+                                              _lib.ptr(ws), wsb, _lib.ptr(keep[0] if keep else None), _lib.ptr(keep[1] if keep else None), _lib.stream_ptr()),
+                   'cb_gemm_tn_instage_f32')
     return out, colsum
 
 
diff --git a/gnn-tail-generalization_amd/trunk.py b/gnn-tail-generalization_amd/trunk.py
--- a/gnn-tail-generalization_amd/trunk.py
+++ b/gnn-tail-generalization_amd/trunk.py
@@ -51,8 +51,8 @@
             for name, here in ctx.saved_layout}
 
 
-def _dw_regen(x, gz, p, seed, row0, rowscale):
-    dw = gemm.mm_tn_adrop(x, gz, p, seed, row0, rowscale=rowscale)
+def _dw_regen(x, gz, p, seed, row0, rowscale, keep_x0=None):
+    dw = gemm.mm_tn_adrop(x, gz, p, seed, row0, rowscale=rowscale, keep_x0=keep_x0)
     return dw if dw is not None else gemm.mm_tn(ops._dropout_raw(x, p, seed, row0 * x.shape[1]), gz, rowscale=rowscale)
 
 
@@ -483,14 +483,16 @@
 
     def _front(self):
         c, x, w_in, b_in, row0, bwd, p, seeds = self.cfg, self.x, self.w_in, self.b_in, self.row0, self.bwd, self.cfg.p, self.cfg.seeds
+        self.keep = [None, None]
         indrop = p > 0 and _switch('CB_TRUNK_INDROP', '1') != '0'
         copy = _switch('CB_TRUNK_X0_COPY', '1') == '1'
         if (indrop or p == 0) and not c.agg_bf16 and c.L >= 1 and w_in.shape[0] == 256 and _switch('CB_TRUNK_FRONT', '1') != '0':
             w0, _b0, le0 = self.layers[0]
             fr = gemm.trunk_front(x, w_in, b_in, w0, self.a, le0, p, seeds[0], seeds[1], row0, want_bits=bwd, want_drop=bwd and p > 0 and copy,
-                                  z_out=_exchanged(self.graph, x.shape[0]) if hasattr(self.graph, 'part') else None)
+                                  z_out=_exchanged(self.graph, x.shape[0]) if hasattr(self.graph, 'part') else None, want_keep=self._keep_words())
             if fr is not None:
-                x0, x0_bits, cur, z_front = fr
+                x0, x0_bits, cur, z_front = fr[:4]
+                self.keep = list(fr[4:6]) if len(fr) > 4 else self.keep
                 return (x, x0, x0_bits, x0 if p == 0 else cur, z_front), True
         if indrop:
             wb = bwd and w_in.shape[0] == 256
@@ -506,6 +508,12 @@
         else:
             x0 = cur = gemm.mm_nn(xd, w_in.t().contiguous(), bias=b_in, relu=True)
         return (xd, x0, None, cur, None), False
+
+    def _keep_words(self):
+        c, x = self.cfg, self.x
+        return (_switch('CB_KEEP_WORDS', '1') != '0' and self.bwd and c.p > 0 and self.row0 == 0 and not hasattr(self.graph, 'part') and not c.residual
+                and not c.agg_bf16 and _switch('CB_INSTAGE_FOLD', '1') != '0' and x.dim() == 2 and x.shape[1] == 128 and x.stride(1) == 1
+                and gemm.mm_tn_instage_supported(x.new_empty((1, 256)), x, x.shape[0]))
 
     def dropped_x0(self):
         return ops._dropout_raw(self.x0, self.cfg.p, self.cfg.seeds[1], self.row0 * self.x0.shape[1])
@@ -612,7 +620,7 @@
         ctx.graph, ctx.cfg, ctx.row0, ctx.indrop, ctx.n_layer_params = graph, cfg, f.row0, f.indrop, len(layer_params)
         if f.bwd:
             _save(ctx, xd=f.xd, x0=f.x0, w_in=w_in, w_out=w_out, saved_in=f.saved_in, saved_bits=f.saved_bits, layer_params=layer_params,
-                  h_last=f.h_last, h_below=f.h_below, x0_bits=f.x0_bits)
+                  h_last=f.h_last, h_below=f.h_below, x0_bits=f.x0_bits, keep=f.keep)
             ro = f.ro
             ctx.saved_rows = SavedRows('S0' if (ro.plan is not None or ro.sharded is not None) else 'all',
                                        'absent' if f.h_last is not None else 'S1' if (ro.plan is not None and ro.below is not None) else 'all')
@@ -643,6 +651,7 @@
         sv = _saved(ctx)
         self.xd, self.x0, self.w_in, self.w_out = sv['xd'], sv['x0'], sv['w_in'], sv['w_out']
         self.saved_in, self.saved_bits, self.x0_bits = sv['saved_in'], sv['saved_bits'], sv['x0_bits']
+        self.keep = sv['keep'] if sv['keep'][0] is not None and ctx.row0 == 0 and c.p > 0 else None
         self.h_last, self.h_below = sv['h_last'], sv['h_below']
         self.lp, self.where = _layers(sv['layer_params']), ctx.saved_rows
         self.a, self.bnorm = graph.norm_out, graph.norm_in
@@ -680,7 +689,7 @@
     def _dw(self, l, x_in, gz):
         if x_in is not None:
             return gemm.mm_tn(x_in, gz, rowscale=self.a)
-        return _dw_regen(self.x0, gz, self.p, self.seed(1), self.row0, self.a)
+        return _dw_regen(self.x0, gz, self.p, self.seed(1), self.row0, self.a, keep_x0=self.keep[1] if self.keep else None)
 
     def _second(self, below, g_above, pos_above=None):
         if not self.residual or g_above is None:
@@ -912,7 +921,7 @@
         graph, p, need, xd, row0 = self.graph, self.p, self.need, self.xd, self.row0
         g, c.g = c.g, None
         if self.mfold is not None:
-            d_w_in, d_b_in = gemm.mm_tn_instage(g, self.mfold, self.x0_bits, xd, p, self.seed(1), p, self.seeds[0], row0)
+            d_w_in, d_b_in = gemm.mm_tn_instage(g, self.mfold, self.x0_bits, xd, p, self.seed(1), p, self.seeds[0], row0, keep=self.keep)
             del g
             self.gx0 = self.g_mix = self.mfold = None
             graph.instage_folds = getattr(graph, 'instage_folds', 0) + 1
diff --git a/include/coldbrew_hip.h b/include/coldbrew_hip.h
--- a/include/coldbrew_hip.h
+++ b/include/coldbrew_hip.h
@@ -196,7 +196,7 @@
 int cb_trunk_front_f32(const float* x, int64_t ld_x, int64_t M, int64_t K, const void* image_in, const float* bias_in, const void* image_0,
                        const float* rowscale, const float* addend, int64_t ld_add, float* x0, int64_t ld_x0, uint64_t* relu_bits, float* x0_drop,
                        int64_t ld_drop, float* z0, int64_t ld_z, float drop_p, uint64_t seed_x, uint64_t seed_x0, const uint64_t* seed_dev,
-                       int64_t row0, void* stream);
+                       int64_t row0, uint32_t* keep_x, uint64_t* keep_x0, void* stream);
 
 int cb_spmm_csr_weighted_f32(const int32_t* rowptr, const int32_t* col, const float* w, int64_t N, int64_t E, const float* h, int64_t ld_h,
                              int64_t d, const float* row_scale, const float* bias, int relu, float* out, int64_t ld_out, void* stream);
@@ -213,7 +213,8 @@
                           const uint64_t* seed_dev, int64_t row0, uint64_t* relu_bits, void* stream);
 int cb_gemm_tn_adrop_supported(const float* A, int64_t lda, const float* G, int64_t ldg, int64_t K1, int64_t K2);
 int cb_gemm_tn_adrop_f32(const float* A, int64_t lda, const float* G, int64_t ldg, const float* rowscale, float* C, int64_t M, int64_t K1, int64_t K2,
-                         float a_drop_p, uint64_t a_seed, const uint64_t* seed_dev, int64_t row0, void* ws, size_t ws_bytes, void* stream);
+                         float a_drop_p, uint64_t a_seed, const uint64_t* seed_dev, int64_t row0, void* ws, size_t ws_bytes, const uint64_t* keep_x0,
+                         void* stream);
 int cb_gemm_tn_gdrop_supported(const float* A, int64_t lda, const float* G, int64_t ldg, int64_t K1, int64_t K2);
 int cb_gemm_tn_gdrop_f32(const float* A, int64_t lda, const float* G, int64_t ldg, float* C, int64_t M, int64_t K1, int64_t K2, float g_drop_p,
                          uint64_t g_seed, const uint64_t* seed_dev, int64_t row0, void* ws, size_t ws_bytes, void* stream);
@@ -221,7 +222,7 @@
 size_t cb_gemm_tn_instage_workspace_bytes(int64_t M, int64_t K2);
 int cb_gemm_tn_instage_f32(const float* g, const float* mfold, const uint64_t* x0_bits, const float* X, int64_t ldx, float* C, float* colsum, int64_t M, int64_t K2,
                            float g_drop_p, uint64_t g_seed, float x_drop_p, uint64_t x_seed, const uint64_t* seed_dev, int64_t row0, void* ws, size_t ws_bytes,
-                           void* stream);
+                           const uint32_t* keep_x, const uint64_t* keep_x0, void* stream);
 
 int cb_spmm_gemm_store_rows_f32(const cb_csr_view* g, const float* h, int64_t ld_h, int64_t d, const float* col_scale, float* out, int64_t ld_out,
                                 const void* image, const float* g_rowscale, const float* bias, const int64_t* row_ids, const cb_trunk_store* store,
```
